# Chris10M/Ev2Hands

Hardware: AMD Instinct MI355X
Metric: event-windows/sec at B=256 N=2048 (f16x2) (higher is better)
Workload: dtype f32 (each f32 operand split into 2 fp16 planes with per-window power-of-two range scaling, 3 plane products per MAC on the f16 MFMA, f32 accumulate); 1 GPU; TEHNet.forward+MANO both hands, B=256/GPU N=2048 C=4 fp32, E-clouds, random-init 342-key checkpoint, synthetic MANO-shaped assets; global_batch=256, points=2048, channels=4, precision=f16x2, forwards_in_flight=1, world_size_seen=1, parallelism=batch-shard x1

## Files before the change

### ev2hands_amd/csrc/attention.hip

```cpp
#include "common.hpp"
#include "ev2hands_hip.h"

namespace {

constexpr int ATT_D = 256;

__global__ __launch_bounds__(1024) void attn_sim_kernel(const float4* __restrict__ logits, const float* __restrict__ query,
                                                        int ldq, size_t hand_stride, int N, float* __restrict__ sim) {
    __shared__ float red[4][4][ATT_D];
    const int b = blockIdx.x, h = blockIdx.y;
    const int d = threadIdx.x & (ATT_D - 1), part = threadIdx.x >> 8;
    const int per = (N + 3) / 4;
    const int n_lo = part * per, n_hi = min(N, n_lo + per);
    const float* q = query + h * hand_stride + (size_t)b * N * ldq + d;
    const float4* kk = logits + (size_t)b * N;
    float a0 = 0.f, a1 = 0.f, a2 = 0.f, a3 = 0.f;
    int n = n_lo;
    for (; n + 4 <= n_hi; n += 4) {
        const float q0 = q[(size_t)n * ldq], q1 = q[(size_t)(n + 1) * ldq], q2 = q[(size_t)(n + 2) * ldq],
                    q3 = q[(size_t)(n + 3) * ldq];
        const float4 k0 = kk[n], k1 = kk[n + 1], k2 = kk[n + 2], k3 = kk[n + 3];
        a0 = fmaf(k0.x, q0, a0); a1 = fmaf(k0.y, q0, a1); a2 = fmaf(k0.z, q0, a2); a3 = fmaf(k0.w, q0, a3);
        a0 = fmaf(k1.x, q1, a0); a1 = fmaf(k1.y, q1, a1); a2 = fmaf(k1.z, q1, a2); a3 = fmaf(k1.w, q1, a3);
        a0 = fmaf(k2.x, q2, a0); a1 = fmaf(k2.y, q2, a1); a2 = fmaf(k2.z, q2, a2); a3 = fmaf(k2.w, q2, a3);
        a0 = fmaf(k3.x, q3, a0); a1 = fmaf(k3.y, q3, a1); a2 = fmaf(k3.z, q3, a2); a3 = fmaf(k3.w, q3, a3);
    }
    for (; n < n_hi; ++n) {
        const float q0 = q[(size_t)n * ldq];
        const float4 k0 = kk[n];
        a0 = fmaf(k0.x, q0, a0); a1 = fmaf(k0.y, q0, a1); a2 = fmaf(k0.z, q0, a2); a3 = fmaf(k0.w, q0, a3);
    }
    red[part][0][d] = a0; red[part][1][d] = a1; red[part][2][d] = a2; red[part][3][d] = a3;
    __syncthreads();
    if (part == 0) {
        float s[4];
#pragma unroll
        for (int c = 0; c < 4; ++c) {
            const float t = ((red[0][c][d] + red[1][c][d]) + red[2][c][d]) + red[3][c][d];
            s[c] = 0.0625f * t;
        }
        const float mx = fmaxf(fmaxf(s[0], s[1]), fmaxf(s[2], s[3]));
        float e[4], sum = 0.f;
#pragma unroll
        for (int c = 0; c < 4; ++c) { e[c] = expf(s[c] - mx); sum += e[c]; }
#pragma unroll
        for (int c = 0; c < 4; ++c) sim[(((size_t)b * 2 + h) * 4 + c) * ATT_D + d] = e[c] / sum;
    }
}

constexpr int ZS_ROWS = 256;

__global__ __launch_bounds__(256) void attn_zsum_kernel(const float4* __restrict__ logits, const float* __restrict__ q1, int ldq, int N,
                                                        float* __restrict__ zpart) {
    __shared__ float4 sk[ZS_ROWS + 2];
    const int b = blockIdx.y, ch = blockIdx.x, nch = gridDim.x, tid = threadIdx.x;
    const int n0 = ch * ZS_ROWS, n1 = min(N, n0 + ZS_ROWS);
    for (int i = tid; i < ZS_ROWS + 2; i += 256) {
        const int n = n0 - 1 + i;
        sk[i] = (n >= 0 && n < N) ? logits[(size_t)b * N + n] : make_float4(0.f, 0.f, 0.f, 0.f);
    }
    __syncthreads();
    float ax[3][4], ay[3][4];
#pragma unroll
    for (int t = 0; t < 3; ++t)
#pragma unroll
        for (int c = 0; c < 4; ++c) { ax[t][c] = 0.f; ay[t][c] = 0.f; }
    const float* qp = q1 + ((size_t)b * N + n0) * ldq + 2 * tid;
    auto step = [&](int i, float2 v) {
#pragma unroll
        for (int t = 0; t < 3; ++t) {
            const float4 k = sk[i + 2 - t];
            ax[t][0] = fmaf(k.x, v.x, ax[t][0]); ax[t][1] = fmaf(k.y, v.x, ax[t][1]); ax[t][2] = fmaf(k.z, v.x, ax[t][2]); ax[t][3] = fmaf(k.w, v.x, ax[t][3]);
            ay[t][0] = fmaf(k.x, v.y, ay[t][0]); ay[t][1] = fmaf(k.y, v.y, ay[t][1]); ay[t][2] = fmaf(k.z, v.y, ay[t][2]); ay[t][3] = fmaf(k.w, v.y, ay[t][3]);
        }
    };
    const int rows = n1 - n0;
    int i = 0;
    for (; i + 4 <= rows; i += 4) {
        float2 v[4];
#pragma unroll
        for (int u = 0; u < 4; ++u) v[u] = *reinterpret_cast<const float2*>(qp + (size_t)(i + u) * ldq);
#pragma unroll
        for (int u = 0; u < 4; ++u) step(i + u, v[u]);
    }
    for (; i < rows; ++i) step(i, *reinterpret_cast<const float2*>(qp + (size_t)i * ldq));
    float* zp = zpart + ((size_t)b * nch + ch) * 12 * 512 + 2 * tid;
#pragma unroll
    for (int c = 0; c < 4; ++c)
#pragma unroll
        for (int t = 0; t < 3; ++t) *reinterpret_cast<float2*>(zp + (c * 3 + t) * 512) = make_float2(ax[t][c], ay[t][c]);
}

__global__ __launch_bounds__(1024) void attn_simfold_kernel(const float* __restrict__ zpart, int nch, const float4* __restrict__ logits, int N,
                                                            const float* __restrict__ w4t0, const float* __restrict__ w4t1,
                                                            const float* __restrict__ b40, const float* __restrict__ b41, float* __restrict__ sim) {
    __shared__ float4 zs[3 * ATT_D];
    __shared__ float4 kp[1024];
    __shared__ float4 kp2[32];
    __shared__ float red[3][4][ATT_D];
    const int b = blockIdx.x, h = blockIdx.y, tid = threadIdx.x, d = tid & (ATT_D - 1), q = tid >> 8;
    const float* w4t = h ? w4t1 : w4t0;
    if (q < 3) {
        float z[4] = {0.f, 0.f, 0.f, 0.f};
        for (int ch = 0; ch < nch; ++ch)
#pragma unroll
            for (int c = 0; c < 4; ++c) z[c] += zpart[(((size_t)b * nch + ch) * 12 + c * 3 + q) * 512 + h * ATT_D + d];
        zs[q * ATT_D + d] = make_float4(z[0], z[1], z[2], z[3]);
    }
    float4 ks = make_float4(0.f, 0.f, 0.f, 0.f);
    for (int n = tid; n < N; n += 1024) {
        const float4 k = logits[(size_t)b * N + n];
        ks.x += k.x; ks.y += k.y; ks.z += k.z; ks.w += k.w;
    }
    kp[tid] = ks;
    __syncthreads();
    if (tid < 32) {
        float4 k2 = kp[tid * 32];
        for (int j = 1; j < 32; ++j) { const float4 k = kp[tid * 32 + j]; k2.x += k.x; k2.y += k.y; k2.z += k.z; k2.w += k.w; }
        kp2[tid] = k2;
    }
    __syncthreads();
    float a0 = 0.f, a1 = 0.f, a2 = 0.f, a3 = 0.f;
    if (q == 0) {
        float4 K = kp2[0];
        for (int j = 1; j < 32; ++j) { const float4 k = kp2[j]; K.x += k.x; K.y += k.y; K.z += k.z; K.w += k.w; }
        const float bd = (h ? b41 : b40)[d];
        a0 = bd * K.x; a1 = bd * K.y; a2 = bd * K.z; a3 = bd * K.w;
    }
    constexpr int KQ = 3 * ATT_D / 4;
#pragma unroll 8
    for (int k = q * KQ; k < (q + 1) * KQ; ++k) {
        const float w = w4t[(size_t)k * ATT_D + d];
        const float4 z = zs[k];
        a0 = fmaf(w, z.x, a0); a1 = fmaf(w, z.y, a1); a2 = fmaf(w, z.z, a2); a3 = fmaf(w, z.w, a3);
    }
    if (q > 0) { red[q - 1][0][d] = a0; red[q - 1][1][d] = a1; red[q - 1][2][d] = a2; red[q - 1][3][d] = a3; }
    __syncthreads();
    if (q == 0) {
        const float t[4] = {a0, a1, a2, a3};
        float s[4];
#pragma unroll
        for (int c = 0; c < 4; ++c) s[c] = 0.0625f * (((t[c] + red[0][c][d]) + red[1][c][d]) + red[2][c][d]);
        const float mx = fmaxf(fmaxf(s[0], s[1]), fmaxf(s[2], s[3]));
        float e[4], sum = 0.f;
#pragma unroll
        for (int c = 0; c < 4; ++c) { e[c] = expf(s[c] - mx); sum += e[c]; }
#pragma unroll
        for (int c = 0; c < 4; ++c) sim[(((size_t)b * 2 + h) * 4 + c) * ATT_D + d] = e[c] / sum;
    }
}

constexpr int CTX_PTS_PER_WAVE = 32;
template <int VBF16>
__global__ __launch_bounds__(256) void attn_context_kernel(const float* __restrict__ sim, const float* __restrict__ value,
                                                           int ldv, int N, size_t rows_total, float* __restrict__ hf8,
                                                           unsigned* __restrict__ amax, int amax_hand_stride,
                                                           const float* __restrict__ value_unscale, const float* __restrict__ vscale = nullptr) {
    const int b = blockIdx.y;
    const int lane = threadIdx.x & 63, wave = threadIdx.x >> 6;
    float4 w[2][4];
    const float4 vu = value_unscale ? *reinterpret_cast<const float4*>(value_unscale + lane * 4) : make_float4(1.f, 1.f, 1.f, 1.f);
#pragma unroll
    for (int h = 0; h < 2; ++h)
#pragma unroll
        for (int c = 0; c < 4; ++c) {
            float4 t = *reinterpret_cast<const float4*>(sim + (((size_t)b * 2 + h) * 4 + c) * ATT_D + lane * 4);
            t.x *= vu.x; t.y *= vu.y; t.z *= vu.z; t.w *= vu.w;
            if constexpr (VBF16 == 2) {
                const float iv = 1.f / vscale[b];
                t.x *= iv; t.y *= iv; t.z *= iv; t.w *= iv;
            }
            w[h][c] = t;
        }
    const int n0 = (blockIdx.x * 4 + wave) * CTX_PTS_PER_WAVE;
    unsigned am = 0u;
    for (int n = n0; n < n0 + CTX_PTS_PER_WAVE && n < N; ++n) {
        const size_t row = (size_t)b * N + n;
        float4 v;
        if constexpr (VBF16 == 1) {
            const uint2 h = *reinterpret_cast<const uint2*>(reinterpret_cast<const unsigned short*>(value) + row * ldv + lane * 4);
            v = make_float4(__uint_as_float(h.x << 16), __uint_as_float(h.x & 0xffff0000u), __uint_as_float(h.y << 16), __uint_as_float(h.y & 0xffff0000u));
        } else if constexpr (VBF16 == 2) {
            typedef _Float16 h16x2 __attribute__((ext_vector_type(2)));
            const uint2 h = *reinterpret_cast<const uint2*>(reinterpret_cast<const unsigned short*>(value) + row * ldv + lane * 4);
            const h16x2 a = __builtin_bit_cast(h16x2, h.x), b_ = __builtin_bit_cast(h16x2, h.y);
            v = make_float4((float)a[0], (float)a[1], (float)b_[0], (float)b_[1]);
        } else {
            v = *reinterpret_cast<const float4*>(value + row * ldv + lane * 4);
        }
        float acc[8];
#pragma unroll
        for (int h = 0; h < 2; ++h)
#pragma unroll
            for (int c = 0; c < 4; ++c)
                acc[h * 4 + c] = fmaf(w[h][c].w, v.w, fmaf(w[h][c].z, v.z, fmaf(w[h][c].y, v.y, w[h][c].x * v.x)));
        float r4[4], r2[2];
        const bool hi32 = lane & 32, hi16 = lane & 16, hi8 = lane & 8;
#pragma unroll
        for (int i = 0; i < 4; ++i) r4[i] = (hi32 ? acc[4 + i] : acc[i]) + __shfl_xor(hi32 ? acc[i] : acc[4 + i], 32, 64);
#pragma unroll
        for (int i = 0; i < 2; ++i) r2[i] = (hi16 ? r4[2 + i] : r4[i]) + __shfl_xor(hi16 ? r4[i] : r4[2 + i], 16, 64);
        float r = (hi8 ? r2[1] : r2[0]) + __shfl_xor(hi8 ? r2[0] : r2[1], 8, 64);
        r += __shfl_xor(r, 4, 64);
        r += __shfl_xor(r, 2, 64);
        r += __shfl_xor(r, 1, 64);
        if ((lane & 7) == 0) {
            const int gsum = lane >> 3;
            hf8[((size_t)(gsum >> 2) * rows_total + row) * 8 + (gsum & 3)] = r;
            am = max(am, __float_as_uint(r) & 0x7fffffffu);
        } else if ((lane & 7) == 4) {
            const int gsum = lane >> 3;
            hf8[((size_t)(gsum >> 2) * rows_total + row) * 8 + 4 + (gsum & 3)] = 0.f;
        }
    }
    if (amax) {
        unsigned a0 = wave_max_u32_dpp(lane < 32 ? am : 0u), a1 = wave_max_u32_dpp(lane < 32 ? 0u : am);
        if (lane == 0) {
            if (a0) atomicMax(&amax[b], a0);
            if (a1) atomicMax(&amax[amax_hand_stride + b], a1);
        }
    }
}

}

extern "C" int ev2h_attn_sim(const float* logits_pm, const float* query_pm, int ldq, size_t query_hand_stride, int B, int N,
                             float* sim, ev2h_stream_t stream) {
    EV2H_CHECK_ARG(logits_pm && query_pm && sim && B > 0 && N > 0 && ldq >= ATT_D);
    dim3 grid(B, 2);
    attn_sim_kernel<<<grid, 1024, 0, (hipStream_t)stream>>>((const float4*)logits_pm, query_pm, ldq, query_hand_stride, N, sim);
    EV2H_CHECK_LAUNCH();
    return EV2H_OK;
}

extern "C" size_t ev2h_attn_sim_folded_scratch(int B, int N) {
    if (B <= 0 || N <= 0) return 0;
    return (size_t)B * ceil_div(N, ZS_ROWS) * 12 * 512;
}

int ev2h_attn_simfold_partials(const float* zpart, int rows_per_partial, const float* logits_pm, int B, int N, const float* w4t_left,
                               const float* w4t_right, const float* b4_left, const float* b4_right, float* sim, ev2h_stream_t stream) {
    EV2H_CHECK_ARG(zpart && logits_pm && w4t_left && w4t_right && b4_left && b4_right && sim && B > 0 && N > 0 && rows_per_partial > 0 &&
                   N % rows_per_partial == 0);
    attn_simfold_kernel<<<dim3(B, 2), 1024, 0, (hipStream_t)stream>>>(zpart, N / rows_per_partial, (const float4*)logits_pm, N, w4t_left, w4t_right,
                                                                      b4_left, b4_right, sim);
    EV2H_CHECK_LAUNCH();
    return EV2H_OK;
}

extern "C" int ev2h_attn_sim_folded(const float* logits_pm, const float* q1_pm, int ldq, int B, int N, const float* w4t_left,
                                    const float* w4t_right, const float* b4_left, const float* b4_right, float* scratch, float* sim,
                                    ev2h_stream_t stream) {
    EV2H_CHECK_ARG(logits_pm && q1_pm && w4t_left && w4t_right && b4_left && b4_right && scratch && sim);
    EV2H_CHECK_ARG(B > 0 && N > 0 && ldq >= 2 * ATT_D && (ldq % 2) == 0);
    const int nch = ceil_div(N, ZS_ROWS);
    attn_zsum_kernel<<<dim3(nch, B), 256, 0, (hipStream_t)stream>>>((const float4*)logits_pm, q1_pm, ldq, N, scratch);
    EV2H_CHECK_LAUNCH();
    attn_simfold_kernel<<<dim3(B, 2), 1024, 0, (hipStream_t)stream>>>(scratch, nch, (const float4*)logits_pm, N, w4t_left, w4t_right, b4_left,
                                                                      b4_right, sim);
    EV2H_CHECK_LAUNCH();
    return EV2H_OK;
}

extern "C" int ev2h_attn_context(const float* sim, const float* value_pm, int ldv, int B, int N, float* hf8, uint32_t* hf_amax,
                                 int amax_hand_stride, const float* value_unscale, ev2h_stream_t stream) {
    EV2H_CHECK_ARG(sim && value_pm && hf8 && B > 0 && N > 0 && ldv >= ATT_D && (ldv % 4) == 0);
    dim3 grid(ceil_div(N, 4 * CTX_PTS_PER_WAVE), B);
    attn_context_kernel<0><<<grid, 256, 0, (hipStream_t)stream>>>(sim, value_pm, ldv, N, (size_t)B * N, hf8, hf_amax, amax_hand_stride, value_unscale);
    EV2H_CHECK_LAUNCH();
    return EV2H_OK;
}

int ev2h_attn_context_bf16rows(const float* sim, const void* value_pm, int ldv, int B, int N, float* hf8, const float* value_unscale, ev2h_stream_t stream) {
    EV2H_CHECK_ARG(sim && value_pm && hf8 && B > 0 && N > 0 && ldv >= ATT_D && (ldv % 4) == 0);
    dim3 grid(ceil_div(N, 4 * CTX_PTS_PER_WAVE), B);
    attn_context_kernel<1><<<grid, 256, 0, (hipStream_t)stream>>>(sim, reinterpret_cast<const float*>(value_pm), ldv, N, (size_t)B * N, hf8, nullptr, 0, value_unscale);
    EV2H_CHECK_LAUNCH();
    return EV2H_OK;
}

int ev2h_attn_context_f16rows(const float* sim, const void* value_pm, int ldv, int B, int N, float* hf8, uint32_t* hf_amax, int amax_hand_stride,
                              const float* value_unscale, const float* vscale, ev2h_stream_t stream) {
    EV2H_CHECK_ARG(sim && value_pm && hf8 && vscale && B > 0 && N > 0 && ldv >= ATT_D && (ldv % 4) == 0);
    dim3 grid(ceil_div(N, 4 * CTX_PTS_PER_WAVE), B);
    attn_context_kernel<2><<<grid, 256, 0, (hipStream_t)stream>>>(sim, reinterpret_cast<const float*>(value_pm), ldv, N, (size_t)B * N, hf8, hf_amax, amax_hand_stride,
                                                                 value_unscale, vscale);
    EV2H_CHECK_LAUNCH();
    return EV2H_OK;
}
```

### ev2hands_amd/csrc/forward.hip

```cpp
#include <cstdarg>
#include <cstdio>
#include <cstdlib>
#include <cstring>

#include "common.hpp"
#include "planes.hpp"
#include "ev2hands_hip.h"
#include "side_stream.hpp"
#include "workspace.hpp"

int ev2h_gemm_init();

static thread_local char g_err[512] = "";

void ev2h_set_error(const char* fmt, ...) {
    va_list ap;
    va_start(ap, fmt);
    vsnprintf(g_err, sizeof(g_err), fmt, ap);
    va_end(ap);
}

extern "C" const char* ev2h_last_error(void) { return g_err; }
extern "C" int ev2h_abi_version(void) { return EV2H_ABI_VERSION; }

extern "C" void ev2h_struct_sizes(size_t out[8]) {
    out[0] = sizeof(ev2h_gemm_desc);
    out[1] = sizeof(ev2h_sa_desc);
    out[2] = sizeof(ev2h_sa_module);
    out[3] = sizeof(ev2h_weights);
    out[4] = sizeof(ev2h_mano_consts);
    out[5] = sizeof(ev2h_outputs);
    out[6] = sizeof(ev2h_fp_desc);
    out[7] = sizeof(ev2h_tensor_desc);
}

extern "C" int ev2h_init(void) {
    (void)ev2h_side_ctx(nullptr, false);
    return ev2h_gemm_init();
}

static thread_local struct {
    char tag[32];
    hipEvent_t* start;
    hipEvent_t* stop;
    int n;
    long calls;
} g_prof = {"", nullptr, nullptr, 0, 0};

extern "C" int ev2h_profile_set(const char* tag, void** start_events, void** stop_events, int n) {
    if (!tag || n <= 0 || !start_events || !stop_events) {
        g_prof.tag[0] = 0; g_prof.start = g_prof.stop = nullptr; g_prof.n = 0; g_prof.calls = 0;
        return EV2H_OK;
    }
    snprintf(g_prof.tag, sizeof(g_prof.tag), "%s", tag);
    g_prof.start = reinterpret_cast<hipEvent_t*>(start_events);
    g_prof.stop = reinterpret_cast<hipEvent_t*>(stop_events);
    g_prof.n = n;
    g_prof.calls = 0;
    return EV2H_OK;
}

static inline bool prof_hit(const char* tag) { return g_prof.n > 0 && !strcmp(tag, g_prof.tag); }
static inline void prof_begin(const char* tag, ev2h_stream_t st) {
    if (prof_hit(tag)) (void)hipEventRecord(g_prof.start[g_prof.calls % g_prof.n], (hipStream_t)st);
}
static inline void prof_end(const char* tag, ev2h_stream_t st) {
    if (prof_hit(tag)) { (void)hipEventRecord(g_prof.stop[g_prof.calls % g_prof.n], (hipStream_t)st); ++g_prof.calls; }
}

namespace {
__global__ void clock_probe_kernel(unsigned long long ticks, unsigned long long* out) {
    const unsigned long long c0 = __builtin_amdgcn_s_memtime(), r0 = __builtin_amdgcn_s_memrealtime();
    unsigned long long r1 = r0;
    while (r1 - r0 < ticks) { __builtin_amdgcn_s_sleep(8); r1 = __builtin_amdgcn_s_memrealtime(); }
    const unsigned long long c1 = __builtin_amdgcn_s_memtime();
    r1 = __builtin_amdgcn_s_memrealtime();
    if (threadIdx.x == 0) { out[0] = c1 - c0; out[1] = r1 - r0; }
}
}

extern "C" int ev2h_shader_clock_probe(ev2h_stream_t stream, int spin_us, unsigned long long* out_dev) {
    EV2H_CHECK_ARG(out_dev && spin_us > 0 && spin_us <= 100000);
    clock_probe_kernel<<<1, 64, 0, (hipStream_t)stream>>>((unsigned long long)spin_us * 100ull, out_dev);
    EV2H_CHECK_LAUNCH();
    return EV2H_OK;
}

int ev2h_fps_multi_chunk(const float* pts4, int B, int N, int njobs, const int* S, const int64_t* const* init, int32_t* const* idx, float* const* ctr4,
                         int s_begin, int s_end, float* state, ev2h_stream_t stream);
int ev2h_ball_query_range(const float* pts4, const float* ctr4, int B, int N, int S, int s_off, int s_cnt, int nrad, const double* radius,
                          const int* nsample, int32_t* const* gidx, int32_t* cnt, ev2h_stream_t stream);
bool ev2h_gemm_bf16_zsum_supported(const ev2h_gemm_desc* d);
int ev2h_gemm_bf16_zsum(const ev2h_gemm_desc* d, const float* key_pm, float* zpart, int x_bf16, ev2h_stream_t stream, const float* x_scale = nullptr);
int ev2h_fp_mlp_ex(const ev2h_fp_desc* d, int t_bf16, int out_bf16, ev2h_stream_t stream, float* row16_scale = nullptr, float w3_norm = 0.f, float b3_max = 0.f);
int ev2h_attn_context_f16rows(const float* sim, const void* value_pm, int ldv, int B, int N, float* hf8, uint32_t* hf_amax, int amax_hand_stride,
                              const float* value_unscale, const float* vscale, ev2h_stream_t stream);
int ev2h_attn_context_bf16rows(const float* sim, const void* value_pm, int ldv, int B, int N, float* hf8, const float* value_unscale, ev2h_stream_t stream);
int ev2h_attn_simfold_partials(const float* zpart, int rows_per_partial, const float* logits_pm, int B, int N, const float* w4t_left,
                               const float* w4t_right, const float* b4_left, const float* b4_right, float* sim, ev2h_stream_t stream);

namespace {

struct Call {
    Ws ws;
    int prec = EV2H_PREC_F32;
    int f16_families = 0;
    ev2h_stream_t st = nullptr;
    SideCtx* side = nullptr;
    int fam_prec(int fam) const { return prec == EV2H_PREC_F16 && !(f16_families & fam) ? EV2H_PREC_F16X2 : prec; }
    int signal_side(int e) const {
        if (!side) return EV2H_OK;
        EV2H_CHECK_HIP(hipEventRecord(side->ev[e], (hipStream_t)st));
        EV2H_CHECK_HIP(hipStreamWaitEvent(side->stream, side->ev[e], 0));
        return EV2H_OK;
    }
    int side_records(int e) const {
        if (side) EV2H_CHECK_HIP(hipEventRecord(side->ev[e], side->stream));
        return EV2H_OK;
    }
    int wait_side(int e) const {
        if (side) EV2H_CHECK_HIP(hipStreamWaitEvent((hipStream_t)st, side->ev[e], 0));
        return EV2H_OK;
    }
};

struct Rng {
    const uint32_t* xa = nullptr; const uint32_t* xa2 = nullptr; int xg = 0;
    uint32_t* ya = nullptr; int yg = 0;
};

#define RUN(expr)                 \
    do {                          \
        int rc__ = (expr);        \
        if (rc__) return rc__;    \
    } while (0)

struct DenseOpt {
    const float* group_bias = nullptr; int group_rows = 0, ldbias = 0;
    int taps = 1, rows_per_seq = 0;
    int rowmax_rows = 0;
    int skinny = 0;
    int fam = EV2H_FAM_DENSE;
};

static ev2h_gemm_desc dense_desc(const Call& cx, const ev2h_dense& w, const float* X, int ldx, int M, float* Y, int ldy, int relu, const Rng& rg,
                                 const DenseOpt& o = {}) {
    ev2h_gemm_desc d{};
    d.skinny = o.skinny;
    d.x_amax = rg.xa; d.x_amax2 = rg.xa2; d.x_group_rows = rg.xg; d.y_amax = rg.ya; d.y_group_rows = rg.yg;
    d.X = X; d.ldx = ldx; d.W = w.W; d.ldw = w.ldw; d.Y = Y; d.ldy = ldy;
    d.M = M; d.N = w.O; d.K = w.K;
    d.bias = o.group_bias ? o.group_bias : w.b;
    d.bias_group_rows = o.group_rows; d.ldbias = o.ldbias;
    d.relu = relu; d.post_scale = w.post_scale; d.post_shift = w.post_shift;
    d.taps = o.taps; d.rows_per_seq = o.rows_per_seq; d.rowmax_rows = o.rowmax_rows;
    d.precision = cx.fam_prec(o.fam);
    d.Ws = (cx.prec != EV2H_PREC_F32) ? w.Ws : nullptr;
    d.ws_tile_rows = w.ws_tile_rows;
    d.w_unscale = w.w_unscale;
    return d;
}

static int dense(const Call& cx, const ev2h_dense& w, const float* X, int ldx, int M, float* Y, int ldy, int relu, ev2h_stream_t st, const Rng& rg,
                 const DenseOpt& o = {}) {
    const ev2h_gemm_desc d = dense_desc(cx, w, X, ldx, M, Y, ldy, relu, rg, o);
    return ev2h_gemm(&d, st);
}

static int sa_table(int precision, const ev2h_sa_module& m, const float* feat, int ldf, int B, int Npts, float* P1, ev2h_stream_t st,
                    const uint32_t* feat_amax, uint32_t* p1_amax, float* p1_scale, bool chain = true) {
    int c1sum = 0;
    float extra = 0.f;
    for (int i = 0; i < m.nbranch; ++i) {
        c1sum += m.br[i].C1;
        extra = fmaxf(extra, m.br[i].w1x_norm * (float)m.br[i].radius * 1.0000002f);
    }
    ev2h_gemm_desc g{};
    g.X = feat; g.ldx = ldf; g.W = m.W1f; g.ldw = m.kf; g.Y = P1; g.ldy = c1sum;
    g.M = B * Npts; g.N = c1sum; g.K = m.kf; g.bias = m.b1; g.taps = 1;
    g.precision = precision;
    g.w_unscale = m.w1f_unscale;
    if (precision != EV2H_PREC_F32 && m.W1fs) { g.Ws = m.W1fs; g.ws_tile_rows = 128; }
    if (feat_amax) {
        g.x_amax = feat_amax; g.x_group_rows = Npts;
        g.y_amax = p1_amax; g.y_group_rows = Npts;
        g.y_scale = p1_scale; g.y_bound_w = m.w1f_norm; g.y_bound_b = m.b1_max + extra;
        if (precision == EV2H_PREC_F16 && chain) {
            float wmul = 1.f, badd = g.y_bound_b;
            for (int i = 0; i < m.nbranch; ++i) {
                const float iu = 1.000001f / (m.br[i].w2_unscale > 0.f ? m.br[i].w2_unscale : 1.f);
                wmul = fmaxf(wmul, m.br[i].w2_norm * iu);
                badd = fmaxf(badd, (m.br[i].w2_norm * g.y_bound_b + m.br[i].b2_max) * iu);
            }
            g.y_bound_w *= wmul; g.y_bound_b = badd;
        }
    }
    return ev2h_gemm(&g, st);
}

static bool bf16_direct_layer1(int precision, const ev2h_sa_module& m) {
    static const bool table = getenv("EV2H_L1_TABLE") != nullptr;
    return precision != EV2H_PREC_F32 && m.kf == 8 && !table;
}

static int sa_branches(int precision, const char* tag, const ev2h_sa_module& m, const float* pts4, const float* ctr4, int32_t* const* gidx,
                       const int32_t* cnt, int B, int Npts, const float* P1, float* out, int ldo, ev2h_stream_t st, bool ranges,
                       const uint32_t* p1_amax, const float* p1_scale, uint32_t* out_amax, const float* feat = nullptr, int nfeat = 0,
                       const uint32_t* feat_amax = nullptr, float* xyz_out = nullptr, int xyz_ld = 0, int s_off = 0, int s_cnt = 0) {
    int c1sum = 0;
    for (int i = 0; i < m.nbranch; ++i) c1sum += m.br[i].C1;
    int coff1 = 0, coff3 = 0;
    for (int i = 0; i < m.nbranch; ++i) {
        const ev2h_sa_branch& br = m.br[i];
        ev2h_sa_desc d{};
        d.P1 = P1 + coff1; d.ldp = c1sum; d.pts4 = pts4; d.ctr4 = ctr4; d.gidx = gidx[i];
        d.W1x = br.W1x; d.W2 = br.W2; d.b2 = br.b2; d.W3 = br.W3; d.b3 = br.b3;
        d.out = out + coff3; d.ldo = ldo;
        d.B = B; d.Npts = Npts; d.S = m.npoint; d.K = br.K; d.C1 = br.C1; d.C2 = br.C2; d.C3 = br.C3;
        if (s_cnt > 0) { d.S = s_cnt; d.S_total = m.npoint; d.s_off = s_off; }
        d.precision = precision; d.W2s = br.W2s; d.W3s = br.W3s; d.w2_unscale = br.w2_unscale; d.w3_unscale = br.w3_unscale;
        const bool direct = feat && bf16_direct_layer1(precision, m);
        if (direct) {
            d.feat = feat; d.ldf = 8; d.W1f = m.W1f + (size_t)coff1 * m.kf; d.ldw1f = m.kf; d.b1 = m.b1 + coff1; d.nfeat = nfeat;
            d.w1f_unscale = br.w1f_unscale; d.w1x_unscale = br.w1x_unscale;
            if (ranges) { d.feat_amax = feat_amax; d.w1f_norm = m.w1f_norm; d.b1_max = m.b1_max; }
        }
        if (ranges) {
            if (!direct) { d.p1_scale = p1_scale; d.p1_amax = p1_amax; }
            d.out_amax = out_amax;
            d.w1x_norm = br.w1x_norm; d.dmax = (float)br.radius * 1.0000002f ; d.w2_norm = br.w2_norm; d.b2_max = br.b2_max;
        }
        d.cnt = cnt ? cnt + i : nullptr; d.cnt_ld = m.nbranch;
        if (i == 0 && xyz_out) { d.xyz_out = xyz_out; d.xyz_ld = xyz_ld; }
        char t[40];
        snprintf(t, sizeof(t), "%s.%d", tag, i);
        prof_begin(t, st);
        RUN(ev2h_sa_mlp_max(&d, st));
        prof_end(t, st);
        coff1 += br.C1;
        coff3 += br.C3;
    }
    return EV2H_OK;
}

static int sa_module(int precision, const char* tag, const ev2h_sa_module& m, const float* feat, int ldf, const float* pts4, const float* ctr4,
                     int32_t* const* gidx, const int32_t* cnt, int B, int Npts, float* P1, float* out, int ldo, ev2h_stream_t st,
                     const uint32_t* feat_amax, uint32_t* p1_amax, float* p1_scale, uint32_t* out_amax, int nfeat = 0, float* xyz_out = nullptr,
                     int xyz_ld = 0) {
    if (!bf16_direct_layer1(precision, m)) RUN(sa_table(precision, m, feat, ldf, B, Npts, P1, st, feat_amax, p1_amax, p1_scale));
    return sa_branches(precision, tag, m, pts4, ctr4, gidx, cnt, B, Npts, P1, out, ldo, st, feat_amax != nullptr, p1_amax, p1_scale, out_amax,
                       ldf == 8 ? feat : nullptr, nfeat, feat_amax, xyz_out, xyz_ld);
}

}

static int forward_body(const ev2h_weights* w, const ev2h_mano_consts* const* mano, float* xyz_cm, int B, int C, int N, int mhlnes,
                        const int64_t* fps_init, const ev2h_outputs* out, const Call& cx, bool* forked) {
    const Ws& ws = cx.ws;
    const ev2h_stream_t st = cx.st;
    const int R = B * N;
    const int prec = cx.prec;
    const int prec_sa = cx.fam_prec(EV2H_FAM_SA), prec_rows = cx.fam_prec(EV2H_FAM_ROWS), prec_q = cx.fam_prec(EV2H_FAM_QCONV);
    auto rg = [&](int xid, int xg, int yid = -1, int yg = 0, int xid2 = -1) {
        Rng r{};
        if (ws.ranges_on) {
            r.xa = ws.r(xid); r.xg = xg;
            if (xid2 >= 0) r.xa2 = ws.r(xid2);
            if (yid >= 0) { r.ya = ws.r(yid); r.yg = yg; }
        }
        return r;
    };
    if (ws.ranges_on) EV2H_CHECK_HIP(hipMemsetAsync(ws.i(WS_RANGES), 0, ws.L.count[WS_RANGES] * 4, (hipStream_t)st));

    RUN(ev2h_prep_points(xyz_cm, B, C, N, mhlnes, ws.f(WS_PTS4), ws.f(WS_FEAT8), ws.r(R_FEAT), st));
    const bool fork = cx.side != nullptr;
    const ev2h_stream_t sd = fork ? (ev2h_stream_t)cx.side->stream : st;
    RUN(cx.signal_side(EV_INPUT));
    *forked = fork;
    if (!bf16_direct_layer1(prec, w->sa1)) RUN(sa_table(prec_sa, w->sa1, ws.f(WS_FEAT8), 8, B, N, ws.f(WS_P1A), sd, ws.r(R_FEAT), ws.r(R_P1A), ws.p1scale(0)));
    RUN(cx.side_records(EV_SA1_TABLE));
    static const int chunk_env = [] { const char* e = getenv("EV2H_FPS_CHUNKS"); return e ? atoi(e) : -1; }();
    const int chunk_max_wg = chunk_env > 1 ? chunk_env : (N <= 2048 ? 0x7fffffff : 256), chunk_min_b = chunk_env > 1 ? 1 : 8;
    const bool chunked = fork && chunk_env != 0 && B >= chunk_min_b && 3 * B <= chunk_max_wg && bf16_direct_layer1(prec, w->sa1) && w->sa1.npoint % FPS_CHUNKS == 0;
    {
        const int S[3] = {512, 128, 128};
        const int64_t* init[3] = {fps_init, fps_init + 2 * (size_t)B, fps_init + 3 * (size_t)B};
        int32_t* idx[3] = {ws.i(WS_FPS1), ws.i(WS_FPSM_L), ws.i(WS_FPSM_R)};
        float* ctr[3] = {ws.f(WS_CTR1), ws.f(WS_CTRM_L), ws.f(WS_CTRM_R)};
        if (!chunked) {
            RUN(ev2h_fps_multi(ws.f(WS_PTS4), B, N, 3, S, init, idx, ctr, st));
        } else {
            const int q = w->sa1.npoint / FPS_CHUNKS;
            for (int c = 0; c < FPS_CHUNKS; ++c) {
                RUN(ev2h_fps_multi_chunk(ws.f(WS_PTS4), B, N, 3, S, init, idx, ctr, c * q, (c + 1) * q, ws.f(WS_FPS_STATE), sd));
                RUN(cx.side_records(EV_SA1_QUARTER0 + c));
            }
        }
    }
    if (!chunked) RUN(cx.signal_side(EV_SAMPLED));
    int32_t* gi2[2] = {ws.i(WS_GIDX2_0), ws.i(WS_GIDX2_1)};
    {
        const ev2h_sa_module& m = w->sa2;
        RUN(ev2h_fps(ws.f(WS_CTR1), B, 512, 128, fps_init + (size_t)B, ws.i(WS_FPS2), ws.f(WS_CTR2), sd));
        double rad[2]; int ns[2];
        for (int i = 0; i < 2; ++i) { rad[i] = m.br[i].radius; ns[i] = m.br[i].K; }
        RUN(ev2h_ball_query(ws.f(WS_CTR1), ws.f(WS_CTR2), B, 512, 128, 2, rad, ns, gi2, ws.i(WS_CNT2), sd));
        RUN(cx.side_records(EV_SA2_QUERY));
    }
    static const bool unfused_fp1 = getenv("EV2H_FP1_UNFUSED") != nullptr;
    const bool fp1_fused = prec != EV2H_PREC_F32 && w->fp1m.W1fs && !unfused_fp1;
    if (fp1_fused) {
        RUN(ev2h_three_nn_interp(ws.f(WS_PTS4), ws.f(WS_CTR1), B, N, 512, nullptr, 0, 0, nullptr, 0, ws.i(WS_NN1_IDX), ws.f(WS_NN1_W), nullptr, sd));
        RUN(cx.side_records(EV_FP1_NN));
    }
    for (int h = 0; h < 2; ++h) {
        const ev2h_sa_module& m = w->mano_sa1[h];
        double rad[2]; int ns[2];
        int32_t* gi[2] = {ws.i(hand(WS_GIDXM0_L, h)), ws.i(hand(WS_GIDXM1_L, h))};
        for (int i = 0; i < 2; ++i) { rad[i] = m.br[i].radius; ns[i] = m.br[i].K; }
        RUN(ev2h_ball_query(ws.f(WS_PTS4), ws.f(hand(WS_CTRM_L, h)), B, N, 128, 2, rad, ns, gi, ws.i(hand(WS_CNTM_L, h)), sd));
    }
    RUN(cx.side_records(EV_HAND_QUERIES));
    {
        const ev2h_sa_module& m = w->sa1;
        double rad[3]; int ns[3];
        int32_t* gi[3] = {ws.i(WS_GIDX1_0), ws.i(WS_GIDX1_1), ws.i(WS_GIDX1_2)};
        for (int i = 0; i < 3; ++i) { rad[i] = m.br[i].radius; ns[i] = m.br[i].K; }
        if (!chunked) {
            RUN(ev2h_ball_query(ws.f(WS_PTS4), ws.f(WS_CTR1), B, N, 512, 3, rad, ns, gi, ws.i(WS_CNT1), st));
            RUN(cx.wait_side(EV_SA1_TABLE));
            RUN(sa_branches(prec_sa, "sa1", m, ws.f(WS_PTS4), ws.f(WS_CTR1), gi, ws.i(WS_CNT1), B, N, ws.f(WS_P1A), ws.f(WS_L1CAT), 576, st, ws.ranges_on,
                            ws.r(R_P1A), ws.p1scale(0), ws.r(R_L1A), ws.f(WS_FEAT8), C, ws.r(R_FEAT)));
        } else {
            const int q = m.npoint / FPS_CHUNKS;
            for (int c = 0; c < FPS_CHUNKS; ++c) {
                RUN(cx.wait_side(EV_SA1_QUARTER0 + c));
                RUN(ev2h_ball_query_range(ws.f(WS_PTS4), ws.f(WS_CTR1), B, N, 512, c * q, q, 3, rad, ns, gi, ws.i(WS_CNT1), st));
                RUN(sa_branches(prec_sa, "sa1", m, ws.f(WS_PTS4), ws.f(WS_CTR1), gi, ws.i(WS_CNT1), B, N, ws.f(WS_P1A), ws.f(WS_L1CAT), 576, st, ws.ranges_on,
                                ws.r(R_P1A), ws.p1scale(0), ws.r(R_L1A), ws.f(WS_FEAT8), C, ws.r(R_FEAT), nullptr, 0, c * q, q));
            }
        }
    }
    {
        const ev2h_sa_module& m = w->sa2;
        RUN(cx.wait_side(EV_SA2_QUERY));
        RUN(sa_module(prec_sa, "sa2", m, ws.f(WS_L1CAT), 576, ws.f(WS_CTR1), ws.f(WS_CTR2), gi2, ws.i(WS_CNT2), B, 512, ws.f(WS_P1B), ws.f(WS_L2BUF), 520, st,
                      ws.r(R_L1A), ws.r(R_P1B), ws.p1scale(1), ws.r(R_L2), 0, ws.f(WS_L2BUF) + 512, 520));
    }
    RUN(dense(cx, w->sa3[0], ws.f(WS_L2BUF), 520, B * 128, ws.f(WS_SA3H1), 256, 1, st, rg(R_L2, 128, R_SA3H1, 128, R_FEAT)));
    RUN(dense(cx, w->sa3[1], ws.f(WS_SA3H1), 256, B * 128, ws.f(WS_SA3H2), 512, 1, st, rg(R_SA3H1, 128, R_SA3H2, 128)));
    RUN(dense(cx, w->sa3[2], ws.f(WS_SA3H2), 512, B * 128, ws.f(WS_L3), 1024, 1, st, rg(R_SA3H2, 128, R_L3, 1), {.rowmax_rows = 128}));
    RUN(dense(cx, w->fp3_bcast, ws.f(WS_L3), 1024, B, ws.f(WS_FP3BIAS), 256, 0, st, rg(R_L3, 1), {.skinny = 1}));
    RUN(dense(cx, w->fp3_skip, ws.f(WS_L2BUF), 520, B * 128, ws.f(WS_FP3H), 256, 1, st, rg(R_L2, 128, R_FP3H, 128, R_FEAT),
              {.group_bias = ws.f(WS_FP3BIAS), .group_rows = 128, .ldbias = 256}));
    RUN(dense(cx, w->fp3_1, ws.f(WS_FP3H), 256, B * 128, ws.f(WS_FP3O), 256, 1, st, rg(R_FP3H, 128, R_FP3O, 128)));
    RUN(ev2h_three_nn_interp(ws.f(WS_CTR1), ws.f(WS_CTR2), B, 512, 128, ws.f(WS_FP3O), 256, 256, ws.f(WS_L1CAT) + 320, 576,
                             ws.i(WS_NN2_IDX), ws.f(WS_NN2_W), ws.r(R_L1B), st));
    RUN(dense(cx, w->fp2[0], ws.f(WS_L1CAT), 576, B * 512, ws.f(WS_FP2H), 256, 1, st, rg(R_L1A, 512, R_FP2H, 512, R_L1B)));
    RUN(dense(cx, w->fp2[1], ws.f(WS_FP2H), 256, B * 512, ws.f(WS_L1NEW), 128, 1, st, rg(R_FP2H, 512, R_L1NEW, 512)));
    static const bool unfused_cls = getenv("EV2H_CLS_UNFUSED") != nullptr;
    static const bool unfused_zsum = getenv("EV2H_ATTN_UNFUSED_ZSUM") != nullptr;
    static const bool l0_f32 = getenv("EV2H_L0_F32") != nullptr;
    const bool cls_fused = prec != EV2H_PREC_F32 && w->clsm.W2s && !unfused_cls;
    const ev2h_gemm_desc qd = dense_desc(cx, w->qconv0, ws.f(WS_L0), 256, R, ws.f(WS_Q1), 512, 1, rg(R_L0, N),
                                         {.taps = 3, .rows_per_seq = N, .fam = EV2H_FAM_QCONV});
    const bool zsum_ok = !unfused_zsum && prec != EV2H_PREC_F32 && w->qconv0.Ws && ev2h_gemm_bf16_zsum_supported(&qd);
    const bool l0_bf16 = prec == EV2H_PREC_BF16 && fp1_fused && cls_fused && zsum_ok && !l0_f32;
    const bool l0_f16 = prec == EV2H_PREC_F16 && prec_rows == EV2H_PREC_F16 && prec_q == EV2H_PREC_F16 && ws.ranges_on && fp1_fused && cls_fused && zsum_ok && !l0_f32;
    const bool l0_16 = l0_bf16 || l0_f16;
    g_last_l0_bf16 = l0_bf16 ? 1 : (l0_f16 ? 2 : 0);
    if (fp1_fused) {
        const ev2h_sa_module& m = w->fp1m;
        RUN(cx.wait_side(EV_FP1_NN));
        RUN(sa_table(prec_rows, m, ws.f(WS_L1NEW), 128, B, 512, ws.f(WS_FP1T), st, ws.r(R_L1NEW), ws.r(R_FP1T), ws.p1scale(4), false));
        ev2h_fp_desc d{};
        d.T = ws.f(WS_FP1T); d.ldt = 128; d.nn_idx = ws.i(WS_NN1_IDX); d.nn_w = ws.f(WS_NN1_W);
        d.b2 = m.br[0].b2; d.b3 = m.br[0].b3; d.W2s = m.br[0].W2s; d.W3s = m.br[0].W3s;
        d.w2_unscale = m.br[0].w2_unscale; d.w3_unscale = m.br[0].w3_unscale;
        d.out = ws.f(WS_L0); d.ldo = 256; d.B = B; d.N = N; d.S = 512; d.C1 = 128; d.C2 = 128; d.C3 = 256; d.precision = prec_rows;
        if (ws.ranges_on) {
            d.t_scale = ws.p1scale(4); d.t_amax = ws.r(R_FP1T); d.w2_norm = m.br[0].w2_norm; d.b2_max = m.br[0].b2_max; d.out_amax = ws.r(R_L0);
        }
        prof_begin("fp1", st);
        RUN(ev2h_fp_mlp_ex(&d, 0, l0_16, st, l0_f16 ? ws.p1scale(5) : nullptr, m.br[0].w3_norm, m.br[0].b3_max));
        prof_end("fp1", st);
    } else {
        RUN(ev2h_three_nn_interp(ws.f(WS_PTS4), ws.f(WS_CTR1), B, N, 512, ws.f(WS_L1NEW), 128, 128, ws.f(WS_FP1IN), 128,
                                 ws.i(WS_NN1_IDX), ws.f(WS_NN1_W), ws.r(R_FP1IN), st));
        RUN(dense(cx, w->fp1[0], ws.f(WS_FP1IN), 128, R, ws.f(WS_FP1H1), 128, 1, st, rg(R_FP1IN, N, R_FP1H1, N)));
        RUN(dense(cx, w->fp1[1], ws.f(WS_FP1H1), 128, R, ws.f(WS_FP1H2), 128, 1, st, rg(R_FP1H1, N, R_FP1H2, N)));
        RUN(dense(cx, w->fp1[2], ws.f(WS_FP1H2), 128, R, ws.f(WS_L0), 256, 1, st, rg(R_FP1H2, N, R_L0, N)));
    }
    RUN(cx.signal_side(EV_L0));
    if (cls_fused) {
        const ev2h_sa_branch& c = w->clsm;
        ev2h_fp_desc d{};
        d.T = ws.f(WS_L0); d.ldt = 256; d.b2 = c.b2; d.b3 = c.b3; d.W2s = c.W2s; d.W3s = c.W3s;
        d.w2_unscale = c.w2_unscale; d.w3_unscale = c.w3_unscale;
        d.out = ws.f(WS_LOGITS_PM); d.ldo = 4; d.out_cols = 4; d.no_relu_out = 1; d.out_cm = out->class_logits; d.out_cm_stride = out->logits_stride;
        d.B = B; d.N = N; d.C1 = c.C1; d.C2 = c.C2; d.C3 = c.C3; d.precision = prec_rows;
        if (ws.ranges_on) { d.t_amax = ws.r(R_L0); d.w2_norm = c.w2_norm; d.b2_max = c.b2_max; }
        RUN(ev2h_fp_mlp_ex(&d, l0_16, 0, sd, l0_f16 ? ws.p1scale(5) : nullptr));
    } else {
        RUN(dense(cx, w->cls0, ws.f(WS_L0), 256, R, ws.f(WS_CLSH), 256, 1, sd, rg(R_L0, N, R_CLSH, N)));
        RUN(dense(cx, w->cls4, ws.f(WS_CLSH), 256, R, ws.f(WS_LOGITS_PM), 4, 0, sd, rg(R_CLSH, N)));
        RUN(ev2h_transpose_logits(ws.f(WS_LOGITS_PM), B, N, out->class_logits, out->logits_stride, sd));
    }
    RUN(cx.side_records(EV_LOGITS));
    if (zsum_ok) {
        RUN(cx.wait_side(EV_LOGITS));
        prof_begin("qconv0", st);
        RUN(ev2h_gemm_bf16_zsum(&qd, ws.f(WS_LOGITS_PM), ws.f(WS_ZPART), l0_16, st, l0_f16 ? ws.p1scale(5) : nullptr));
        prof_end("qconv0", st);
    } else {
        prof_begin("qconv0", st);
        RUN(ev2h_gemm(&qd, st));
        prof_end("qconv0", st);
    }
    RUN(cx.wait_side(EV_LOGITS));
    if (zsum_ok) {
        RUN(ev2h_attn_simfold_partials(ws.f(WS_ZPART), 128, ws.f(WS_LOGITS_PM), B, N, w->qconv4T[0], w->qconv4T[1], w->qconv4[0].b, w->qconv4[1].b,
                                       ws.f(WS_SIM), st));
    } else {
        RUN(ev2h_attn_sim_folded(ws.f(WS_LOGITS_PM), ws.f(WS_Q1), 512, B, N, w->qconv4T[0], w->qconv4T[1], w->qconv4[0].b, w->qconv4[1].b,
                                 ws.f(WS_ZPART), ws.f(WS_SIM), st));
    }
    if (l0_bf16) RUN(ev2h_attn_context_bf16rows(ws.f(WS_SIM), ws.f(WS_L0), 256, B, N, ws.f(WS_HF8), w->l0_unscale, st));
    else if (l0_f16) RUN(ev2h_attn_context_f16rows(ws.f(WS_SIM), ws.f(WS_L0), 256, B, N, ws.f(WS_HF8), ws.r(R_HF), B, w->l0_unscale, ws.p1scale(5), st));
    else RUN(ev2h_attn_context(ws.f(WS_SIM), ws.f(WS_L0), 256, B, N, ws.f(WS_HF8), ws.r(R_HF), B, w->l0_unscale, st));
    RUN(cx.wait_side(EV_HAND_QUERIES));
    RUN(cx.signal_side(EV_HF8));
    for (int h = 0; h < 2; ++h) {
        const ev2h_sa_module& m = w->mano_sa1[h];
        ev2h_stream_t sh = (h == 1) ? sd : st;
        int32_t* gi[2] = {ws.i(hand(WS_GIDXM0_L, h)), ws.i(hand(WS_GIDXM1_L, h))};
        RUN(sa_module(prec_sa, h ? "manoR" : "manoL", m, ws.f(WS_HF8) + (size_t)h * R * 8, 8, ws.f(WS_PTS4), ws.f(hand(WS_CTRM_L, h)), gi, ws.i(hand(WS_CNTM_L, h)), B, N, ws.f(hand(WS_P1M_L, h)), ws.f(hand(WS_M1BUF_L, h)), 520, sh,
                      ws.r(R_HF + h), ws.r(R_P1M + h), ws.p1scale(2 + h), ws.r(R_M1 + h), 4, ws.f(hand(WS_M1BUF_L, h)) + 512, 520));
        RUN(dense(cx, w->mano_sa2[h][0], ws.f(hand(WS_M1BUF_L, h)), 520, B * 128, ws.f(hand(WS_MSA2H_L, h)), 256, 1, sh, rg(R_M1 + h, 128, R_MSA2H + h, 128, R_FEAT)));
        RUN(dense(cx, w->mano_sa2[h][1], ws.f(hand(WS_MSA2H_L, h)), 256, B * 128, ws.f(hand(WS_M2_L, h)), 512, 1, sh, rg(R_MSA2H + h, 128, R_M2 + h, 1), {.rowmax_rows = 128}));
        RUN(dense(cx, w->head0[h], ws.f(hand(WS_M2_L, h)), 512, B, ws.f(hand(WS_FC1_L, h)), 1024, 1, sh, rg(R_M2 + h, 1, R_FC1 + h, 1), {.skinny = 1}));
        const int ldprm = out->params_stride ? (int)out->params_stride : w->head4[h].O;
        RUN(dense(cx, w->head4[h], ws.f(hand(WS_FC1_L, h)), 1024, B, out->params[h], ldprm, 0, sh, rg(R_FC1 + h, 1), {.skinny = 1}));
        if (mano[h]) RUN(ev2h_mano(mano[h], out->params[h], ldprm, B, out->vertices[h], out->vertices_stride, out->joints[h], out->joints_stride, sh));
    }
    return EV2H_OK;
}

extern "C" int ev2h_forward(const ev2h_weights* w, const ev2h_mano_consts* mano_left, const ev2h_mano_consts* mano_right,
                            float* xyz_cm, int B, int C, int N, int mhlnes, const int64_t* fps_init, const ev2h_outputs* out,
                            void* workspace, size_t workspace_bytes, ev2h_stream_t st) {
    EV2H_CHECK_ARG(w && xyz_cm && fps_init && out && workspace);
    EV2H_CHECK_ARG(B > 0 && N >= 128 && N <= 32768 && (C == 4 || C == 5));
    EV2H_CHECK_ARG(out->class_logits && out->params[0] && out->params[1]);
    EV2H_CHECK_ARG(!mano_left || (out->vertices[0] && out->joints[0]));
    EV2H_CHECK_ARG(!mano_right || (out->vertices[1] && out->joints[1]));
    EV2H_CHECK_ARG((out->logits_stride == 0 || out->logits_stride >= (size_t)4 * N) && (out->params_stride == 0 || out->params_stride >= (size_t)w->head4[0].O));
    EV2H_CHECK_ARG(w->head4[0].O == w->head4[1].O && w->head4[0].O >= 17 && w->head4[0].O <= 61);
    for (int h = 0; h < 2; ++h) {
        const ev2h_mano_consts* mc = h ? mano_right : mano_left;
        if (mc && 3 + mc->ncomps + 13 != w->head4[h].O) {
            ev2h_set_error("ev2h_forward: the checkpoint regresses %d pose coefficients per hand, the %s MANO model takes %d", w->head4[h].O - 16,
                           h ? "right" : "left", mc->ncomps);
            return EV2H_ERR_ARG;
        }
    }
    EV2H_CHECK_ARG(out->params_stride <= 0x7fffffff);
    EV2H_CHECK_ARG((out->vertices_stride == 0 || out->vertices_stride >= 2334) && (out->joints_stride == 0 || out->joints_stride >= 63));
    EV2H_CHECK_ARG(w->sa1.npoint == 512 && w->sa2.npoint == 128 && w->mano_sa1[0].npoint == 128 && w->mano_sa1[1].npoint == 128);
    EV2H_CHECK_ARG(w->sa1.nbranch == 3 && w->sa2.nbranch == 2 && w->mano_sa1[0].nbranch == 2 && w->mano_sa1[1].nbranch == 2);
    if ((w->precision == EV2H_PREC_F16X2 || w->precision == EV2H_PREC_F16) && !(w->flags & (EV2H_W_EQUALIZED | EV2H_W_UNEQUALIZED_OK))) {
        ev2h_set_error("ev2h_forward: F16X2 / F16 weights are not channel-equalised (pack them with ev2h_pack_weights(..., EV2H_PACK_EQUALIZE), "
                       "or set EV2H_W_UNEQUALIZED_OK in ev2h_weights.flags to run them anyway, or use BF16X3 / F32)");
        return EV2H_ERR_ARG;
    }
    RUN(ev2h_init());
    Call cx;
    cx.prec = w->precision;
    cx.f16_families = w->precision == EV2H_PREC_F16 ? w->f16_families : 0;
    cx.st = st;
    Ws& ws = cx.ws;
    ws.base = static_cast<char*>(workspace);
    ws.B = B;
    ws.ranges_on = (w->precision == EV2H_PREC_F16X2 || w->precision == EV2H_PREC_F16);
    build_layout(ws.L, B, N);
    if (workspace_bytes < ws.L.total) {
        ev2h_set_error("ev2h_forward: workspace too small (%zu < %zu bytes)", workspace_bytes, ws.L.total);
        return EV2H_ERR_WORKSPACE;
    }
    const ev2h_mano_consts* mano[2] = {mano_left, mano_right};
    SideCtx* side = ev2h_side_ctx(st, true);
    if (g_side_disabled) side = nullptr;
    cx.side = side;
    bool forked = false;
    const int rc = forward_body(w, mano, xyz_cm, B, C, N, mhlnes, fps_init, out, cx, &forked);
    if (forked) {
        const hipError_t e1 = hipEventRecord(side->ev[EV_JOIN], side->stream);
        const hipError_t e2 = hipStreamWaitEvent((hipStream_t)st, side->ev[EV_JOIN], 0);
        if (rc == EV2H_OK && (e1 != hipSuccess || e2 != hipSuccess)) {
            ev2h_set_error("ev2h_forward: joining the side stream failed: %s", hipGetErrorString(e1 != hipSuccess ? e1 : e2));
            return EV2H_ERR_HIP;
        }
    }
    return rc;
}
```

### ev2hands_amd/csrc/gemm_bf16.hip

```cpp
#include <cstdlib>

#include "planes.hpp"
#include "ev2hands_hip.h"

namespace {


constexpr int GB_BM = 128, GB_BN = 128, GB_BK = 32, GB_THREADS = 512;
constexpr int GO_THREADS_ = 256, GB_BN_ = 128;

struct GemmBP {
    const float* X; int ldx;
    const float* W; int ldw;
    float* Y; int ldy;
    int M, N, K;
    const float* bias; int bias_group_rows; int ldbias;
    int relu;
    const float* post_scale; const float* post_shift;
    int taps; int Kc; int rows_per_seq;
    int rowmax_rows;
    float w_unscale;
    const unsigned* x_amax; const unsigned* x_amax2; int x_group_rows;
    unsigned* y_amax; int y_group_rows;
    float* y_scale; float y_bound_w, y_bound_b;
// ... 449 lines not shown
        for (int i = lane; i < 4 * KLD; i += 64) km = fmaxf(km, (i % KLD) < GB_BM + 2 ? fabsf(keyL[i]) : 0.f);
        sk = f16x2_scale(wave_max_u32_dpp(__float_as_uint(km)));
    }
    const int m = l31 < 12 ? l31 : 0, kc = m / 3, kt = m - 3 * kc;
    const float* kr = keyL + kc * KLD + 2 - kt + wm * 64;
    f32x16 z[2];
#pragma unroll
    for (int j = 0; j < 2; ++j)
#pragma unroll
        for (int r = 0; r < 16; ++r) z[j][r] = 0.f;
#pragma unroll
    for (int i = 0; i < 2; ++i)
#pragma unroll
        for (int kb = 0; kb < 2; ++kb) {
            u32x4 ap[plane_count(NS)];
#pragma unroll
            for (int w = 0; w < 4; ++w) {
                const float a0 = kr[32 * i + mfma_row(8 * kb + 2 * w, half)] * sk, a1 = kr[32 * i + mfma_row(8 * kb + 2 * w + 1, half)] * sk;
                unsigned o[plane_count(NS)];
                split_planes<NS>(a0, a1, o);
#pragma unroll
                for (int s_ = 0; s_ < plane_count(NS); ++s_) ap[s_][w] = o[s_];
            }
#pragma unroll
            for (int j = 0; j < 2; ++j) {
                u32x4 bq[plane_count(NS)];
#pragma unroll
                for (int w = 0; w < 4; ++w) {
                    unsigned o[plane_count(NS)];
                    split_planes<NS>(acc[i][j][8 * kb + 2 * w] * sq, acc[i][j][8 * kb + 2 * w + 1] * sq, o);
#pragma unroll
                    for (int s_ = 0; s_ < plane_count(NS); ++s_) bq[s_][w] = o[s_];
                }
#pragma unroll
                for (int q = 0; q < Planes<NS>::NPROD; ++q) z[j] = mfma_planes<NS>(ap[Planes<NS>::A[q]], bq[Planes<NS>::B[q]], z[j]);
            }
        }
    const float iq = pow2_inverse(sq), ik = pow2_inverse(sk);
    const int ch = pos0 / GB_BM, nch = p.rows_per_seq / GB_BM;
    const long bw = m0 / p.rows_per_seq;
    float* zp = p.zs_out + ((size_t)bw * nch + ch) * 12 * p.N;
    if (wm == 1) {
#pragma unroll
        for (int j = 0; j < 2; ++j)
#pragma unroll
            for (int r = 0; r < 8; ++r) {
                const int mr = mfma_row(r, half);
                if (mr < 12) red[mr * GB_BN_ + wn * 64 + j * 32 + l31] = (z[j][r] * iq) * ik;
            }
    }
    __syncthreads();
    if (wm == 0) {
#pragma unroll
        for (int j = 0; j < 2; ++j)
#pragma unroll
            for (int r = 0; r < 8; ++r) {
                const int mr = mfma_row(r, half);
                const int col = n0 + wn * 64 + j * 32 + l31;
                if (mr < 12 && col < p.N) zp[(size_t)mr * p.N + col] = (z[j][r] * iq) * ik + red[mr * GB_BN_ + wn * 64 + j * 32 + l31];
            }
    }
}

constexpr int GO_BN = 128, GO_THREADS = 256;

template <int NS, bool TAP3>
struct GOCfg {
    static constexpr int RS = plane_count(NS) * 64 + 16;
    static constexpr int A_ROWS = GB_BM + (TAP3 ? 2 : 0);
    static constexpr int A_BYTES = A_ROWS * RS;
    static constexpr int B_BYTES = GO_BN * RS;
    static constexpr int LDS_BYTES = A_BYTES + B_BYTES;
};

template <int NS, bool TAP3, bool PIPE = false, bool ZS = false>
__global__ __launch_bounds__(GO_THREADS, 3) void gemm_nt_bf16_occ_kernel(GemmBP p, const char* __restrict__ Ws) {
    static_assert(!ZS || TAP3, "the q1-free epilogue belongs to the tap kernel");
    using Cfg = GOCfg<NS, TAP3>;
    constexpr int RS = Cfg::RS;
    static_assert(!(PIPE && TAP3), "the pipelined variant is for the plain K loop");
    extern __shared__ __attribute__((aligned(16))) char smem[];
    char* sA = smem;
    char* sB = smem + Cfg::A_BYTES;

    const int L = xcd_remap(blockIdx.x, p.nblk);
    const int tn = L % p.tiles_n, tm = L / p.tiles_n;
    const int m0 = tm * GB_BM, n0 = tn * GO_BN;
    const int tid = threadIdx.x, lane = tid & 63;
    const int wave = __builtin_amdgcn_readfirstlane(tid >> 6);
    const int wm = wave >> 1, wn = wave & 1;
    const int half = lane >> 5, l31 = lane & 31;
    const int lrow = tid >> 1, lseg = tid & 1;
    const int nk = (p.K + GB_BK - 1) / GB_BK;
    f32x4 ra[4], rh[4];
    bool oka = true, okh = true, fulla = true;
    const float xs = x_row_scale<NS>(p, m0);
    const float xsh = xs;

    auto load16 = [&](const float* g, bool full, f32x4 (&r)[4]) {
        const float* g2 = full ? g + 8 : g;
        asm volatile("global_load_dwordx4 %0, %4, off\n\tglobal_load_dwordx4 %1, %4, off offset:16\n\t"
                     "global_load_dwordx4 %2, %5, off\n\tglobal_load_dwordx4 %3, %5, off offset:16"
                     : "=&v"(r[0]), "=&v"(r[1]), "=&v"(r[2]), "=&v"(r[3]) : "v"(g), "v"(g2) : "memory");
    };
    auto gload = [&](int kt, f32x4 (&dst)[4]) {
        const int k = kt * GB_BK + lseg * 16;
        int tap = 0, kc = k;
        if (p.taps == 3) { tap = k / p.Kc; kc = k - tap * p.Kc; }
        const int m = m0 + lrow;
        bool ok = (m < p.M) && (k < p.K);
        long src = m;
        if (p.taps == 3) {
            const int pos = m % p.rows_per_seq + tap - 1;
            ok = ok && (pos >= 0) && (pos < p.rows_per_seq);
            src = (long)m + tap - 1;
        }
        fulla = (k + 16 <= p.K);
        load16(p.X + (ok ? src : 0) * p.ldx + (ok ? kc : 0), fulla, dst);
        oka = ok;
    };
    auto load16h = [&](const unsigned short* g, f32x4 (&r)[4]) {
        asm volatile("global_load_dwordx4 %0, %2, off\n\tglobal_load_dwordx4 %1, %2, off offset:16" : "=&v"(r[0]), "=&v"(r[1]) : "v"(g) : "memory");
    };
    auto gload3 = [&](int kc) {
        const int k = kc * GB_BK + lseg * 16;
        const int m = m0 + lrow;
        oka = m < p.M;
        const bool xh = (NS == 1 || NS == 4) && p.x_bf16;
        if (xh) load16h(reinterpret_cast<const unsigned short*>(p.X) + (oka ? (long)m : 0) * p.ldx + k, ra);
        else load16(p.X + (oka ? (long)m : 0) * p.ldx + k, true, ra);
        if (tid < 4) {
            const long mh = (tid >> 1) ? (long)m0 + GB_BM : (long)m0 - 1;
            okh = (tid >> 1) ? ((m0 + GB_BM) % p.rows_per_seq != 0 && mh < p.M) : (m0 % p.rows_per_seq != 0);
            if (xh) load16h(reinterpret_cast<const unsigned short*>(p.X) + (okh ? mh : 0) * p.ldx + k, rh);
            else load16(p.X + (okh ? mh : 0) * p.ldx + k, true, rh);
        }
    };
    auto wait_all = [&]() {
        if constexpr (TAP3)
            asm volatile("s_waitcnt vmcnt(0)" : "+v"(ra[0]), "+v"(ra[1]), "+v"(ra[2]), "+v"(ra[3]), "+v"(rh[0]), "+v"(rh[1]), "+v"(rh[2]), "+v"(rh[3]) : : "memory");
        else
            asm volatile("s_waitcnt vmcnt(0)" : "+v"(ra[0]), "+v"(ra[1]), "+v"(ra[2]), "+v"(ra[3]) : : "memory");
    };
    auto swrite_row = [&](const f32x4 (&r)[4], bool ok, int ldsrow, float sc) {
        if constexpr ((NS == 1 || NS == 4) && TAP3) {
            if (p.x_bf16) {
#pragma unroll
                for (int hh = 0; hh < 2; ++hh) {
                    u32x4 v = __builtin_bit_cast(u32x4, r[hh]);
                    if (!ok) v = u32x4{0u, 0u, 0u, 0u};
                    *reinterpret_cast<u32x4*>(sA + ldsrow * RS + lseg * 32 + hh * 16) = v;
                }
                return;
            }
        }
#pragma unroll
        for (int hh = 0; hh < 2; ++hh) {
            f32x4 r0 = r[2 * hh], r1 = r[2 * hh + 1];
            if (!ok || (hh == 1 && !fulla)) { r0 = f32x4{0.f, 0.f, 0.f, 0.f}; r1 = r0; }
            scale_rows<NS>(r0, sc); scale_rows<NS>(r1, sc);
            unsigned q[4][plane_count(NS)];
            split_planes<NS>(r0[0], r0[1], q[0]);
            split_planes<NS>(r0[2], r0[3], q[1]);
            split_planes<NS>(r1[0], r1[1], q[2]);
            split_planes<NS>(r1[2], r1[3], q[3]);
#pragma unroll
            for (int s = 0; s < plane_count(NS); ++s) {
                u32x4 v = {q[0][s], q[1][s], q[2][s], q[3][s]};
                *reinterpret_cast<u32x4*>(sA + ldsrow * RS + s * 64 + lseg * 32 + hh * 16) = v;
            }
        }
    };
    auto dma_b = [&](int kt) {
        const char* src = Ws + ((size_t)tn * nk + kt) * Cfg::B_BYTES;
        for (int off = wave * 1024; off < Cfg::B_BYTES; off += 4 * 1024)
            __builtin_amdgcn_global_load_lds((const __attribute__((address_space(1))) void*)(src + off + lane * 16),
                                             (__attribute__((address_space(3))) void*)(sB + off), 16, 0, 0);
    };
    static_assert(Cfg::B_BYTES % 1024 == 0, "B tile image must be a whole number of 1 KiB DMA pieces");

    f32x16 acc[2][2];
#pragma unroll
    for (int i = 0; i < 2; ++i)
#pragma unroll
        for (int j = 0; j < 2; ++j)
#pragma unroll
            for (int r = 0; r < 16; ++r) acc[i][j][r] = 0.f;

    auto mma_tile = [&](int arow) {
        const char* pa = sA + (wm * 64 + l31 + arow) * RS + half * 16;
        const char* pb = sB + (wn * 64 + l31) * RS + half * 16;
#pragma unroll
        for (int m = 0; m < 2; ++m) {
            u32x4 a[2][plane_count(NS)], b[2][plane_count(NS)];
#pragma unroll
            for (int s = 0; s < plane_count(NS); ++s) {
                a[0][s] = *reinterpret_cast<const u32x4*>(pa + s * 64 + m * 32);
                a[1][s] = *reinterpret_cast<const u32x4*>(pa + 32 * RS + s * 64 + m * 32);
                b[0][s] = *reinterpret_cast<const u32x4*>(pb + s * 64 + m * 32);
                b[1][s] = *reinterpret_cast<const u32x4*>(pb + 32 * RS + s * 64 + m * 32);
            }
#pragma unroll
            for (int q = 0; q < Planes<NS>::NPROD; ++q)
#pragma unroll
                for (int i = 0; i < 2; ++i)
#pragma unroll
                    for (int j = 0; j < 2; ++j)
                        acc[i][j] = mfma_planes<NS>(a[i][Planes<NS>::A[q]], b[j][Planes<NS>::B[q]], acc[i][j]);
        }
        __builtin_amdgcn_s_waitcnt(0x0070);
    };
    if constexpr (TAP3) {
        const int nkc = p.Kc / GB_BK;
        for (int kc = 0; kc < nkc; ++kc) {
            if (kc) __builtin_amdgcn_s_barrier();
            dma_b(kc);
            gload3(kc);
            wait_all();
            swrite_row(ra, oka, lrow + 1, xs);
            if (tid < 4) swrite_row(rh, okh, (tid >> 1) ? GB_BM + 1 : 0, xsh);
            __builtin_amdgcn_s_waitcnt(0x0070);
            __builtin_amdgcn_s_barrier();
#pragma unroll 1
            for (int tap = 0; tap < 3; ++tap) {
                if (tap) {
                    __builtin_amdgcn_s_barrier();
                    dma_b(tap * nkc + kc);
                    __builtin_amdgcn_s_waitcnt(0x0070);
                    __builtin_amdgcn_s_barrier();
                }
                mma_tile(tap);
            }
        }
    } else if constexpr (PIPE) {
        constexpr int KT = 1;
        char* const base = smem;
        auto use = [&](int bufi, int j) { sA = base + (bufi * KT + j) * Cfg::LDS_BYTES; sB = sA + Cfg::A_BYTES; };
        f32x4 rq[KT][4];
        bool okq[KT], fullq[KT];
        auto stage = [&](int kt0, int bufi) {
#pragma unroll
            for (int j = 0; j < KT; ++j)
                if (kt0 + j < nk) {
                    use(bufi, j);
                    dma_b(kt0 + j);
                    gload(kt0 + j, rq[j]);
                    okq[j] = oka; fullq[j] = fulla;
                }
        };
        auto commit = [&](int kt0, int bufi) {
            if constexpr (KT == 2)
                asm volatile("s_waitcnt vmcnt(0)" : "+v"(rq[0][0]), "+v"(rq[0][1]), "+v"(rq[0][2]), "+v"(rq[0][3]), "+v"(rq[1][0]), "+v"(rq[1][1]), "+v"(rq[1][2]), "+v"(rq[1][3]) : : "memory");
            else
                asm volatile("s_waitcnt vmcnt(0)" : "+v"(rq[0][0]), "+v"(rq[0][1]), "+v"(rq[0][2]), "+v"(rq[0][3]) : : "memory");
#pragma unroll
            for (int j = 0; j < KT; ++j)
                if (kt0 + j < nk) {
                    use(bufi, j);
                    fulla = fullq[j];
                    swrite_row(rq[j], okq[j], lrow, xs);
                }
            __builtin_amdgcn_s_waitcnt(0x0070);
        };
        stage(0, 0);
        commit(0, 0);
        int bufi = 0;
        for (int kt = 0; kt < nk; kt += KT, bufi ^= 1) {
            __builtin_amdgcn_s_barrier();
            const bool more = kt + KT < nk;
            if (more) stage(kt + KT, bufi ^ 1);
#pragma unroll
            for (int j = 0; j < KT; ++j)
                if (kt + j < nk) { use(bufi, j); mma_tile(0); }
            if (more) commit(kt + KT, bufi ^ 1);
        }
        __builtin_amdgcn_s_barrier();
    } else {
        for (int kt = 0; kt < nk; ++kt) {
            if (kt) __builtin_amdgcn_s_barrier();
            dma_b(kt);
            gload(kt, ra);
            wait_all();
            swrite_row(ra, oka, lrow, xs);
            __builtin_amdgcn_s_waitcnt(0x0070);
            __builtin_amdgcn_s_barrier();
            mma_tile(0);
        }
    }

    if constexpr (ZS) {
        zsum_epilogue<NS>(p, acc, m0, wm, wn, n0, smem, tid);
        return;
    }
    gemm_epilogue<NS, 2, 2, false>(p, acc, m0, wm * 64, n0 + wn * 64, wm, wn * 64, GO_BN, reinterpret_cast<float*>(smem), tid);
}

template <int NS, bool TAP3, bool ZS = false>
int launch_go_t(const GemmBP& p, const char* Ws, hipStream_t st) {
    static PerDevice attr_set{};
    EV2H_ONCE_PER_DEVICE(attr_set,
        EV2H_CHECK_HIP(hipFuncSetAttribute(reinterpret_cast<const void*>(gemm_nt_bf16_occ_kernel<NS, TAP3, false, ZS>),
                                           hipFuncAttributeMaxDynamicSharedMemorySize, GOCfg<NS, TAP3>::LDS_BYTES)););
    gemm_nt_bf16_occ_kernel<NS, TAP3, false, ZS><<<p.nblk, GO_THREADS, GOCfg<NS, TAP3>::LDS_BYTES, st>>>(p, Ws);
    EV2H_CHECK_LAUNCH();
    return EV2H_OK;
}

template <int NS>
struct GSCfg {
    static constexpr int RS = plane_count(NS) * 64 + 16;
    static constexpr int A_BYTES = 64 * RS, B_BYTES = 64 * RS, BUF = A_BYTES + B_BYTES, LDS_BYTES = 2 * BUF;
};

template <int NS>
__global__ __launch_bounds__(GO_THREADS, 3) void gemm_nt_bf16_small_kernel(GemmBP p, const char* __restrict__ Ws) {
    using Cfg = GSCfg<NS>;
    constexpr int RS = Cfg::RS;
    extern __shared__ __attribute__((aligned(16))) char smem[];
    const int L = xcd_remap(blockIdx.x, p.nblk);
    const int tn = L % p.tiles_n, tm = L / p.tiles_n;
    const int m0 = tm * 64, n0 = tn * 64;
    const int tid = threadIdx.x, lane = tid & 63;
    const int wave = __builtin_amdgcn_readfirstlane(tid >> 6);
    const int wm = wave >> 1, wn = wave & 1;
    const int half = lane >> 5, l31 = lane & 31;
    const int lrow = tid >> 2, lseg = tid & 3;
    const int nk = (p.K + GB_BK - 1) / GB_BK;
    const float xs = x_row_scale<NS>(p, m0);
    f32x4 r0, r1;
    bool ok = true;
    auto gload = [&](int kt) {
        const int k = kt * GB_BK + lseg * 8, m = m0 + lrow;
        ok = (m < p.M) && (k < p.K);
        const float* g = p.X + (ok ? (long)m : 0) * p.ldx + (ok ? k : 0);
        asm volatile("global_load_dwordx4 %0, %2, off\n\tglobal_load_dwordx4 %1, %2, off offset:16" : "=&v"(r0), "=&v"(r1) : "v"(g) : "memory");
    };
    auto commit = [&](char* A) {
        asm volatile("s_waitcnt vmcnt(0)" : "+v"(r0), "+v"(r1) : : "memory");
        f32x4 a = r0, b = r1;
        if (!ok) { a = f32x4{0.f, 0.f, 0.f, 0.f}; b = a; }
        scale_rows<NS>(a, xs); scale_rows<NS>(b, xs);
        unsigned q[4][plane_count(NS)];
        split_planes<NS>(a[0], a[1], q[0]);
        split_planes<NS>(a[2], a[3], q[1]);
        split_planes<NS>(b[0], b[1], q[2]);
        split_planes<NS>(b[2], b[3], q[3]);
#pragma unroll
        for (int s_ = 0; s_ < plane_count(NS); ++s_) {
            u32x4 v = {q[0][s_], q[1][s_], q[2][s_], q[3][s_]};
            *reinterpret_cast<u32x4*>(A + lrow * RS + s_ * 64 + lseg * 16) = v;
        }
        __builtin_amdgcn_s_waitcnt(0x0070);
    };
    auto dma_b = [&](int kt, char* B) {
        const char* src = Ws + ((size_t)(tn >> 1) * nk + kt) * (size_t)(GO_BN * RS) + (size_t)(tn & 1) * Cfg::B_BYTES;
        for (int off = wave * 1024; off < Cfg::B_BYTES; off += 4 * 1024)
            __builtin_amdgcn_global_load_lds((const __attribute__((address_space(1))) void*)(src + off + lane * 16),
                                             (__attribute__((address_space(3))) void*)(B + off), 16, 0, 0);
    };
    static_assert(Cfg::B_BYTES % 1024 == 0, "half an image tile must be a whole number of 1 KiB DMA pieces");
    f32x16 acc[1][1];
#pragma unroll
    for (int r = 0; r < 16; ++r) acc[0][0][r] = 0.f;
    auto mma = [&](const char* A, const char* B) {
        const char* pa = A + (wm * 32 + l31) * RS + half * 16;
        const char* pb = B + (wn * 32 + l31) * RS + half * 16;
#pragma unroll
        for (int m = 0; m < 2; ++m) {
            u32x4 a[plane_count(NS)], b[plane_count(NS)];
#pragma unroll
            for (int s_ = 0; s_ < plane_count(NS); ++s_) {
                a[s_] = *reinterpret_cast<const u32x4*>(pa + s_ * 64 + m * 32);
                b[s_] = *reinterpret_cast<const u32x4*>(pb + s_ * 64 + m * 32);
            }
#pragma unroll
            for (int q = 0; q < Planes<NS>::NPROD; ++q) acc[0][0] = mfma_planes<NS>(a[Planes<NS>::A[q]], b[Planes<NS>::B[q]], acc[0][0]);
        }
        __builtin_amdgcn_s_waitcnt(0x0070);
    };
    dma_b(0, smem + Cfg::A_BYTES);
    gload(0);
    commit(smem);
    for (int kt = 0; kt < nk; ++kt) {
        __builtin_amdgcn_s_barrier();
        const bool more = kt + 1 < nk;
        char* cur = smem + (kt & 1) * Cfg::BUF;
        char* nxt = smem + ((kt + 1) & 1) * Cfg::BUF;
        if (more) { dma_b(kt + 1, nxt + Cfg::A_BYTES); gload(kt + 1); }
        mma(cur, cur + Cfg::A_BYTES);
        if (more) commit(nxt);
    }
    __builtin_amdgcn_s_barrier();
    gemm_epilogue<NS, 1, 1, false>(p, acc, m0, wm * 32, n0 + wn * 32, wm, wn * 32, 64, reinterpret_cast<float*>(smem), tid);
}

template <int NS>
int launch_go_small(GemmBP p, const char* Ws, hipStream_t st) {
    p.tiles_n = ceil_div(p.N, 64);
    p.nblk = ceil_div(p.M, 64) * p.tiles_n;
    static PerDevice attr_set{};
    EV2H_ONCE_PER_DEVICE(attr_set,
        EV2H_CHECK_HIP(hipFuncSetAttribute(reinterpret_cast<const void*>(gemm_nt_bf16_small_kernel<NS>),
                                           hipFuncAttributeMaxDynamicSharedMemorySize, GSCfg<NS>::LDS_BYTES)););
    gemm_nt_bf16_small_kernel<NS><<<p.nblk, GO_THREADS, GSCfg<NS>::LDS_BYTES, st>>>(p, Ws);
    EV2H_CHECK_LAUNCH();
    return EV2H_OK;
}

template <int NS>
constexpr int go_pipe_lds() { return 2 * GOCfg<NS, false>::LDS_BYTES; }

template <int NS>
int launch_go_pipe(const GemmBP& p, const char* Ws, hipStream_t st) {
    static PerDevice attr_set{};
    EV2H_ONCE_PER_DEVICE(attr_set,
        EV2H_CHECK_HIP(hipFuncSetAttribute(reinterpret_cast<const void*>(gemm_nt_bf16_occ_kernel<NS, false, true>),
                                           hipFuncAttributeMaxDynamicSharedMemorySize, go_pipe_lds<NS>())););
    gemm_nt_bf16_occ_kernel<NS, false, true><<<p.nblk, GO_THREADS, go_pipe_lds<NS>(), st>>>(p, Ws);
    EV2H_CHECK_LAUNCH();
    return EV2H_OK;
}

template <int NS>
int launch_go(const GemmBP& p, const char* Ws, hipStream_t st) {
    if (p.taps == 3 && p.Kc % GB_BK == 0 && p.rows_per_seq % GB_BM == 0 && p.M % p.rows_per_seq == 0)
        return launch_go_t<NS, true>(p, Ws, st);
    if (p.nblk <= 64 && p.rowmax_rows == 0 && p.taps == 1) return launch_go_small<NS>(p, Ws, st);
    if (p.nblk <= 128) return launch_go_pipe<NS>(p, Ws, st);
    return launch_go_t<NS, false>(p, Ws, st);
}

}

int ev2h_gemm_tile_geometry(int ns, int out[2]) {
    out[0] = ns == 1 ? GBCfg<1>::RS : ns == 2 ? GBCfg<2>::RS : ns == 3 ? GBCfg<3>::RS : GBCfg<4>::RS;
    out[1] = GB_BK;
    return EV2H_OK;
}

bool ev2h_gemm_bf16_zsum_supported(const ev2h_gemm_desc* d) {
    if (!(d->taps == 3 && d->Ws && d->ws_tile_rows == 128 && (d->precision == EV2H_PREC_F16X2 || d->precision == EV2H_PREC_BF16 || d->precision == EV2H_PREC_BF16X3 || d->precision == EV2H_PREC_F16) &&
          d->K % GB_BK == 0 && d->rows_per_seq > 0 && d->rows_per_seq % GB_BM == 0 && d->M % d->rows_per_seq == 0 && d->N % GO_BN == 0))
        return false;
    if ((d->precision == EV2H_PREC_F16X2 || d->precision == EV2H_PREC_F16) && d->x_amax) {
        const int xg = d->x_group_rows > 0 ? d->x_group_rows : 1;
        if (xg % GB_BM != 0 || xg % d->rows_per_seq != 0) return false;
    }
    return true;
}

int ev2h_gemm_bf16_zsum(const ev2h_gemm_desc* d, const float* key_pm, float* zpart, int x_bf16, ev2h_stream_t stream, const float* x_scale) {
    EV2H_CHECK_ARG(d && key_pm && zpart && ev2h_gemm_bf16_zsum_supported(d));
    EV2H_CHECK_ARG(!x_bf16 || d->precision == EV2H_PREC_BF16 || (d->precision == EV2H_PREC_F16 && x_scale && d->x_group_rows > 0));
    GemmBP p{};
    p.X = d->X; p.ldx = d->ldx; p.W = d->W; p.ldw = d->ldw; p.Y = nullptr; p.ldy = 0;
    p.M = d->M; p.N = d->N; p.taps = 3; p.Kc = d->K; p.K = d->K * 3;
    p.rows_per_seq = d->rows_per_seq;
    p.bias = d->bias; p.relu = d->relu; p.post_scale = d->post_scale; p.post_shift = d->post_shift;
    p.w_unscale = d->w_unscale > 0.f ? d->w_unscale : 1.f;
    p.x_group_rows = p.y_group_rows = 1;
    if ((d->precision == EV2H_PREC_F16X2 || d->precision == EV2H_PREC_F16) && d->x_amax) {
        p.x_amax = d->x_amax; p.x_amax2 = d->x_amax2; p.x_group_rows = d->x_group_rows > 0 ? d->x_group_rows : 1;
    }
    p.zs_key = reinterpret_cast<const float4*>(key_pm); p.zs_out = zpart;
    p.x_bf16 = x_bf16;
    if (x_bf16 && d->precision == EV2H_PREC_F16) { p.x_scale = x_scale; p.x_amax = p.x_amax2 = nullptr; p.x_group_rows = d->x_group_rows; }
    p.tiles_n = d->N / GO_BN;
    p.nblk = (d->M / GB_BM) * p.tiles_n;
    if (d->precision == EV2H_PREC_F16X2) return launch_go_t<2, true, true>(p, (const char*)d->Ws, (hipStream_t)stream);
    if (d->precision == EV2H_PREC_BF16) return launch_go_t<1, true, true>(p, (const char*)d->Ws, (hipStream_t)stream);
    if (d->precision == EV2H_PREC_BF16X3) return launch_go_t<3, true, true>(p, (const char*)d->Ws, (hipStream_t)stream);
    if (d->precision == EV2H_PREC_F16) return launch_go_t<4, true, true>(p, (const char*)d->Ws, (hipStream_t)stream);
    return EV2H_ERR_ARG;
}

int ev2h_gemm_bf16(const ev2h_gemm_desc* d, ev2h_stream_t stream) {
    EV2H_CHECK_ARG((d->K % 8) == 0);
    if (d->taps == 3) EV2H_CHECK_ARG((d->K % 16) == 0);
    GemmBP p{};
    p.X = d->X; p.ldx = d->ldx; p.W = d->W; p.ldw = d->ldw; p.Y = d->Y; p.ldy = d->ldy;
    p.M = d->M; p.N = d->N; p.taps = d->taps; p.Kc = d->K; p.K = d->K * d->taps;
    p.rows_per_seq = d->rows_per_seq;
    p.bias = d->bias; p.bias_group_rows = d->bias_group_rows; p.ldbias = d->ldbias;
    p.relu = d->relu; p.post_scale = d->post_scale; p.post_shift = d->post_shift;
    p.rowmax_rows = d->rowmax_rows;
    p.w_unscale = d->w_unscale > 0.f ? d->w_unscale : 1.f;
    if (d->precision == EV2H_PREC_F16X2 || d->precision == EV2H_PREC_F16) {
        p.x_amax = d->x_amax; p.x_amax2 = d->x_amax2; p.x_group_rows = d->x_group_rows > 0 ? d->x_group_rows : 1;
        p.y_amax = d->y_amax; p.y_group_rows = d->y_group_rows > 0 ? d->y_group_rows : 1;
        p.y_scale = d->y_scale; p.y_bound_w = d->y_bound_w; p.y_bound_b = d->y_bound_b;
        if (!p.x_amax) { p.x_amax2 = nullptr; p.y_scale = nullptr; }
        if (p.y_scale) EV2H_CHECK_ARG(p.x_group_rows == p.y_group_rows && d->rowmax_rows == 0);
        if (d->taps == 3 && p.x_amax) EV2H_CHECK_ARG(p.x_group_rows % d->rows_per_seq == 0);
    } else {
        p.x_group_rows = p.y_group_rows = 1;
    }
    const bool general = (p.x_amax && p.x_group_rows % GB_BM != 0) ||
                         (p.y_amax && d->rowmax_rows == 0 && p.y_group_rows % GB_BM != 0);
    if (general) {
        p.tiles_n = ceil_div(d->N, GB_BN);
        p.nblk = ceil_div(d->M, GB_BM) * p.tiles_n;
        return d->precision == EV2H_PREC_F16 ? launch_gb<4, true>(p, (hipStream_t)stream) : launch_gb<2, true>(p, (hipStream_t)stream);
    }
    if (d->Ws && d->ws_tile_rows == 128) {
        p.tiles_n = ceil_div(d->N, GO_BN);
        p.nblk = ceil_div(d->M, GB_BM) * p.tiles_n;
        if (d->precision == EV2H_PREC_BF16X3) return launch_go<3>(p, (const char*)d->Ws, (hipStream_t)stream);
        if (d->precision == EV2H_PREC_F16X2) return launch_go<2>(p, (const char*)d->Ws, (hipStream_t)stream);
        if (d->precision == EV2H_PREC_BF16) return launch_go<1>(p, (const char*)d->Ws, (hipStream_t)stream);
        if (d->precision == EV2H_PREC_F16) return launch_go<4>(p, (const char*)d->Ws, (hipStream_t)stream);
    }
    if (d->Ws) {
        p.tiles_n = ceil_div(d->N, GW_BN);
        p.nblk = ceil_div(d->M, GB_BM) * p.tiles_n;
        if (d->precision == EV2H_PREC_BF16X3) return launch_gw<3>(p, (const char*)d->Ws, (hipStream_t)stream);
        if (d->precision == EV2H_PREC_F16X2) return launch_gw<2>(p, (const char*)d->Ws, (hipStream_t)stream);
        if (d->precision == EV2H_PREC_BF16) return launch_gw<1>(p, (const char*)d->Ws, (hipStream_t)stream);
        if (d->precision == EV2H_PREC_F16) return launch_gw<4>(p, (const char*)d->Ws, (hipStream_t)stream);
    }
    p.tiles_n = ceil_div(d->N, GB_BN);
    p.nblk = ceil_div(d->M, GB_BM) * p.tiles_n;
    if (d->precision == EV2H_PREC_BF16X3) return launch_gb<3, false>(p, (hipStream_t)stream);
    if (d->precision == EV2H_PREC_F16X2) return launch_gb<2, false>(p, (hipStream_t)stream);
    if (d->precision == EV2H_PREC_BF16) return launch_gb<1, false>(p, (hipStream_t)stream);
    if (d->precision == EV2H_PREC_F16) return launch_gb<4, false>(p, (hipStream_t)stream);
    ev2h_set_error("ev2h_gemm: unknown precision %d", d->precision);
    return EV2H_ERR_ARG;
}
```

### ev2hands_amd/csrc/sa_mlp_bf16.hip

```cpp
#include <algorithm>
#include <cmath>
#include <cstdlib>
#include <type_traits>
#include "planes.hpp"
#include "ev2hands_hip.h"

namespace {

struct SaBP {
    const float* P1; int ldp;
    const float4* pts4;
    const float4* ctr4;
    const int32_t* gidx;
    const float4* W1x;
    const char* W2s; const float* b2;
    const char* W3s; const float* b3;
    float* out; int ldo;
    int B, Npts, S, K;
    int S_total, s_off;
    int nblk;
    const int32_t* cnt; int cnt_ld;
    float u2, u3;
    int per_xcd;
    const float* p1_scale; const unsigned* p1_amax;
    float w1x_norm, dmax, w2_norm, b2_max;
    unsigned* out_amax;
    const int32_t* nn_idx; const float* nn_w; int N;
    int ncols; int relu_out; float* out_cm; size_t out_cm_stride;
    const float* feat; int ldf; const float* W1f; int ldw1f; const float* b1; int nfeat;
    const unsigned* feat_amax; float w1f_norm, b1_max, u1f, u1x;
    float a1f, a1x, a1b;
    int spg;
    float* xyz_out; int xyz_ld;
    int t_bf16, out_bf16;
    float* row16_scale; float w3_norm, b3_max;
};

#ifdef EV2H_SAB_TIMELINE
__device__ long long g_sab_timeline[256];
#define STAMP(i) do { if (dbgw && strip == dbg_strip) g_sab_timeline[(i)] = __builtin_amdgcn_s_memtime(); } while (0)
#else
#define STAMP(i) do { } while (0)
#endif
constexpr int SAB_WAVES = 8;
constexpr int SAB_THREADS = SAB_WAVES * 64;

template <int C1, int C2, int C3, int NS>
struct SaBCfg {
    static constexpr int NPL = plane_count(NS);
    static constexpr bool F16 = planes_f16(NS);
    static constexpr int T2 = (C2 + 31) / 32;
    static constexpr int REM = C2 % 32;
    static constexpr int M_LAST = REM == 0 ? 2 : (REM <= 16 ? 1 : 2);
    static constexpr int C2P = 32 * (T2 - 1) + 16 * M_LAST;
    static constexpr int T3 = C3 / 32;
    static constexpr int NC1 = C1 / 32;
    static constexpr int RS2 = NPL * 64 + 16;
    static constexpr int RS3 = NPL * C2P * 2 + 16;
    static constexpr int TB2 = T2 * 32 * RS2;
    static constexpr int TB3 = 32 * RS3;
    static constexpr int SB2W = F16 ? SAB_WAVES * T2 * 32 * 4 : 0;
    static constexpr int RSA = (NS == 3) ? 112 : 80;
    static constexpr int W1B = (NS == 1 || NS == 4) ? C1 * 32 : F16 ? C1 * RSA + SAB_WAVES * C1 * 4 : C1 * RSA + C1 * 4;
    static constexpr int REC_SLOTS = 64;
    static constexpr int REC = F16 ? REC_SLOTS * 4 : 0;
    static constexpr int SMALL_NOREC = W1B + T2 * 32 * 4 + 16 + SB2W;
    static constexpr int SMALL = SMALL_NOREC + REC;
    static constexpr int tile_bytes(int cpt, int upt) { return ((cpt * TB2 > upt * TB3 ? cpt * TB2 : upt * TB3) + 1023) / 1024 * 1024; }
    static constexpr bool fits(int n) { return NC1 % n == 0 && T3 % n == 0 && 2 * tile_bytes(n, n) + SMALL <= 158 * 1024; }
    static constexpr int CPT = fits(2) ? 2 : 1, UPT = CPT;
    static constexpr int TILE = tile_bytes(CPT, UPT);
    static constexpr int LDS_BYTES = 2 * TILE + SMALL;
    static constexpr int RES_W = (NC1 * TB2 + T3 * TB3 + 1023) / 1024 * 1024;
    static constexpr int RES_LDS_BYTES = RES_W + SMALL;
    static constexpr bool FITS_RESIDENT = RES_LDS_BYTES <= 160 * 1024 && C1 >= 64;
    static constexpr bool PACK4 = (NS == 2) && REM >= 1 && REM <= 4;
};

template <int C1, int C2, int C3, int NS, bool RES, int MODE>
constexpr int sab_min_waves() {
    return (NS == 4 && RES && MODE == 3 && 2 * SaBCfg<C1, C2, C3, NS>::RES_LDS_BYTES <= 160 * 1024) ? 4 : 2;
}
template <int C1, int C2, int C3, int NS, bool RES, int MODE = 0>
__global__ __launch_bounds__(SAB_THREADS, (sab_min_waves<C1, C2, C3, NS, RES, MODE>())) void sa_mlp_max_bf16_kernel(SaBP p) {
    constexpr int WV = SAB_WAVES;
    constexpr bool ROWS = MODE == 1 || MODE == 2, DIRECT = MODE == 2;
    static_assert(!(RES && ROWS), "the row-output variants stream their tiles");
    constexpr bool L1M = (NS == 1 || NS == 4) && !ROWS;
    constexpr bool L1F = (NS == 2 || NS == 3) && MODE == 3;
    constexpr bool L2PIPE = !ROWS && (NS == 1 || NS == 4) && (C1 / 32) % 2 == 0;
    constexpr bool H2FUSE = NS != 3;
    constexpr bool FRAG_PIPE = (NS != 3);
    using Cfg = SaBCfg<C1, C2, C3, NS>;
    using PL = Planes<NS>;
    constexpr int NPL = Cfg::NPL;
    constexpr bool F16 = Cfg::F16;
    constexpr int T2 = Cfg::T2, T3 = Cfg::T3, NC1 = Cfg::NC1, RS2 = Cfg::RS2, RS3 = Cfg::RS3, C2P = Cfg::C2P;
    constexpr int WBYTES = RES ? Cfg::RES_W : 2 * Cfg::TILE;
    extern __shared__ __attribute__((aligned(16))) char smem[];
    char* wt0 = smem;
    char* wt1 = smem + Cfg::TILE;
    f32x4* sW1xT = reinterpret_cast<f32x4*>(smem + WBYTES);
    float* sb2 = reinterpret_cast<float*>(smem + WBYTES + Cfg::W1B);

    const int tid = threadIdx.x, lane = tid & 63;
    const int wave = __builtin_amdgcn_readfirstlane(tid >> 6);
    const int half = lane >> 5, l31 = lane & 31;
    const int L = xcd_remap(blockIdx.x, p.nblk);
    const int ngroups = p.B * p.S;
    constexpr bool hasfeat = MODE == 3;
    constexpr bool fmode = L1F && hasfeat;
    float* sb1w = F16 ? reinterpret_cast<float*>(smem + WBYTES + C1 * Cfg::RSA) + wave * C1 : reinterpret_cast<float*>(smem + WBYTES + C1 * Cfg::RSA);

    if constexpr (L1M) {
        const float iaf = F16 ? 1.f / p.a1f : 1.f, iax = F16 ? 1.f / p.a1x : 1.f, iab = F16 ? 1.f / p.a1b : 1.f;
        for (int i = tid; i < C1; i += WV * 64) {
            const float4 w = p.W1x[i];
            float k[16];
#pragma unroll
            for (int j = 0; j < 16; ++j) k[j] = 0.f;
            k[5] = k[8] = w.x * iax; k[6] = k[9] = w.y * iax; k[7] = k[10] = w.z * iax;
            if (hasfeat) {
                for (int j = 0; j < p.nfeat; ++j) k[j] = p.W1f[(size_t)i * p.ldw1f + j] * iaf;
#pragma unroll
                for (int j = 0; j < 4; ++j) k[12 + j] = k[j];
                k[11] = p.b1[i] * iab;
            }
            unsigned* d = reinterpret_cast<unsigned*>(smem + WBYTES) + i * 8;
#pragma unroll
            for (int j = 0; j < 8; ++j) { unsigned o[1]; split_planes<NS>(k[2 * j], k[2 * j + 1], o); d[j] = o[0]; }
        }
    } else if constexpr (!ROWS) {
        if (fmode) {
            const float iu = F16 ? 1.f / p.u1f : 1.f, iux = F16 ? 1.f / p.u1x : 1.f;
            for (int i = tid; i < C1; i += WV * 64) {
                const float4 w = p.W1x[i];
                float k[8];
#pragma unroll
                for (int j = 0; j < 8; ++j) k[j] = 0.f;
                for (int j = 0; j < p.nfeat; ++j) k[j] = p.W1f[(size_t)i * p.ldw1f + j] * iu;
                k[5] = w.x * iux; k[6] = w.y * iux; k[7] = w.z * iux;
                if constexpr (F16) {
                    unsigned* d = reinterpret_cast<unsigned*>(smem + WBYTES + i * Cfg::RSA);
#pragma unroll
                    for (int j = 0; j < 4; ++j) {
                        unsigned o[2];
                        split_planes<2>(k[2 * j], k[2 * j + 1], o);
                        d[j] = o[0]; d[4 + j] = o[0]; d[8 + j] = o[1]; d[12 + j] = 0u;
                    }
                } else if constexpr (NS == 3) {
                    unsigned* d = reinterpret_cast<unsigned*>(smem + WBYTES + i * Cfg::RSA);
#pragma unroll
                    for (int j = 0; j < 4; ++j) {
                        unsigned o[3];
                        split_planes<3>(k[2 * j], k[2 * j + 1], o);
                        d[j] = o[0]; d[4 + j] = o[0]; d[8 + j] = o[1]; d[12 + j] = o[1]; d[16 + j] = o[2]; d[20 + j] = o[0];
                    }
                    sb1w[i] = p.b1[i];
                }
            }
        } else {
            for (int i = tid; i < C1; i += WV * 64) {
                const float4 w = p.W1x[i];
                float* d = reinterpret_cast<float*>(sW1xT) + (i >> 2) * 12 + (i & 3);
                d[0] = w.x; d[4] = w.y; d[8] = w.z;
            }
        }
    }
    for (int i = tid; i < T2 * 32; i += WV * 64) sb2[i] = p.b2[i] / p.u2;
    float* sbw = F16 ? reinterpret_cast<float*>(smem + WBYTES + Cfg::W1B + T2 * 32 * 4 + 16) + wave * (T2 * 32) : sb2;

    auto dma_tile = [&](const char* src, char* dst, int bytes) {
        for (int off = wave * 1024; off < bytes; off += WV * 1024) {
            if (off + lane * 16 < bytes)
                __builtin_amdgcn_global_load_lds((const __attribute__((address_space(1))) void*)(src + off + lane * 16),
                                                 (__attribute__((address_space(3))) void*)(dst + off), 16, 0, 0);
        }
    };
    constexpr int CPT = RES ? 1 : Cfg::CPT, UPT = RES ? 1 : Cfg::UPT;
    auto dma_w2 = [&](int step, char* dst) { dma_tile(p.W2s + (size_t)step * CPT * Cfg::TB2, dst, CPT * Cfg::TB2); };
    auto dma_w3 = [&](int step, char* dst) { dma_tile(p.W3s + (size_t)step * UPT * Cfg::TB3, dst, UPT * Cfg::TB3); };

    int buf = 0;
    if constexpr (RES && F16) {
        if (tid < Cfg::REC_SLOTS) reinterpret_cast<unsigned*>(smem + WBYTES + Cfg::SMALL_NOREC)[tid] = 0u;
    }
    if constexpr (RES) {
        dma_tile(p.W2s, smem, NC1 * Cfg::TB2);
        dma_tile(p.W3s, smem + NC1 * Cfg::TB2, T3 * Cfg::TB3);
    } else {
        dma_w2(0, wt0);
    }
    asm volatile("s_waitcnt vmcnt(0)" ::: "memory");
    __syncthreads();

    const int xcd = blockIdx.x & 7, slot = blockIdx.x >> 3, nbx = p.nblk >> 3;
    const int g_end = RES ? min(ngroups, (xcd + 1) * p.per_xcd) : ngroups;
  const int spg = (RES || ROWS) ? 1 : max(1, __builtin_amdgcn_readfirstlane(p.spg)), sw = wave % spg;
  for (int g = (RES ? xcd * p.per_xcd + slot * WV : (spg > 1 ? L * (WV / spg) + wave / spg : L * WV)) + wave * (RES || spg == 1); RES ? g < g_end : true;
       g += nbx * WV) {
    const bool valid = g < ngroups;
    const int gg = valid ? g : ngroups - 1;
    const int b = gg / p.S;
    const size_t gf = ROWS ? (size_t)gg : (size_t)b * p.S_total + p.s_off + (gg - b * p.S);
    float mrun[T3];
#pragma unroll
    for (int u = 0; u < T3; ++u) mrun[u] = -INFINITY;

    float4 ctr = make_float4(0.f, 0.f, 0.f, 0.f);
    const int32_t* gi = nullptr;
    if constexpr (!ROWS) { ctr = p.ctr4[gf]; gi = p.gidx + gf * p.K + sw * 32; }
    const int row0 = ROWS ? (gg - b * p.S) * 32 : 0;
    unsigned am = 0u;
    constexpr bool C2ONE = NS == 4 && !ROWS;
    float s1 = 1.f, c2 = p.u2, c3 = C2ONE ? p.u3 * p.u2 : p.u3;
    float so = 1.f;
    float b1s_f = 1.f, b1s_x = 1.f, b1s_b = 1.f;
    const bool fform = fmode || (L1M && hasfeat);
    if constexpr (F16) {
        if (fform && p.feat_amax) {
            const float bnd = __fmaf_rn(p.w1f_norm, __uint_as_float(p.feat_amax[b]), p.b1_max) + p.w1x_norm * p.dmax;
            s1 = f16x2_scale(__float_as_uint(bnd));
            float s2 = f16x2_scale(__float_as_uint(__fmaf_rn(p.w2_norm, bnd, p.b2_max)));
            if constexpr (C2ONE) { s1 = fminf(s1, p.u2 * s2); s2 = s1 * pow2_inverse(p.u2); }
            c2 = p.u2 * s2 * pow2_inverse(s1);
            c3 = p.u3 * pow2_inverse(s2);
        } else if (!fform && p.p1_amax) {
            float a1 = __uint_as_float(p.p1_amax[b]);
            if constexpr (DIRECT) {
                if (NS == 4 && p.t_bf16) s1 = p.row16_scale[b];
                else { s1 = f16x2_scale(p.p1_amax[b]); a1 *= s1; }
            }
            else s1 = p.p1_scale[b];
            const float inv_s1 = pow2_inverse(s1);
            const float bh1 = a1 + s1 * (p.w1x_norm * p.dmax);
            const float bh2 = __fmaf_rn(p.w2_norm, bh1 * inv_s1, p.b2_max);
            float s2 = f16x2_scale(__float_as_uint(bh2));
            c2 = p.u2 * s2 * inv_s1;
            c3 = p.u3 * pow2_inverse(s2);
            if constexpr (C2ONE) {
                s2 = s1 * pow2_inverse(p.u2);
                c3 = (s2 * bh2 <= 65504.f) ? p.u3 * pow2_inverse(s2) : __uint_as_float(0x7fc00000u);
            }
        }
        s1 = __uint_as_float(__builtin_amdgcn_readfirstlane(__float_as_uint(s1)));
        c2 = __uint_as_float(__builtin_amdgcn_readfirstlane(__float_as_uint(c2)));
        c3 = __uint_as_float(__builtin_amdgcn_readfirstlane(__float_as_uint(c3)));
        if constexpr (ROWS && NS == 4) {
            if (p.out_bf16) {
                const float bound2 = 32768.f * (c3 / p.u3);
                so = f16x2_scale(__float_as_uint(__fmaf_rn(p.w3_norm, bound2, p.b3_max)));
                so = __uint_as_float(__builtin_amdgcn_readfirstlane(__float_as_uint(so)));
                if (lane == 0 && valid && row0 == 0) p.row16_scale[b] = so;
            }
        }
        for (int i = lane; i < T2 * 32; i += 64) sbw[i] = sb2[i] * s1;
        if constexpr (L1F) {
            if (fmode) for (int i = lane; i < C1; i += 64) sb1w[i] = p.b1[i] * s1;
        }
        if constexpr (L1M) { b1s_f = s1 * p.a1f; b1s_x = s1 * p.a1x; b1s_b = s1 * p.a1b; }
    }
    int my_strips = ROWS ? 1 : p.K >> 5;
    if (!ROWS && p.cnt) my_strips = min(my_strips, max(1, (p.cnt[gf * p.cnt_ld] + 31) >> 5));
    if (spg > 1) my_strips = (valid && sw < my_strips) ? 1 : 0;
    int nstrips = my_strips;
    if constexpr (!RES && !ROWS) {
        int* s_strips = reinterpret_cast<int*>(smem + WBYTES + Cfg::W1B + T2 * 32 * 4);
        if (tid == 0) *s_strips = 1;
        __syncthreads();
        if (lane == 0) atomicMax(s_strips, my_strips);
        __syncthreads();
        nstrips = *s_strips;
    }

#ifdef EV2H_SAB_TIMELINE
    const bool dbgw = (blockIdx.x == 300 && tid == 0);
    const int dbg_strip = nstrips > 1 ? 1 : 0;
#endif
    constexpr bool XPF = !ROWS && NS != 3;
    f32x4 raw[4];
    int idx_cur = 0, idx_nxt = 0;
    float4 q_cur = make_float4(0.f, 0.f, 0.f, 0.f), f0_cur = q_cur, f1_cur = q_cur;
    if constexpr (XPF) {
        idx_cur = gi[l31];
        q_cur = p.pts4[(size_t)b * p.Npts + idx_cur];
        if (hasfeat) {
            const float4* fr = reinterpret_cast<const float4*>(p.feat + ((size_t)b * p.Npts + idx_cur) * p.ldf);
            f0_cur = fr[0]; f1_cur = fr[1];
        }
    }
    for (int strip = 0; strip < nstrips; ++strip) {
        STAMP(0);
        if constexpr (!RES) {
            if (strip >= my_strips) {
                for (int c = 0; c < NC1; ++c) {
                    char* nxt = buf ? wt0 : wt1;
                    if (c % CPT == 0) { if (c + CPT < NC1) dma_w2(c / CPT + 1, nxt); else dma_w3(0, nxt); }
                    if (c % CPT == CPT - 1) { asm volatile("s_waitcnt vmcnt(0)" ::: "memory"); __syncthreads(); buf ^= 1; }
                }
                for (int u = 0; u < T3; ++u) {
                    char* nxt = buf ? wt0 : wt1;
                    if (u % UPT == 0) { if (u + UPT < T3) dma_w3(u / UPT + 1, nxt); else if (strip + 1 < nstrips) dma_w2(0, nxt); }
                    if (u % UPT == UPT - 1) { asm volatile("s_waitcnt vmcnt(0)" ::: "memory"); __syncthreads(); buf ^= 1; }
                }
                continue;
            }
        }
        float dx = 0.f, dy = 0.f, dz = 0.f;
        auto qi = [&](int j4) { return 2 * j4 + half; };
        const float4* prow = nullptr;
        const float4* trow[3] = {nullptr, nullptr, nullptr};
        float tw[3] = {0.f, 0.f, 0.f};
        u32x4 b1f = {0u, 0u, 0u, 0u};
        u32x4 b1g = {0u, 0u, 0u, 0u};
        float cj = 1.f;
        f32x4 trw[ROWS ? 3 : 1][4];
        auto fetch = [&](int c) {
#pragma unroll
            for (int j = 0; j < ((ROWS && !DIRECT) ? 3 : 1); ++j)
#pragma unroll
                for (int j4 = 0; j4 < 4; ++j4) {
                    if constexpr ((NS == 1 || NS == 4) && DIRECT) {
                        if (p.t_bf16) {
                            const uint2 h = *reinterpret_cast<const uint2*>(reinterpret_cast<const char*>(trow[j]) + (size_t)(c * 32 + 4 * qi(j4)) * 2);
                            if constexpr (NS == 1) {
                                trw[j][j4] = f32x4{__uint_as_float(h.x << 16), __uint_as_float(h.x & 0xffff0000u), __uint_as_float(h.y << 16),
                                                   __uint_as_float(h.y & 0xffff0000u)};
                            } else {
                                const f16x2 a = __builtin_bit_cast(f16x2, h.x), b_ = __builtin_bit_cast(f16x2, h.y);
                                trw[j][j4] = f32x4{(float)a[0], (float)a[1], (float)b_[0], (float)b_[1]};
                            }
                            continue;
                        }
                    }
                    trw[j][j4] = *reinterpret_cast<const f32x4*>(trow[j] + c * 8 + qi(j4));
                }
        };
        auto blend = [&]() {
#pragma unroll
            for (int j4 = 0; j4 < 4; ++j4)
#pragma unroll
                for (int e = 0; e < 4; ++e)
                    raw[j4][e] = DIRECT ? ((F16 && !(NS == 4 && p.t_bf16)) ? trw[0][j4][e] * s1 : trw[0][j4][e])
                                        : __fmaf_rn(tw[2], trw[ROWS ? 2 : 0][j4][e], __fmaf_rn(tw[1], trw[ROWS ? 1 : 0][j4][e], __fmul_rn(tw[0], trw[0][j4][e])));
        };
        if constexpr (DIRECT) {
            trow[0] = ((NS == 1 || NS == 4) && p.t_bf16)
                          ? reinterpret_cast<const float4*>(reinterpret_cast<const char*>(p.P1) + ((size_t)b * p.N + min(row0 + l31, p.N - 1)) * p.ldp * 2)
                          : reinterpret_cast<const float4*>(p.P1 + ((size_t)b * p.N + min(row0 + l31, p.N - 1)) * p.ldp);
            fetch(0);
            blend();
        } else if constexpr (ROWS) {
            const size_t gr = ((size_t)b * p.N + min(row0 + l31, p.N - 1)) * 3;
#pragma unroll
            for (int j = 0; j < 3; ++j) {
                trow[j] = reinterpret_cast<const float4*>(p.P1 + ((size_t)b * p.Npts + p.nn_idx[gr + j]) * p.ldp);
                tw[j] = p.nn_w[gr + j];
            }
            fetch(0);
            blend();
        } else {
            const int idx = XPF ? idx_cur : gi[strip * 32 + l31];
            const float4 q = XPF ? q_cur : p.pts4[(size_t)b * p.Npts + idx];
            if constexpr (XPF) idx_nxt = (strip + 1 < my_strips) ? gi[(strip + 1) * 32 + l31] : idx_cur;
            dx = __fsub_rn(q.x, ctr.x); dy = __fsub_rn(q.y, ctr.y); dz = __fsub_rn(q.z, ctr.z);
            if constexpr (F16 && !L1M) { if (!fmode) { dx *= s1; dy *= s1; dz *= s1; } }
            if (fmode) {
                if constexpr (L1F && NS == 3) {
                    const float4* fr = reinterpret_cast<const float4*>(p.feat + ((size_t)b * p.Npts + idx) * p.ldf);
                    const float4 fa = fr[0], fb = fr[1];
                    const float v[8] = {fa.x, fa.y, fa.z, fa.w, fb.x, dx, dy, dz};
#pragma unroll
                    for (int w = 0; w < 4; ++w) {
                        unsigned o[3];
                        split_planes<3>(v[2 * w], v[2 * w + 1], o);
                        b1f[w] = half ? o[1] : o[0];
                        b1g[w] = half ? o[2] : o[0];
                    }
                }
                if constexpr (L1F && F16) {
                    float v[8] = {f0_cur.x, f0_cur.y, f0_cur.z, f0_cur.w, f1_cur.x, dx, dy, dz};
                    const float af = fmaxf(fmaxf(fmaxf(fabsf(v[0]), fabsf(v[1])), fmaxf(fabsf(v[2]), fabsf(v[3]))), fabsf(v[4]));
                    const float ax = fmaxf(fmaxf(fabsf(v[5]), fabsf(v[6])), fabsf(v[7]));
                    const float kap = fminf(f16x2_scale(__float_as_uint(af)) * (1.f / p.u1f), f16x2_scale(__float_as_uint(ax)) * (1.f / p.u1x));
                    const float sgf = kap * p.u1f, sgx = kap * p.u1x;
                    cj = s1 * pow2_inverse(kap);
#pragma unroll
                    for (int j = 0; j < 5; ++j) v[j] *= sgf;
#pragma unroll
                    for (int j = 5; j < 8; ++j) v[j] *= sgx;
#pragma unroll
                    for (int w = 0; w < 4; ++w) {
                        unsigned o[2];
                        split_planes<2>(v[2 * w], v[2 * w + 1], o);
                        b1f[w] = half ? o[1] : o[0];
                    }
                }
            } else if constexpr (L1M) {
                float f[8];
#pragma unroll
                for (int j = 0; j < 8; ++j) f[j] = 0.f;
                if (hasfeat) {
                    f[0] = f0_cur.x; f[1] = f0_cur.y; f[2] = f0_cur.z; f[3] = f0_cur.w; f[4] = f1_cur.x;
                    if constexpr (F16) {
#pragma unroll
                        for (int j = 0; j < 5; ++j) f[j] *= b1s_f;
                    }
                } else {
                    prow = reinterpret_cast<const float4*>(p.P1 + ((size_t)b * p.Npts + idx) * p.ldp);
                    if (strip == 0) {
#pragma unroll
                        for (int j4 = 0; j4 < 4; ++j4) raw[j4] = *reinterpret_cast<const f32x4*>(prow + qi(j4));
                    }
                }
                auto lo_of = [](float x) {
                    if constexpr (F16) return x - (float)(_Float16)x;
                    else return x - __uint_as_float(__builtin_bit_cast(unsigned, __builtin_convertvector(f32x2{x, 0.f}, bf16x2)) << 16);
                };
                const float ex = F16 ? dx * b1s_x : dx, ey = F16 ? dy * b1s_x : dy, ez = F16 ? dz * b1s_x : dz;
                const float va[8] = {f[0], f[1], f[2], f[3], f[4], lo_of(ex), lo_of(ey), lo_of(ez)};
                const float vb[8] = {ex, ey, ez, F16 ? (hasfeat ? b1s_b : 0.f) : 1.f, lo_of(f[0]), lo_of(f[1]), lo_of(f[2]), lo_of(f[3])};
#pragma unroll
                for (int w = 0; w < 4; ++w) {
                    unsigned o[1];
                    split_planes<NS>(half ? vb[2 * w] : va[2 * w], half ? vb[2 * w + 1] : va[2 * w + 1], o);
                    b1f[w] = o[0];
                }
            } else {
                prow = reinterpret_cast<const float4*>(p.P1 + ((size_t)b * p.Npts + idx) * p.ldp);
                if (!XPF || strip == 0) {
#pragma unroll
                    for (int j4 = 0; j4 < 4; ++j4) raw[j4] = *reinterpret_cast<const f32x4*>(prow + qi(j4));
                }
            }
        }
        auto layer1 = [&](int c) {
            f32x16 acc;
            if constexpr (L1F && NS == 3) {
#pragma unroll
                for (int q = 0; q < 4; ++q) {
                    const f32x4 bv = *reinterpret_cast<const f32x4*>(sb1w + 32 * c + 8 * q + 4 * half);
#pragma unroll
                    for (int e = 0; e < 4; ++e) acc[4 * q + e] = bv[e];
                }
                const char* ar = smem + WBYTES + (32 * c + l31) * Cfg::RSA + half * 16;
                const u32x4 a0 = *reinterpret_cast<const u32x4*>(ar), a1 = *reinterpret_cast<const u32x4*>(ar + 32), a2 = *reinterpret_cast<const u32x4*>(ar + 64);
                acc = mfma_planes<3>(a2, b1g, acc);
                acc = mfma_planes<3>(a1, b1f, acc);
                return mfma_planes<3>(a0, b1f, acc);
            } else if constexpr (L1F) {
#pragma unroll
                for (int r = 0; r < 16; ++r) acc[r] = 0.f;
                const char* ar = smem + WBYTES + (32 * c + l31) * Cfg::RSA + half * 16;
                const u32x4 ah = *reinterpret_cast<const u32x4*>(ar), al = *reinterpret_cast<const u32x4*>(ar + 32);
                acc = mfma_planes<2>(al, b1f, acc);
                return mfma_planes<2>(ah, b1f, acc);
            } else {
            if (hasfeat) {
#pragma unroll
                for (int r = 0; r < 16; ++r) acc[r] = 0.f;
            } else {
#pragma unroll
                for (int r = 0; r < 16; ++r) acc[r] = raw[r >> 2][r & 3];
            }
            const u32x4 a1 = *reinterpret_cast<const u32x4*>(smem + WBYTES + (32 * c + l31) * 32 + half * 16);
            return mfma_planes<NS>(a1, b1f, acc);
            }
        };
        f32x16 d1;
        if constexpr (L1F) { if (fmode) d1 = layer1(0); }
        if constexpr (L1M) {
            d1 = layer1(0);
            if (!hasfeat && NC1 > 1) {
#pragma unroll
                for (int j4 = 0; j4 < 4; ++j4) raw[j4] = *reinterpret_cast<const f32x4*>(prow + 8 + qi(j4));
            }
        }

        f32x16 h2[T2];
#pragma unroll
        for (int t = 0; t < T2; ++t)
#pragma unroll
            for (int j = 0; j < 4; ++j) {
                const f32x4 bv = *reinterpret_cast<const f32x4*>(sbw + 32 * t + 8 * j + 4 * half);
#pragma unroll
                for (int e = 0; e < 4; ++e) h2[t][4 * j + e] = bv[e];
            }

#ifdef EV2H_SAB_TIMELINE
        if (dbgw && strip == dbg_strip) asm volatile("s_waitcnt vmcnt(0)" ::: "memory");
#endif
        STAMP(1);
        auto finish_slice = [&](int c, int j4, u32x4 (&bp)[2][NPL]) {
            if constexpr (L1M) {
#pragma unroll
                for (int w = 2 * j4; w < 2 * j4 + 2; ++w) {
                    unsigned o[1];
                    split_planes<NS>(d1[2 * w], d1[2 * w + 1], o);
                    bp[w >> 2][0][w & 3] = relu_pk_bf16(o[0]);
                }
            } else if (fmode) {
                if constexpr (L1F && NS == 3) {
                    const int q = j4;
                    unsigned lo[3], hi[3];
                    split_planes<3>(relu_bits(d1[4 * q]), relu_bits(d1[4 * q + 1]), lo);
                    split_planes<3>(relu_bits(d1[4 * q + 2]), relu_bits(d1[4 * q + 3]), hi);
#pragma unroll
                    for (int s_ = 0; s_ < 3; ++s_) {
                        bp[q >> 1][s_][(q & 1) * 2 + 0] = lo[s_];
                        bp[q >> 1][s_][(q & 1) * 2 + 1] = hi[s_];
                    }
                }
                if constexpr (L1F && F16) {
                    const int q = j4;
                    const f32x4 bv = *reinterpret_cast<const f32x4*>(sb1w + 32 * c + 8 * q + 4 * half);
                    unsigned lo[NPL], hi[NPL];
                    split_planes<NS>(relu_sat_f16(__fmaf_rn(d1[4 * q], cj, bv[0])), relu_sat_f16(__fmaf_rn(d1[4 * q + 1], cj, bv[1])), lo);
                    split_planes<NS>(relu_sat_f16(__fmaf_rn(d1[4 * q + 2], cj, bv[2])), relu_sat_f16(__fmaf_rn(d1[4 * q + 3], cj, bv[3])), hi);
#pragma unroll
                    for (int s_ = 0; s_ < NPL; ++s_) {
                        bp[q >> 1][s_][(q & 1) * 2 + 0] = lo[s_];
                        bp[q >> 1][s_][(q & 1) * 2 + 1] = hi[s_];
                    }
                }
            } else {
                const f32x4* wp = sW1xT + (8 * c + 2 * j4 + half) * 3;
                const f32x4 wx = wp[0], wy = wp[1], wz = wp[2];
                f32x4 v;
#pragma unroll
                for (int e = 0; e < 4; ++e)
                    v[e] = ROWS ? raw[j4][e] : __fmaf_rn(wz[e], dz, __fmaf_rn(wy[e], dy, __fmaf_rn(wx[e], dx, raw[j4][e])));
                unsigned lo[NPL], hi[NPL];
                if constexpr (DIRECT) {
                    split_planes<NS>(v[0], v[1], lo);
                    split_planes<NS>(v[2], v[3], hi);
                } else if constexpr (NS == 1) {
                    split_planes<NS>(v[0], v[1], lo);
                    split_planes<NS>(v[2], v[3], hi);
                    lo[0] = relu_pk_bf16(lo[0]); hi[0] = relu_pk_bf16(hi[0]);
                } else if constexpr (F16) {
                    split_planes<NS>(relu_sat_f16(v[0]), relu_sat_f16(v[1]), lo);
                    split_planes<NS>(relu_sat_f16(v[2]), relu_sat_f16(v[3]), hi);
                } else {
                    split_planes<NS>(relu_bits(v[0]), relu_bits(v[1]), lo);
                    split_planes<NS>(relu_bits(v[2]), relu_bits(v[3]), hi);
                }
#pragma unroll
                for (int s = 0; s < NPL; ++s) {
                    bp[j4 >> 1][s][(j4 & 1) * 2 + 0] = lo[s];
                    bp[j4 >> 1][s][(j4 & 1) * 2 + 1] = hi[s];
                }
            }
        };
        auto mfma_groups = [&](const char* cur, u32x4 (&bp)[2][NPL], auto&& between) {
            const char* pa = cur + l31 * RS2 + (16 * half) * 2;
            auto ld2 = [&](int pr, u32x4 (&x0)[NPL], u32x4 (&x1)[NPL]) {
                const int m0 = (2 * pr) / T2, t0 = (2 * pr) % T2, m1 = (2 * pr + 1) / T2, t1 = (2 * pr + 1) % T2;
#pragma unroll
                for (int s = 0; s < NPL; ++s) {
                    x0[s] = *reinterpret_cast<const u32x4*>(pa + 32 * t0 * RS2 + s * 64 + m0 * 16);
                    x1[s] = *reinterpret_cast<const u32x4*>(pa + 32 * t1 * RS2 + s * 64 + m1 * 16);
                }
            };
            u32x4 fa[2][2][NPL];
            if constexpr (FRAG_PIPE) ld2(0, fa[0][0], fa[0][1]);
#pragma unroll
            for (int pr = 0; pr < T2; ++pr) {
                const int m0 = (2 * pr) / T2, t0 = (2 * pr) % T2, m1 = (2 * pr + 1) / T2, t1 = (2 * pr + 1) % T2;
                if constexpr (FRAG_PIPE) {
                    if (pr + 1 < T2) ld2(pr + 1, fa[(pr + 1) & 1][0], fa[(pr + 1) & 1][1]);
                    __builtin_amdgcn_sched_barrier(0);
                } else {
                    ld2(pr, fa[pr & 1][0], fa[pr & 1][1]);
                }
                u32x4 (&a0)[NPL] = fa[pr & 1][0];
                u32x4 (&a1)[NPL] = fa[pr & 1][1];
#pragma unroll
                for (int j = 0; j < PL::NPROD; ++j) {
                    if (!(Cfg::PACK4 && t0 == T2 - 1 && PL::A[j] == 1)) h2[t0] = mfma_planes<NS>(a0[PL::A[j]], bp[m0][PL::B[j]], h2[t0]);
                    if (!(Cfg::PACK4 && t1 == T2 - 1 && PL::A[j] == 1)) h2[t1] = mfma_planes<NS>(a1[PL::A[j]], bp[m1][PL::B[j]], h2[t1]);
                }
                if constexpr (FRAG_PIPE) __builtin_amdgcn_sched_barrier(0);
                between(pr);
            }
        };
        auto l2_dma = [&](int c) {
            if constexpr (!RES) {
                char* nxt = buf ? wt0 : wt1;
                if (c % CPT == 0) { if (c + CPT < NC1) dma_w2(c / CPT + 1, nxt); else dma_w3(0, nxt); }
            }
        };
        auto l2_sync = [&](int c) {
            STAMP(4 + 4 * c);
            if constexpr (!RES) {
                if (c % CPT == CPT - 1) {
                    asm volatile("s_waitcnt vmcnt(0)" ::: "memory");
                    __syncthreads();
                    buf ^= 1;
                }
            }
            STAMP(5 + 4 * c);
        };
        u32x4 bpA[2][NPL];
        if constexpr (!L2PIPE) {
#pragma unroll 1
            for (int c = 0; c < NC1; ++c) {
                STAMP(2 + 4 * c);
                char* cur = RES ? smem + c * Cfg::TB2 : (buf ? wt1 : wt0) + (c % CPT) * Cfg::TB2;
                l2_dma(c);
#pragma unroll
                for (int j4 = 0; j4 < 4; ++j4) finish_slice(c, j4, bpA);
                if constexpr (ROWS) {
                    if (c + 1 < NC1) fetch(c + 1);
                } else if (!L1M && !fmode && c + 1 < NC1) {
#pragma unroll
                    for (int j4 = 0; j4 < 4; ++j4) raw[j4] = *reinterpret_cast<const f32x4*>(prow + (c + 1) * 8 + qi(j4));
                }
                STAMP(3 + 4 * c);
                mfma_groups(cur, bpA, [](int) {});
                if constexpr (ROWS) {
                    if (c + 1 < NC1) blend();
                }
                if constexpr (L1F) {
                    if (fmode && c + 1 < NC1) d1 = layer1(c + 1);
                }
                if constexpr (L1M) {
                    if (c + 1 < NC1) {
                        d1 = layer1(c + 1);
                        if (!hasfeat && c + 2 < NC1) {
#pragma unroll
                            for (int j4 = 0; j4 < 4; ++j4) raw[j4] = *reinterpret_cast<const f32x4*>(prow + (c + 2) * 8 + qi(j4));
                        }
                    }
                }
                l2_sync(c);
            }
        } else {
            u32x4 bpB[2][NPL];
            const bool vtab = !L1M && !fmode;
#pragma unroll
            for (int j4 = 0; j4 < 4; ++j4) {
                finish_slice(0, j4, bpA);
                if (vtab) raw[j4] = *reinterpret_cast<const f32x4*>(prow + 8 + qi(j4));
            }
            auto l2_step = [&](int c, u32x4 (&bc)[2][NPL], u32x4 (&bn)[2][NPL]) {
                STAMP(2 + 4 * c);
                char* cur = RES ? smem + c * Cfg::TB2 : (buf ? wt1 : wt0) + (c % CPT) * Cfg::TB2;
                l2_dma(c);
                const bool more = c + 1 < NC1;
                if (more) {
                    if constexpr (L1F) { if (fmode) d1 = layer1(c + 1); }
                    if constexpr (L1M) {
                        d1 = layer1(c + 1);
                        if (!hasfeat && c + 2 < NC1) {
#pragma unroll
                            for (int j4 = 0; j4 < 4; ++j4) raw[j4] = *reinterpret_cast<const f32x4*>(prow + (c + 2) * 8 + qi(j4));
                        }
                    }
                }
                STAMP(3 + 4 * c);
                mfma_groups(cur, bc, [&](int pr) {
                    if (more) {
#pragma unroll
                        for (int j4 = 0; j4 < 4; ++j4) {
                            if (j4 * T2 / 4 == pr) {
                                __builtin_amdgcn_sched_barrier(0);
                                finish_slice(c + 1, j4, bn);
                                if (vtab && c + 2 < NC1) raw[j4] = *reinterpret_cast<const f32x4*>(prow + (c + 2) * 8 + qi(j4));
                                __builtin_amdgcn_sched_barrier(0);
                            }
                        }
                    }
                });
                l2_sync(c);
            };
#pragma unroll 1
            for (int c = 0; c < NC1; c += 2) {
                l2_step(c, bpA, bpB);
                l2_step(c + 1, bpB, bpA);
            }
        }

        STAMP(38);
        if constexpr (XPF) {
            if (strip + 1 < my_strips) {
                q_cur = p.pts4[(size_t)b * p.Npts + idx_nxt];
                if (hasfeat) {
                    const float4* fr = reinterpret_cast<const float4*>(p.feat + ((size_t)b * p.Npts + idx_nxt) * p.ldf);
                    f0_cur = fr[0]; f1_cur = fr[1];
                } else {
                    const float4* pn = reinterpret_cast<const float4*>(p.P1 + ((size_t)b * p.Npts + idx_nxt) * p.ldp);
#pragma unroll
                    for (int j4 = 0; j4 < 4; ++j4) raw[j4] = *reinterpret_cast<const f32x4*>(pn + qi(j4));
                }
                idx_cur = idx_nxt;
            }
        }
        if constexpr (Cfg::PACK4) {
#pragma unroll
            for (int r = 0; r < 4; ++r) { h2[T2 - 1][r] += h2[T2 - 1][r + 4]; h2[T2 - 1][r + 4] = 0.f; }
        }
        u32x4 h2p[NPL][T2][2];
        auto split_half = [&](int t, int m) {
#pragma unroll
            for (int k = 4 * m; k < 4 * m + 4; ++k) {
                unsigned o[NPL];
                if constexpr (C2ONE) {
                    split_planes<NS>(h2[t][2 * k], h2[t][2 * k + 1], o);
                    o[0] = relu_pk_bf16(o[0]);
                }
                else if constexpr (F16) split_planes<NS>(relu_sat_f16(h2[t][2 * k] * c2), relu_sat_f16(h2[t][2 * k + 1] * c2), o);
                else if constexpr (NS == 1) { split_planes<NS>(h2[t][2 * k], h2[t][2 * k + 1], o); o[0] = relu_pk_bf16(o[0]); }
                else split_planes<NS>(relu_bits(h2[t][2 * k] * c2), relu_bits(h2[t][2 * k + 1] * c2), o);
#pragma unroll
                for (int s = 0; s < NPL; ++s) h2p[s][t][k >> 2][k & 3] = o[s];
            }
            if constexpr (Cfg::PACK4) {
                if (t == T2 - 1 && m == 0) {
                    const unsigned h01 = h2p[0][T2 - 1][0][0], h23 = h2p[0][T2 - 1][0][1];
                    const unsigned l01 = h2p[1][T2 - 1][0][0], l23 = h2p[1][T2 - 1][0][1];
                    const unsigned ph01 = (unsigned)__shfl_xor((int)h01, 32, 64), ph23 = (unsigned)__shfl_xor((int)h23, 32, 64);
                    h2p[0][T2 - 1][0][0] = half ? ph01 : h01;
                    h2p[0][T2 - 1][0][1] = half ? ph23 : h23;
                    h2p[0][T2 - 1][0][2] = half ? 0u : l01;
                    h2p[0][T2 - 1][0][3] = half ? 0u : l23;
                }
            }
        };
#pragma unroll
        for (int t = 0; t < (H2FUSE ? 1 : T2); ++t) { split_half(t, 0); split_half(t, 1); }
        STAMP(39);

        auto finish_tile = [&](int u, const f32x16& acc) {
            float mx = fmaxf(fmaxf(acc[0], acc[1]), acc[2]);
#pragma unroll
            for (int r = 3; r < 15; r += 2) mx = fmaxf(fmaxf(mx, acc[r]), acc[r + 1]);
            mx = fmaxf(mx, acc[15]);
#pragma unroll
            for (int uu = 0; uu < T3; ++uu) mrun[uu] = (uu == u) ? fmaxf(mrun[uu], mx) : mrun[uu];
        };
        constexpr int TPS = (!ROWS && (RES || UPT == 2)) ? 2 : 1;
        static_assert(T3 % TPS == 0, "layer-3 tiles are walked in pairs");
        auto l3_step = [&](int u, auto first_tag) {
            constexpr bool FIRST = decltype(first_tag)::value;
            STAMP(40 + 4 * u);
            char* cur = RES ? smem + NC1 * Cfg::TB2 + u * Cfg::TB3 : (buf ? wt1 : wt0) + (u % UPT) * Cfg::TB3;
            char* nxt = buf ? wt0 : wt1;
            if constexpr (!RES) {
                if (u % UPT == 0) {
                    const bool more_w3 = (u + UPT < T3);
                    const bool more = more_w3 || (strip + 1 < nstrips);
                    if (more_w3) dma_w3(u / UPT + 1, nxt); else if (more) dma_w2(0, nxt);
                }
            }
            float b3u = 0.f;
            if constexpr (ROWS) b3u = p.b3[32 * u + l31];
            f32x16 acc, acc1;
#pragma unroll
            for (int r = 0; r < 16; ++r) { acc[r] = 0.f; acc1[r] = 0.f; }
            const char* pb = cur + l31 * RS3 + (8 * half) * 2;
            constexpr int NG3 = 2 * (T2 - 1) + Cfg::M_LAST;
            auto ld3 = [&](int g, u32x4 (&x)[NPL], u32x4 (&x1)[TPS == 2 ? NPL : 1]) {
#pragma unroll
                for (int s = 0; s < NPL; ++s) {
                    x[s] = *reinterpret_cast<const u32x4*>(pb + s * (C2P * 2) + (16 * g) * 2);
                    if constexpr (TPS == 2) x1[s] = *reinterpret_cast<const u32x4*>(pb + Cfg::TB3 + s * (C2P * 2) + (16 * g) * 2);
                }
            };
            u32x4 fw[2][NPL], fw1[2][TPS == 2 ? NPL : 1];
            if constexpr (FRAG_PIPE) ld3(0, fw[0], fw1[0]);
#pragma unroll
            for (int t = 0; t < T2; ++t) {
#pragma unroll
                for (int m = 0; m < 2; ++m) {
                    if (t < T2 - 1 || m < Cfg::M_LAST) {
                        const int g = 2 * t + m;
                        if constexpr (FRAG_PIPE) {
                            if (g + 1 < NG3) ld3(g + 1, fw[(g + 1) & 1], fw1[(g + 1) & 1]);
                            __builtin_amdgcn_sched_barrier(0);
                        } else {
                            ld3(g, fw[g & 1], fw1[g & 1]);
                        }
                        u32x4 a[NPL];
                        u32x4 (&w)[NPL] = fw[g & 1];
                        u32x4 (&w1)[TPS == 2 ? NPL : 1] = fw1[g & 1];
#pragma unroll
                        for (int s = 0; s < NPL; ++s) a[s] = h2p[s][t][m];
#pragma unroll
                        for (int j = 0; j < PL::NPROD; ++j) {
                            if (Cfg::PACK4 && t == T2 - 1 && !(PL::A[j] == 0 && PL::B[j] == 0)) continue;
                            if constexpr (TPS == 2) {
                                acc = mfma_planes<NS>(a[PL::A[j]], w[PL::B[j]], acc);
                                acc1 = mfma_planes<NS>(a[PL::A[j]], w1[PL::B[j]], acc1);
                            } else {
                                if (((2 * t + m) * PL::NPROD + j) & 1) acc1 = mfma_planes<NS>(a[PL::A[j]], w[PL::B[j]], acc1);
                                else acc = mfma_planes<NS>(a[PL::A[j]], w[PL::B[j]], acc);
                            }
                        }
                        if constexpr (FRAG_PIPE) __builtin_amdgcn_sched_barrier(0);
                        if constexpr (FIRST) {
                            if (t + 1 < T2) {
                                if constexpr (!FRAG_PIPE) __builtin_amdgcn_sched_barrier(0);
                                split_half(t + 1, m);
                                __builtin_amdgcn_sched_barrier(0);
                            }
                        }
                    }
                }
            }
            STAMP(41 + 4 * u);
            if constexpr (TPS == 2) {
                finish_tile(u, acc);
                finish_tile(u + 1, acc1);
            } else {
#pragma unroll
                for (int r = 0; r < 16; ++r) acc[r] += acc1[r];
                if constexpr (ROWS) {
                    float* orow = p.out + ((size_t)b * p.N + row0 + 4 * half) * p.ldo + 32 * u + l31;
                    const bool colok = valid && (32 * u + l31 < p.ncols);
                    float* ocm = p.out_cm ? p.out_cm + (size_t)b * p.out_cm_stride + (size_t)(32 * u + l31) * p.N + row0 + 4 * half : nullptr;
    #pragma unroll
                    for (int r = 0; r < 16; ++r) {
                        const int pt = 8 * (r >> 2) + (r & 3);
                        float o = acc[r] * c3 + b3u;
                        if (p.relu_out) o = fmaxf(o, 0.f);
                        if (colok && row0 + 4 * half + pt < p.N) {
                            if (NS == 1 && p.out_bf16) {
                                unsigned short* o16 = reinterpret_cast<unsigned short*>(p.out) + ((size_t)b * p.N + row0 + 4 * half + pt) * p.ldo + 32 * u + l31;
                                *o16 = (unsigned short)(__builtin_bit_cast(unsigned, __builtin_convertvector(f32x2{o, 0.f}, bf16x2)) & 0xffffu);
                            } else if (NS == 4 && p.out_bf16) {
                                o = fminf(o * so, 65504.f);
                                unsigned short* o16 = reinterpret_cast<unsigned short*>(p.out) + ((size_t)b * p.N + row0 + 4 * half + pt) * p.ldo + 32 * u + l31;
                                const _Float16 h16 = (_Float16)o;
                                *o16 = __builtin_bit_cast(unsigned short, h16);
                                o = (float)h16;
                            } else
                            orow[(size_t)pt * p.ldo] = o;
                            if (ocm) ocm[pt] = o;
                            am = max(am, abs_bits(o));
                        }
                    }
                } else {
                    finish_tile(u, acc);
                }
            }
            STAMP(42 + 4 * u);
            if constexpr (!RES) {
                if ((u + TPS - 1) % UPT == UPT - 1) {
                    asm volatile("s_waitcnt vmcnt(0)" ::: "memory");
                    __syncthreads();
                    buf ^= 1;
                }
            }
            STAMP(43 + 4 * u);
        };
        if constexpr (H2FUSE) l3_step(0, std::true_type{});
#pragma unroll 1
        for (int u = H2FUSE ? TPS : 0; u < T3; u += TPS) l3_step(u, std::false_type{});
        STAMP(37);
    }
    if constexpr (!ROWS && !RES) {
        if (spg > 1) {
            float* smax = reinterpret_cast<float*>(smem);
#pragma unroll
            for (int u = 0; u < T3; ++u) {
                const float v = fmaxf(mrun[u], __shfl_xor(mrun[u], 32, 64));
                if (half == 0) smax[wave * C3 + 32 * u + l31] = v;
            }
            __syncthreads();
            if (sw == 0) {
#pragma unroll
                for (int u = 0; u < T3; ++u) {
                    float v = smax[wave * C3 + 32 * u + l31];
                    for (int k = 1; k < spg; ++k) v = fmaxf(v, smax[(wave + k) * C3 + 32 * u + l31]);
                    mrun[u] = v;
                }
            }
        }
    }
    if constexpr (!ROWS) {
#pragma unroll
        for (int u = 0; u < T3; ++u) {
            const float v = fmaxf(mrun[u], __shfl_xor(mrun[u], 32, 64));
            if (valid && half == 0 && sw == 0) {
                float o = fmaxf(v * c3 + p.b3[32 * u + l31], 0.f);
                if constexpr (C2ONE) o = (c3 == c3) ? o : c3;
                p.out[gf * p.ldo + 32 * u + l31] = o;
                am = max(am, __float_as_uint(o));
            }
        }
    }
    if constexpr (!ROWS) {
        if (p.xyz_out && valid && sw == 0 && lane < 8)
            p.xyz_out[gf * p.xyz_ld + lane] = lane == 0 ? ctr.x : lane == 1 ? ctr.y : lane == 2 ? ctr.z : 0.f;
    }
    if constexpr (F16) {
        if (p.out_amax) {
            am = wave_max_u32_dpp(am);
            char* rec = smem + WBYTES + Cfg::SMALL_NOREC;
            if constexpr (RES) {
                if (lane == 0 && am) {
                    const int slot = b - (xcd * p.per_xcd) / p.S;
                    unsigned old = 0u;
                    if (slot >= 0 && slot < Cfg::REC_SLOTS) old = atomicMax(reinterpret_cast<unsigned*>(rec) + slot, am);
                    if (am > old) atomicMax(&p.out_amax[b], am);
                }
            } else {
                int* sb = reinterpret_cast<int*>(rec);
                unsigned* sa = reinterpret_cast<unsigned*>(rec + 32);
                if (lane == 0) { sb[wave] = (valid && am) ? b : -1; sa[wave] = am; }
                __syncthreads();
                if (lane == 0 && valid && am) {
                    bool first = true;
                    unsigned m = am;
#pragma unroll
                    for (int w = 0; w < WV; ++w) {
                        if (sb[w] == b) { first = first && w >= wave; m = max(m, sa[w]); }
                    }
                    if (first) atomicMax(&p.out_amax[b], m);
                }
            }
        }
    }
    if constexpr (!RES) break;
  }
}

template <int C1, int C2, int C3, int NS, int MODE = 0>
int launch_sab(SaBP p, hipStream_t st) {
    using Cfg = SaBCfg<C1, C2, C3, NS>;
    static const bool streamed_only = getenv("EV2H_SA_STREAMED") != nullptr;
    if constexpr (Cfg::FITS_RESIDENT) {
        if (!streamed_only) {
            static PerDevice wg_slot{};
            std::atomic<int>& wg = wg_slot.cur();
            int wg_per_cu = wg.load(std::memory_order_acquire);
            if (!wg_per_cu) {
                auto k = sa_mlp_max_bf16_kernel<C1, C2, C3, NS, true, MODE>;
                EV2H_CHECK_HIP(hipFuncSetAttribute(reinterpret_cast<const void*>(k), hipFuncAttributeMaxDynamicSharedMemorySize, Cfg::RES_LDS_BYTES));
                int n = 0;
                EV2H_CHECK_HIP(hipOccupancyMaxActiveBlocksPerMultiprocessor(&n, k, SAB_THREADS, Cfg::RES_LDS_BYTES));
                wg_per_cu = n > 0 ? n : 1;
                wg.store(wg_per_cu, std::memory_order_release);
            }
            const int ngroups = p.B * p.S;
            const int want = 256 * wg_per_cu;
            p.per_xcd = ceil_div(ceil_div(ngroups, 8), SAB_WAVES) * SAB_WAVES;
            p.nblk = 8 * std::min(want / 8, ceil_div(p.per_xcd, SAB_WAVES));
            sa_mlp_max_bf16_kernel<C1, C2, C3, NS, true, MODE><<<p.nblk, SAB_THREADS, Cfg::RES_LDS_BYTES, st>>>(p);
            EV2H_CHECK_LAUNCH();
            return EV2H_OK;
        }
    }
    static PerDevice attr_set{};
    EV2H_ONCE_PER_DEVICE(attr_set,
        EV2H_CHECK_HIP(hipFuncSetAttribute(reinterpret_cast<const void*>(sa_mlp_max_bf16_kernel<C1, C2, C3, NS, false, MODE>),
                                           hipFuncAttributeMaxDynamicSharedMemorySize, Cfg::LDS_BYTES)););
    {
        const int spg = p.K / 32;
        p.spg = 1;
        if ((spg == 2 || spg == 4) && p.nblk < 256 && SAB_WAVES * C3 * 4 <= 2 * Cfg::TILE) {
            p.spg = spg;
            p.nblk = ceil_div(p.B * p.S, SAB_WAVES / spg);
        }
    }
    sa_mlp_max_bf16_kernel<C1, C2, C3, NS, false, MODE><<<p.nblk, SAB_THREADS, Cfg::LDS_BYTES, st>>>(p);
    EV2H_CHECK_LAUNCH();
    return EV2H_OK;
}

template <int NS, int MODE = 0>
int dispatch_sab(const SaBP& p, int c1, int c2, int c3, hipStream_t st) {
    if constexpr (MODE == 0) {
        if (p.feat) return dispatch_sab<NS, 3>(p, c1, c2, c3, st);
    }
    if (c1 == 32 && c2 == 32 && c3 == 64) return launch_sab<32, 32, 64, NS, MODE>(p, st);
    if (c1 == 64 && c2 == 64 && c3 == 128) return launch_sab<64, 64, 128, NS, MODE>(p, st);
    if (c1 == 64 && c2 == 96 && c3 == 128) return launch_sab<64, 96, 128, NS, MODE>(p, st);
    if (c1 == 128 && c2 == 128 && c3 == 256) return launch_sab<128, 128, 256, NS, MODE>(p, st);
    if (c1 == 128 && c2 == 196 && c3 == 256) return launch_sab<128, 196, 256, NS, MODE>(p, st);
    ev2h_set_error("ev2h_sa_mlp_max: unsupported MLP widths %d-%d-%d", c1, c2, c3);
    return EV2H_ERR_ARG;
}

}

#ifdef EV2H_SAB_TIMELINE
extern "C" int ev2h_sab_timeline_read(long long* host) {
    return (int)hipMemcpyFromSymbol(host, HIP_SYMBOL(g_sab_timeline), sizeof(long long) * 256);
}
#endif
template <int C1, int C2, int C3, int NS, int MODE>
static int launch_fp(SaBP p, hipStream_t st) {
    using Cfg = SaBCfg<C1, C2, C3, NS>;
    auto k = sa_mlp_max_bf16_kernel<C1, C2, C3, NS, false, MODE>;
    static PerDevice attr_set{};
    EV2H_ONCE_PER_DEVICE(attr_set,
        EV2H_CHECK_HIP(hipFuncSetAttribute(reinterpret_cast<const void*>(k), hipFuncAttributeMaxDynamicSharedMemorySize, Cfg::LDS_BYTES)););
    k<<<p.nblk, SAB_THREADS, Cfg::LDS_BYTES, st>>>(p);
    EV2H_CHECK_LAUNCH();
    return EV2H_OK;
}

template <int NS>
static int dispatch_fp(const SaBP& p, const ev2h_fp_desc* d, hipStream_t st) {
    if (d->nn_idx && d->C1 == 128 && d->C2 == 128 && d->C3 == 256) return launch_fp<128, 128, 256, NS, 1>(p, st);
    if (!d->nn_idx && d->C1 == 256 && d->C2 == 256 && d->C3 == 32) return launch_fp<256, 256, 32, NS, 2>(p, st);
    ev2h_set_error("ev2h_fp_mlp: unsupported chain %d-%d-%d (%s)", d->C1, d->C2, d->C3, d->nn_idx ? "interpolated" : "plain rows");
    return EV2H_ERR_ARG;
}

int ev2h_gemm_tile_geometry(int ns, int out[2]);
namespace {
template <int C1, int C2, int C3, int NS>
int fill_geometry(int out[10]) {
    using Cfg = SaBCfg<C1, C2, C3, NS>;
    out[0] = Cfg::T2; out[1] = Cfg::C2P; out[2] = Cfg::RS2; out[3] = Cfg::RS3; out[4] = Cfg::TB2; out[5] = Cfg::TB3;
    out[8] = Cfg::PACK4 ? Cfg::REM : 0;
    out[9] = 1;
    return EV2H_OK;
}
template <int NS>
int geometry_ns(int c1, int c2, int c3, int out[10]) {
    if (c1 == 32 && c2 == 32 && c3 == 64) return fill_geometry<32, 32, 64, NS>(out);
    if (c1 == 64 && c2 == 64 && c3 == 128) return fill_geometry<64, 64, 128, NS>(out);
    if (c1 == 64 && c2 == 96 && c3 == 128) return fill_geometry<64, 96, 128, NS>(out);
    if (c1 == 128 && c2 == 128 && c3 == 256) return fill_geometry<128, 128, 256, NS>(out);
    if (c1 == 128 && c2 == 196 && c3 == 256) return fill_geometry<128, 196, 256, NS>(out);
    if (c1 == 256 && c2 == 256 && c3 == 32) return fill_geometry<256, 256, 32, NS>(out);
    return EV2H_ERR_ARG;
}
}

extern "C" int ev2h_tile_geometry(int C1, int C2, int C3, int planes, int out[10]) {
    EV2H_CHECK_ARG(out && planes >= 1 && planes <= 4);
    for (int i = 0; i < 10; ++i) out[i] = 0;
    const int rc = planes == 1 ? geometry_ns<1>(C1, C2, C3, out) : planes == 2 ? geometry_ns<2>(C1, C2, C3, out) : planes == 3 ? geometry_ns<3>(C1, C2, C3, out) : geometry_ns<4>(C1, C2, C3, out);
    if (rc) { ev2h_set_error("ev2h_tile_geometry: unsupported chain %d-%d-%d", C1, C2, C3); return rc; }
    return ev2h_gemm_tile_geometry(planes, out + 6);
}

int ev2h_fp_mlp_ex(const ev2h_fp_desc* d, int t_bf16, int out_bf16, ev2h_stream_t stream, float* row16_scale = nullptr, float w3_norm = 0.f, float b3_max = 0.f);
extern "C" int ev2h_fp_mlp(const ev2h_fp_desc* d, ev2h_stream_t stream) { return ev2h_fp_mlp_ex(d, 0, 0, stream); }

int ev2h_fp_mlp_ex(const ev2h_fp_desc* d, int t_bf16, int out_bf16, ev2h_stream_t stream, float* row16_scale, float w3_norm, float b3_max) {
    EV2H_CHECK_ARG(d && d->T && d->W2s && d->W3s && d->b2 && d->b3 && d->out);
    EV2H_CHECK_ARG(!(t_bf16 || out_bf16) || ((d->precision == EV2H_PREC_BF16 || (d->precision == EV2H_PREC_F16 && row16_scale && d->t_amax)) &&
                                             (!out_bf16 || !d->out_cm) && (!t_bf16 || !d->nn_idx)));
    EV2H_CHECK_ARG((d->nn_idx != nullptr) == (d->nn_w != nullptr));
    EV2H_CHECK_ARG(d->B > 0 && d->N > 0 && d->ldt >= d->C1 && (d->ldt % 4) == 0);
    const int ncols = d->out_cols > 0 ? d->out_cols : d->C3;
    EV2H_CHECK_ARG(ncols <= d->C3 && d->ldo >= ncols);
    if (d->nn_idx) EV2H_CHECK_ARG(d->S >= 3);
    SaBP p{};
    p.P1 = d->T; p.ldp = d->ldt; p.nn_idx = d->nn_idx; p.nn_w = d->nn_w; p.N = d->N;
    p.W2s = (const char*)d->W2s; p.b2 = d->b2; p.W3s = (const char*)d->W3s; p.b3 = d->b3;
    p.out = d->out; p.ldo = d->ldo; p.B = d->B; p.Npts = d->S; p.S = ceil_div(d->N, 32); p.K = 32;
    p.S_total = p.S; p.s_off = 0;
    p.ncols = ncols; p.relu_out = d->no_relu_out ? 0 : 1; p.out_cm = d->out_cm;
    p.t_bf16 = t_bf16; p.out_bf16 = out_bf16;
    p.row16_scale = row16_scale; p.w3_norm = w3_norm; p.b3_max = b3_max;
    p.out_cm_stride = d->out_cm_stride ? d->out_cm_stride : (size_t)ncols * d->N;
    p.u2 = d->w2_unscale > 0.f ? d->w2_unscale : 1.f; p.u3 = d->w3_unscale > 0.f ? d->w3_unscale : 1.f;
    p.nblk = ceil_div(d->B * p.S, SAB_WAVES);
    if (d->precision == EV2H_PREC_F16X2 || d->precision == EV2H_PREC_F16) {
        p.out_amax = d->out_amax;
        if (d->t_amax) {
            EV2H_CHECK_ARG(d->w2_norm >= 0.f && d->b2_max >= 0.f);
            EV2H_CHECK_ARG(d->nn_idx ? d->t_scale != nullptr : d->t_scale == nullptr);
            p.p1_scale = d->t_scale; p.p1_amax = d->t_amax; p.w1x_norm = 0.f; p.dmax = 1.f; p.w2_norm = d->w2_norm; p.b2_max = d->b2_max;
        }
    }
    hipStream_t st = (hipStream_t)stream;
    if (d->precision == EV2H_PREC_BF16X3) return dispatch_fp<3>(p, d, st);
    if (d->precision == EV2H_PREC_F16X2) return dispatch_fp<2>(p, d, st);
    if (d->precision == EV2H_PREC_BF16) return dispatch_fp<1>(p, d, st);
    if (d->precision == EV2H_PREC_F16) return dispatch_fp<4>(p, d, st);
    ev2h_set_error("ev2h_fp_mlp: precision %d is not a 16-bit plane mode (F32: ev2h_three_nn_interp + ev2h_gemm)", d->precision);
    return EV2H_ERR_ARG;
}

int ev2h_sa_mlp_max_bf16(const ev2h_sa_desc* d, ev2h_stream_t stream) {
    EV2H_CHECK_ARG(d->W2s && d->W3s);
    SaBP p{};
    p.P1 = d->P1; p.ldp = d->ldp; p.pts4 = (const float4*)d->pts4; p.ctr4 = (const float4*)d->ctr4; p.gidx = d->gidx;
    p.W1x = (const float4*)d->W1x; p.W2s = (const char*)d->W2s; p.b2 = d->b2; p.W3s = (const char*)d->W3s; p.b3 = d->b3;
    p.out = d->out; p.ldo = d->ldo; p.B = d->B; p.Npts = d->Npts; p.S = d->S; p.K = d->K;
    p.S_total = d->S_total > 0 ? d->S_total : d->S; p.s_off = d->s_off;
    EV2H_CHECK_ARG(p.s_off >= 0 && p.s_off + p.S <= p.S_total);
    p.cnt = d->cnt; p.cnt_ld = d->cnt_ld;
    p.xyz_out = d->xyz_out; p.xyz_ld = d->xyz_ld;
    p.u2 = d->w2_unscale > 0.f ? d->w2_unscale : 1.f; p.u3 = d->w3_unscale > 0.f ? d->w3_unscale : 1.f;
    p.nblk = ceil_div(d->B * d->S, SAB_WAVES);
    if (d->feat) {
        EV2H_CHECK_ARG(d->W1f && d->b1 && d->nfeat >= 0 && d->nfeat <= 5 &&
                       d->ldf >= 8 && (d->ldf % 4) == 0 && d->ldw1f >= d->nfeat);
        p.feat = d->feat; p.ldf = d->ldf; p.W1f = d->W1f; p.ldw1f = d->ldw1f; p.b1 = d->b1; p.nfeat = d->nfeat;
        p.u1f = d->w1f_unscale > 0.f ? d->w1f_unscale : 1.f;
        p.u1x = d->w1x_unscale > 0.f ? d->w1x_unscale : 1.f;
        if ((d->precision == EV2H_PREC_F16X2 || d->precision == EV2H_PREC_F16) && d->feat_amax) {
            EV2H_CHECK_ARG(d->dmax > 0.f && d->w1f_norm >= 0.f && d->b1_max >= 0.f && d->w1x_norm >= 0.f && d->w2_norm >= 0.f && d->b2_max >= 0.f);
            p.feat_amax = d->feat_amax; p.w1f_norm = d->w1f_norm; p.b1_max = d->b1_max;
            p.w1x_norm = d->w1x_norm; p.dmax = d->dmax; p.w2_norm = d->w2_norm; p.b2_max = d->b2_max;
        }
    } else {
        EV2H_CHECK_ARG(d->P1 != nullptr);
    }
    if (d->precision == EV2H_PREC_BF16) EV2H_CHECK_ARG(p.u2 == 1.f);
    if (d->precision == EV2H_PREC_F16X2 || d->precision == EV2H_PREC_F16) {
        p.out_amax = d->out_amax;
        if (d->p1_scale) {
            EV2H_CHECK_ARG(d->p1_amax && d->dmax > 0.f && d->w1x_norm >= 0.f && d->w2_norm >= 0.f && d->b2_max >= 0.f);
            p.p1_scale = d->p1_scale; p.p1_amax = d->p1_amax;
            p.w1x_norm = d->w1x_norm; p.dmax = d->dmax; p.w2_norm = d->w2_norm; p.b2_max = d->b2_max;
        }
    }
    p.a1f = p.a1x = p.a1b = 1.f;
    if (d->precision == EV2H_PREC_F16 && (p.feat_amax || p.p1_scale)) {
        auto pow2_below = [](float norm) { int e = 0; if (!(norm > 0.f) || !std::isfinite(norm)) return 1.f; (void)std::frexp(norm, &e); return std::ldexp(1.f, e - 1 - 8); };
        p.a1x = pow2_below(d->w1x_norm);
        if (d->feat) { p.a1f = pow2_below(d->w1f_norm); p.a1b = pow2_below(d->b1_max); }
    }
    hipStream_t st = (hipStream_t)stream;
    if (d->precision == EV2H_PREC_BF16X3) return dispatch_sab<3>(p, d->C1, d->C2, d->C3, st);
    if (d->precision == EV2H_PREC_F16X2) return dispatch_sab<2>(p, d->C1, d->C2, d->C3, st);
    if (d->precision == EV2H_PREC_BF16) return dispatch_sab<1>(p, d->C1, d->C2, d->C3, st);
    if (d->precision == EV2H_PREC_F16) return dispatch_sab<4>(p, d->C1, d->C2, d->C3, st);
    ev2h_set_error("ev2h_sa_mlp_max: unknown precision %d", d->precision);
    return EV2H_ERR_ARG;
}
```

### ev2hands_amd/csrc/workspace.hip

```cpp
#include <cstring>

#include "planes.hpp"
#include "workspace.hpp"

#define X(id, name, count) name,
static const char* const kWsNames[WS_COUNT] = {EV2H_WS_BUFFERS(X)};
#undef X
#define X(id, name) name,
static const char* const kRangeNames[R_COUNT] = {EV2H_RANGE_RECORDS(X)};
#undef X

thread_local int g_last_l0_bf16 = 0;

void build_layout(Layout& L, int B, int N) {
    const size_t R = (size_t)B * N;
    const size_t b = (size_t)B;
#define X(id, name, count) count,
    const size_t counts[WS_COUNT] = {EV2H_WS_BUFFERS(X)};
#undef X
    L.total = 0;
    for (int i = 0; i < WS_COUNT; ++i) {
        L.off[i] = L.total;
        L.count[i] = counts[i];
        L.total += (counts[i] * 4 + 255) / 256 * 256;
    }
}

static int find_name(const char* const* names, int n, const char* name) {
    for (int i = 0; i < n; ++i)
        if (!strcmp(names[i], name)) return i;
    return -1;
}

extern "C" size_t ev2h_workspace_bytes(int B, int N) {
    if (B <= 0 || N <= 0) return 0;
    Layout L;
    build_layout(L, B, N);
    return L.total;
}

extern "C" const void* ev2h_workspace_buffer(void* workspace, int B, int N, const char* name, size_t* count) {
    if (!workspace || !name || B <= 0 || N <= 0) return nullptr;
    Layout L;
    build_layout(L, B, N);
    if (!strncmp(name, "rng.", 4)) {
        const int r = find_name(kRangeNames, R_COUNT, name + 4);
        if (r < 0) return nullptr;
        if (count) *count = (size_t)B;
        return static_cast<char*>(workspace) + L.off[WS_RANGES] + (size_t)r * B * 4;
    }
    const int id = find_name(kWsNames, WS_COUNT, name);
    if (id < 0) return nullptr;
    if (count) *count = L.count[id];
    return static_cast<char*>(workspace) + L.off[id];
}

extern "C" const void* ev2h_workspace_buffer_ex(void* workspace, int B, int N, const char* name, size_t* count, int* elem_type) {
    const void* p = ev2h_workspace_buffer(workspace, B, N, name, count);
    if (elem_type) *elem_type = (p && !strcmp(name, "l0")) ? g_last_l0_bf16 : 0;
    return p;
}

struct SpreadEntry { const char* name; WsId buf; int rows; int ld; int col0; int ncols; int rec; int rec2; size_t hand_off; };
constexpr int EV2H_MAX_SPREAD = 32;

static int spread_entries(SpreadEntry* e) {
    int n = 0;
    e[n++] = {"feat", WS_FEAT8, 0, 8, 0, 8, R_FEAT, -1, 0};
    e[n++] = {"l1", WS_L1CAT, 512, 576, 0, 320, R_L1A, -1, 0};
    e[n++] = {"l1cat", WS_L1CAT, 512, 576, 0, 576, R_L1A, R_L1B, 0};
    e[n++] = {"l2", WS_L2BUF, 128, 520, 0, 515, R_L2, R_FEAT, 0};
    e[n++] = {"sa3h1", WS_SA3H1, 128, 256, 0, 256, R_SA3H1, -1, 0};
    e[n++] = {"sa3h2", WS_SA3H2, 128, 512, 0, 512, R_SA3H2, -1, 0};
    e[n++] = {"l3", WS_L3, 1, 1024, 0, 1024, R_L3, -1, 0};
    e[n++] = {"fp3h", WS_FP3H, 128, 256, 0, 256, R_FP3H, -1, 0};
    e[n++] = {"fp3o", WS_FP3O, 128, 256, 0, 256, R_FP3O, -1, 0};
    e[n++] = {"fp2h", WS_FP2H, 512, 256, 0, 256, R_FP2H, -1, 0};
    e[n++] = {"l1new", WS_L1NEW, 512, 128, 0, 128, R_L1NEW, -1, 0};
    e[n++] = {"l0", WS_L0, 0, 256, 0, 256, R_L0, -1, 0};
    for (int h = 0; h < 2; ++h) {
        e[n++] = {h ? "hfR" : "hfL", WS_HF8, 0, 8, 0, 8, R_HF + h, -1, (size_t)h};
        e[n++] = {h ? "m1R" : "m1L", hand(WS_M1BUF_L, h), 128, 520, 0, 515, R_M1 + h, R_FEAT, 0};
        e[n++] = {h ? "msa2hR" : "msa2hL", hand(WS_MSA2H_L, h), 128, 256, 0, 256, R_MSA2H + h, -1, 0};
        e[n++] = {h ? "m2R" : "m2L", hand(WS_M2_L, h), 1, 512, 0, 512, R_M2 + h, -1, 0};
        e[n++] = {h ? "fc1R" : "fc1L", hand(WS_FC1_L, h), 1, 1024, 0, 1024, R_FC1 + h, -1, 0};
    }
    return n;
}

namespace {
__global__ __launch_bounds__(256) void spread_count_kernel(const float* __restrict__ buf, size_t window_stride, int rows, int ld, int col0, int ncols,
                                                           const unsigned* __restrict__ rec, const unsigned* __restrict__ rec2,
                                                           unsigned* __restrict__ counts, int half_elems) {
    const int b = blockIdx.y;
    unsigned a = rec[b];
    if (rec2) a = max(a, rec2[b]);
    const float s = f16x2_scale(a);
    const float* base = buf + (size_t)b * window_stride;
    const size_t total = (size_t)rows * ncols;
    unsigned nz = 0, lo = 0, hi = 0;
    for (size_t i = (size_t)blockIdx.x * 256 + threadIdx.x; i < total; i += (size_t)gridDim.x * 256) {
        const size_t r = i / ncols;
        const int c = (int)(i - r * ncols);
        const float v = fabsf(half_elems ? (float)reinterpret_cast<const _Float16*>(buf)[(size_t)b * window_stride + r * ld + col0 + c] : base[r * ld + col0 + c]) * s;
        nz += v > 0.f;
        lo += v > 0.f && v < 0.125f;
        hi += v > 0.f && v < 6.103515625e-05f;
    }
    nz = (unsigned)wave_sum_f32((float)nz); lo = (unsigned)wave_sum_f32((float)lo); hi = (unsigned)wave_sum_f32((float)hi);
    if ((threadIdx.x & 63) == 0) {
        atomicAdd(&counts[(size_t)b * 3 + 0], nz);
        atomicAdd(&counts[(size_t)b * 3 + 1], lo);
        atomicAdd(&counts[(size_t)b * 3 + 2], hi);
    }
}
}

extern "C" int ev2h_range_report_entries(const char** names, int max_names) {
    SpreadEntry e[EV2H_MAX_SPREAD];
    const int n = spread_entries(e);
    for (int i = 0; i < n && names && i < max_names; ++i) names[i] = e[i].name;
    return n;
}

extern "C" int ev2h_range_report(void* workspace, int B, int N, uint32_t* counts, ev2h_stream_t st) {
    EV2H_CHECK_ARG(workspace && counts && B > 0 && N >= 128 && N <= 32768);
    Ws ws;
    ws.base = static_cast<char*>(workspace);
    ws.B = B;
    ws.ranges_on = true;
    build_layout(ws.L, B, N);
    SpreadEntry e[EV2H_MAX_SPREAD];
    const int n = spread_entries(e);
    EV2H_CHECK_HIP(hipMemsetAsync(counts, 0, (size_t)n * B * 3 * sizeof(uint32_t), (hipStream_t)st));
    for (int i = 0; i < n; ++i) {
        const int rows = e[i].rows ? e[i].rows : N;
        const float* p = ws.f(e[i].buf) + e[i].hand_off * (size_t)B * N * 8;
        const size_t per_window = (size_t)rows * e[i].ld;
        const int gx = (int)std::min<size_t>(64, ((size_t)rows * e[i].ncols + 4095) / 4096);
        spread_count_kernel<<<dim3(std::max(gx, 1), B), 256, 0, (hipStream_t)st>>>(p, per_window, rows, e[i].ld, e[i].col0, e[i].ncols, ws.r(e[i].rec),
                                                                                  e[i].rec2 >= 0 ? ws.r(e[i].rec2) : nullptr, counts + (size_t)i * B * 3,
                                                                                  (e[i].buf == WS_L0 && g_last_l0_bf16 == 2) ? 1 : 0);
        EV2H_CHECK_LAUNCH();
    }
    return EV2H_OK;
}
```

### ev2hands_amd/model.py

```python
from __future__ import annotations

import ctypes as C
import math
import os

import numpy as np
import torch
import torch.nn as nn

from . import _lib, synth
from .mano import ManoHand, ManoOutput, create_mano_layers
from .pack import PackedWeights


class _MsgParams(nn.Module):

    def __init__(self, fan_in, mlps):
        super().__init__()
        self.conv_blocks = nn.ModuleList()
        self.bn_blocks = nn.ModuleList()
        for mlp in mlps:
            convs, bns, last = nn.ModuleList(), nn.ModuleList(), fan_in
            for o in mlp:
                convs.append(nn.Conv2d(last, o, 1))
# ... 68 lines not shown
        self._key_tensors = None
        self._key_gen = 0
        self._faces_cache = {}
        self._ws = None
        self.fps_init = None

    def _key_list(self):
        ts = self._key_tensors
        self._key_calls = getattr(self, "_key_calls", 0) + 1
        if ts is not None and self._key_calls % 64 == 0:
            fresh = list(self.parameters()) + list(self.buffers())
            if len(fresh) != len(ts) or any(a is not b for a, b in zip(fresh, ts)):
                ts = None
        if ts is None:
            ts = self._key_tensors = list(self.parameters()) + list(self.buffers())
            self._key_gen += 1
        return ts

    def _pack_key(self):
        ts = self._key_list()
        return (str(ts[0].device), self._key_gen, [t.data_ptr() for t in ts], [t._version for t in ts])

    def _version_key(self):
        ts = self._key_list()
        return (self._key_gen, [t._version for t in ts], [t.data_ptr() for t in ts])

    def _apply(self, fn, *args, **kwargs):
        self._key_tensors = None
        return super()._apply(fn, *args, **kwargs)

    def load_state_dict(self, *args, **kwargs):
        self._key_tensors = None
        return super().load_state_dict(*args, **kwargs)

    def __setattr__(self, name, value):
        if isinstance(value, (nn.Parameter, nn.Module)):
            self.__dict__["_key_tensors"] = None
        super().__setattr__(name, value)

    AUTO_TOLERANCE = 5e-5

    def effective_precision(self) -> str:
        if self.precision != "auto":
            return self.precision
        return self._auto[1] if self._auto is not None else "f16x2"

    def packed(self, device) -> PackedWeights:
        prec = self.effective_precision()
        key = (str(device), prec, self.equalize, self.f16_families, self._pack_key())
        if self._packed is None or self._packed_key != key:
            spare = getattr(self, "_packed_spare", None)
            if spare is not None and spare[0] == key:
                self._packed_spare = (self._packed_key, self._packed) if self._keep_spare else None
                self._packed, self._packed_key = spare[1], key
                return self._packed
            if self._keep_spare and self._packed is not None:
                self._packed_spare = (self._packed_key, self._packed)
            else:
                self._packed_spare = None
                self._packed = None
            self._packed = PackedWeights(self.state_dict(), device, self.in_channels, prec, equalize=self.equalize, f16_families=self.f16_families)
            self._packed_key = key
        return self._packed

    def workspace(self, nbytes: int, device) -> torch.Tensor:
        if self._ws is None or self._ws.numel() < nbytes or self._ws.device != torch.device(device):
            self._ws = None
            self._ws = torch.empty(nbytes, dtype=torch.uint8, device=device)
        return self._ws

    def draw_fps_init(self, B: int, N: int):
        return [torch.randint(0, hi, (B,), dtype=torch.long) for hi in (N, synth.SA1_NPOINT, N, N)]

    @staticmethod
    def seeded_fps_init(seed: int, window_ids: torch.Tensor, N: int, out: torch.Tensor | None = None) -> torch.Tensor:
        B = int(window_ids.shape[0])
        if window_ids.dtype != torch.int32 or not window_ids.is_cuda or not window_ids.is_contiguous() or window_ids.dim() != 1:
            raise ValueError("window_ids must be a contiguous int32 device tensor [B]")
        if not 0 <= int(seed) < 2 ** 64:
            raise ValueError("seed must be an unsigned 64-bit integer")
        if out is None:
            out = torch.empty(4, B, dtype=torch.long, device=window_ids.device)
        elif tuple(out.shape) != (4, B) or out.dtype != torch.long or not out.is_contiguous():
            raise ValueError(f"out must be a contiguous int64 [4, {B}] tensor")
        if B:
            _lib.check(_lib.lib().ev2h_fps_init_seeded(int(seed), window_ids.data_ptr(), B, int(N), synth.SA1_NPOINT, out.data_ptr(),
                                                       _lib.stream_handle()), "ev2h_fps_init_seeded")
        return out

    @staticmethod
    def _inits_to_device(inits, device) -> torch.Tensor:
        if torch.is_tensor(inits):
            st = inits.to(torch.long)
        else:
            st = torch.stack([t.to(torch.long) for t in inits])
        if st.device.type == "cpu":
            pin = torch.empty(st.shape, dtype=torch.long, pin_memory=True)
            pin.copy_(st)
            return pin.to(device, non_blocking=True)
        return st.to(device, non_blocking=True).contiguous()

    def _check_input(self, xyz):
        if self.training:
            raise NotImplementedError("ev2hands_amd implements the inference forward (net.eval()) only")
        if xyz.dim() != 3 or xyz.shape[1] != self.in_channels:
            raise RuntimeError(f"expected input [B, {self.in_channels}, N], got {tuple(xyz.shape)}")
        if not xyz.is_cuda:
            raise RuntimeError("ev2hands_amd runs on the GPU only (there is no CPU fallback); move the input to cuda")
        if xyz.dtype != torch.float32:
            raise RuntimeError("input must be float32")
        if self.mhlnes and not xyz.is_contiguous():
            raise RuntimeError("MHLNES=1 writes channel 2 in place and needs a contiguous input")

    def _enqueue(self, x, init_dev, mano_hands, rows=None, ws=None):
        device = x.device
        B, Cin, N = x.shape
        L = _lib.lib()
        pw = self.packed(device)
        native = {s: isinstance(mano_hands[s], ManoHand) for s in ("left", "right")}
        consts = {s: (C.byref(mano_hands[s].consts()) if native[s] else None) for s in ("left", "right")}

        f32 = dict(device=device, dtype=torch.float32)
        out = _lib.Outputs()
        NP, NVF = 3 + self.n_pose_params + 10 + 3, synth.MANO_NV * 3
        if rows is None:
            logits = torch.empty(B, 4, N, **f32)
            params = [torch.empty(B, NP, **f32) for _ in range(2)]
            verts = [torch.empty(B, synth.MANO_NV, 3, **f32) for _ in range(2)]
            joints = [torch.empty(B, 21, 3, **f32) for _ in range(2)]
        else:
            W = rows.shape[1] if rows.dim() == 2 else 0
            per_hand = NP + NVF + 63
            if (rows.dim() != 2 or rows.shape[0] != B or W < 4 * N + 2 * per_hand or rows.dtype != torch.float32 or rows.device != device
                    or rows.stride() != (W, 1)):
                raise RuntimeError(f"rows must be a float32 [B={B}, >= {4 * N + 2 * per_hand}] row-major matrix on {device}")
            logits = rows[:, :4 * N].view(B, 4, N)
            params, verts, joints = [], [], []
            for h in range(2):
                o = 4 * N + h * per_hand
                params.append(rows[:, o:o + NP])
                verts.append(rows[:, o + NP:o + NP + NVF].view(B, synth.MANO_NV, 3))
                joints.append(rows[:, o + NP + NVF:o + per_hand].view(B, 21, 3))
            out.logits_stride = out.params_stride = out.vertices_stride = out.joints_stride = W
        out.class_logits = logits.data_ptr()
        for h in range(2):
            out.params[h] = params[h].data_ptr()
            out.vertices[h] = verts[h].data_ptr()
            out.joints[h] = joints[h].data_ptr()
        nbytes = L.ev2h_workspace_bytes(B, N)
        if ws is None:
            ws = self.workspace(nbytes, device)
        elif ws.numel() < nbytes or ws.device != device:
            raise RuntimeError("workspace too small or on another device")
        with torch.cuda.device(device):
            _lib.check(L.ev2h_bind_stream(_lib.stream_handle(), None), "ev2h_bind_stream")
            _lib.check(L.ev2h_forward(C.byref(pw.struct), consts["left"], consts["right"], x.data_ptr(), B, Cin, N, self.mhlnes,
                                      init_dev.data_ptr(), C.byref(out), ws.data_ptr(), nbytes, _lib.stream_handle()),
                       "ev2h_forward")
        res = {"class_logits": logits}
        npose = self.n_pose_params
        for h, side in enumerate(("left", "right")):
            p = params[h]
            d = {"global_orient": p[:, :3], "hand_pose": p[:, 3:3 + npose], "betas": p[:, 3 + npose:-3], "transl": p[:, -3:]}
            if native[side]:
                d = {"vertices": verts[h], "j3d": joints[h], **d}
            else:
                hd = mano_hands[side].shapedirs.device
                d = {k: v.to(hd) for k, v in d.items()}
                o = mano_hands[side](**d)
                d = {"vertices": o.vertices, "j3d": o.joints, **d}
                if rows is not None:
                    verts[h].copy_(o.vertices.to(device))
                    joints[h].copy_(o.joints.to(device))
            res[side] = d
        self._last_shape = (B, N)
        self._last_ws = ws
        return res

    def range_report(self) -> dict:
        B, N = self._last_shape
        L = _lib.lib()
        names = (C.c_char_p * 64)()
        n = L.ev2h_range_report_entries(names, 64)
        ws = self._last_ws
        counts = torch.zeros(n, B, 3, dtype=torch.int32, device=ws.device)
        with torch.cuda.device(ws.device):
            _lib.check(L.ev2h_range_report(ws.data_ptr(), B, N, counts.data_ptr(), _lib.stream_handle()), "ev2h_range_report")
        c = counts.cpu().to(torch.int64)
        out = {}
        for i in range(n):
            nz, lo, hi = c[i, :, 0], c[i, :, 1], c[i, :, 2]
            out[names[i].decode()] = {"nonzero": nz, "below_2^-17": lo, "below_2^-28": hi,
                                      "worst_fraction": float((lo.double() / nz.clamp(min=1).double()).max())}
        return out

    def verify_precision(self, xyz, mano_hands, fps_init=None, reference: str = "bf16x3") -> dict:
        self._check_input(xyz)
        B, _, N = xyz.shape
        inits = fps_init if fps_init is not None else (self.fps_init if self.fps_init is not None else self.draw_fps_init(B, N))
        keep = self.precision
        outs = {}
        try:
            for prec in ("f16x2", reference):
                self.precision = prec
                self.fps_init = inits
                x = xyz.clone() if self.mhlnes else xyz
                with torch.no_grad():
                    o = self.forward(x, mano_hands)
                outs[prec] = {"class_logits": o["class_logits"].clone(),
                              **{f"{s}.{k}": o[s][k].clone() for s in ("left", "right") for k in ("global_orient", "hand_pose", "betas", "transl", "vertices", "j3d")}}
                if prec == "f16x2":
                    rng = self.range_report()
                    wsp = self._packed.weight_spread()
        finally:
            self.precision = keep
            self.fps_init = None
        a, b = outs["f16x2"], outs[reference]
        per = {k: float((a[k] - b[k]).abs().max() / b[k].abs().max().clamp(min=1e-30)) for k in a}
        agree = float((a["class_logits"].argmax(1) == b["class_logits"].argmax(1)).float().mean())
        nzw = sum(v[0] for v in wsp.values())
        rep = {"max_rel": max(per.values()), "per_output": per, "argmax_agreement": agree, "reference": reference, "range": rng,
               "range_worst": max(rng.items(), key=lambda kv: kv[1]["worst_fraction"])[0] if rng else None,
               "weights": {"nonzero": nzw, "below_2^-17": sum(v[1] for v in wsp.values())}}
        rep["ok"] = bool(rep["max_rel"] <= self.AUTO_TOLERANCE and agree == 1.0)
        return rep

    def _auto_decide(self, xyz, mano_hands, inits):
        key = (str(xyz.device), self.equalize, self._pack_key())
        if self._auto is not None and self._auto[0] == key:
            return
        self._auto = None
        self.precision = "f16x2"
        self._keep_spare = True
        try:
            rep = self.verify_precision(xyz, mano_hands, fps_init=inits)
        finally:
            self.precision = "auto"
            self._keep_spare = False
        ok = bool(rep["ok"])
        rep["ok_this_rank"] = ok
        try:
            import torch.distributed as tdist
            if tdist.is_available() and tdist.is_initialized() and tdist.get_world_size() > 1:
                from .dist import _group_moves_device_memory
                t = torch.tensor([1 if ok else 0], dtype=torch.int32, device=xyz.device if _group_moves_device_memory(None) else "cpu")
                tdist.all_reduce(t, op=tdist.ReduceOp.MIN)
                ok = bool(int(t.item()))
                rep["ranks"] = tdist.get_world_size()
        except ImportError:
            pass
        rep["ok"] = ok
        self._auto = (key, "f16x2" if ok else "bf16x3", rep)
        want = (str(xyz.device), self._auto[1], self.equalize, self.f16_families, self._pack_key())
        if self._packed_key != want and self._packed_spare is not None and self._packed_spare[0] == want:
            self._packed, self._packed_key = self._packed_spare[1], want
        self._packed_spare = None

    @property
    def auto_report(self):
        return None if self._auto is None else self._auto[2]

    def forward(self, xyz, mano_hands, rows=None, ws=None):
        self._check_input(xyz)
        device = xyz.device
        B, Cin, N = xyz.shape
        x = xyz if self.mhlnes else xyz.contiguous()
        inits = self.fps_init if self.fps_init is not None else self.draw_fps_init(B, N)
        self.fps_init = None
        if self.precision == "auto":
            self._auto_decide(xyz, mano_hands, inits)
        init_dev = self._inits_to_device(inits, device)
        res = self._enqueue(x, init_dev, mano_hands, rows=rows, ws=ws)
        for side in ("left", "right"):
            res[side]["faces"] = self._tiled_faces(mano_hands[side], B)
        return res

    def _tiled_faces(self, hand, B: int):
        key = (id(hand), id(hand.faces), B)
        hit = self._faces_cache.get(key)
        if hit is None:
            if len(self._faces_cache) > 8:
                self._faces_cache.clear()
            tiled = np.tile(hand.faces, (B, 1, 1))
            tiled.flags.writeable = False
            hit = self._faces_cache[key] = (tiled, hand, hand.faces)
        return hit[0]

    def capture(self, xyz, mano_hands, fps_init=None) -> "CapturedForward":
        self._check_input(xyz)
        if not all(isinstance(mano_hands[s], ManoHand) for s in ("left", "right")):
            raise TypeError("capture needs hand models from ev2hands_amd.create_mano_layers (foreign hand models run host code)")
        return CapturedForward(self, xyz, mano_hands, fps_init)

    def debug_buffer(self, name: str, dtype=torch.float32) -> torch.Tensor:
        B, N = self._last_shape
        L = _lib.lib()
        cnt = C.c_size_t(0)
        ws = self._last_ws
        et = C.c_int(0)
        p = L.ev2h_workspace_buffer_ex(ws.data_ptr(), B, N, name.encode(), C.byref(cnt), C.byref(et))
        if not p:
            raise KeyError(name)
        off = p - ws.data_ptr()
        if et.value in (1, 2):
            if dtype != torch.float32:
                raise TypeError(f"workspace buffer {name!r} holds {'bf16' if et.value == 1 else 'fp16'} values in this mode: ask for float32")
            if et.value == 1:
                return ws[off:off + cnt.value * 2].view(torch.bfloat16).float()
            v = ws[off:off + cnt.value * 2].view(torch.float16).float().view(B, -1)
            return (v / self.debug_buffer("p1scale").view(6, B)[5].view(B, 1)).view(-1)
        return ws[off:off + cnt.value * 4].view(dtype).clone()


class CapturedForward:

    def __init__(self, net: TEHNet, xyz, mano_hands, fps_init=None):
        device = xyz.device
        B, _, N = xyz.shape
        self.net, self.hands, self.B, self.N = net, mano_hands, B, N
        self.x = xyz.detach().clone().contiguous()
        inits = fps_init if fps_init is not None else net.draw_fps_init(B, N)
        self.init = torch.stack([t.to(torch.long) for t in inits]).to(device).contiguous()
        self._ws = torch.empty(_lib.lib().ev2h_workspace_bytes(B, N), dtype=torch.uint8, device=device)
        if net.precision == "auto":
            net._auto_decide(self.x, mano_hands, [t.cpu() for t in self.init])
        self._pw = net.packed(device)
        self._key = (net.effective_precision(), net.equalize, net._version_key())
        for s in ("left", "right"):
            mano_hands[s].consts()
        self._mano_keep = {s: (mano_hands[s]._keep, mano_hands[s].shapedirs._version) for s in ("left", "right")}
        with torch.no_grad():
            net._enqueue(self.x, self.init, mano_hands, ws=self._ws)
            torch.cuda.synchronize(device)
            self.graph = torch.cuda.CUDAGraph()
            with torch.cuda.graph(self.graph):
                self.out = net._enqueue(self.x, self.init, mano_hands, ws=self._ws)
        self.faces = {s: np.tile(mano_hands[s].faces, (B, 1, 1)) for s in ("left", "right")}
        for s in ("left", "right"):
            self.faces[s].flags.writeable = False
            self.out[s]["faces"] = self.faces[s]
        if net.mhlnes:
            self.x.copy_(xyz)

    def replay(self, xyz=None, fps_init=None) -> dict:
        if (self.net.effective_precision(), self.net.equalize, self.net._version_key()) != self._key:
            raise RuntimeError("the network's parameters, device or precision changed since this forward was captured: the graph "
                               "holds the old packed weights -- capture again")
        if any(self.hands[s].shapedirs._version != self._mano_keep[s][1] for s in ("left", "right")):
            raise RuntimeError("a hand model's shapedirs changed since this forward was captured -- capture again")
        if xyz is not None:
            if tuple(xyz.shape) != tuple(self.x.shape):
                raise RuntimeError(f"captured for input {tuple(self.x.shape)}, got {tuple(xyz.shape)}")
            self.x.copy_(xyz, non_blocking=True)
        if fps_init is not None:
            self.init.copy_(TEHNet._inits_to_device(fps_init, self.init.device), non_blocking=True)
        elif xyz is not None:
            self.init.copy_(TEHNet._inits_to_device(self.net.draw_fps_init(self.B, self.N), self.init.device), non_blocking=True)
        self.graph.replay()
        if self.net.mhlnes and xyz is not None:
            xyz[:, 2].copy_(self.x[:, 2])
        return self.out


def _rotation_x_180() -> torch.Tensor:
    c, s = math.cos(math.pi), math.sin(math.pi)
    return torch.tensor([[1.0, 0.0, 0.0, 0.0], [0.0, c, -s, 0.0], [0.0, s, c, 0.0], [0.0, 0.0, 0.0, 1.0]],
                        dtype=torch.float64)


class TEHNetWrapper:

    def __init__(self, device, mano_path="../data/models", mano_assets=None, precision=None, n_pose_params=None):
        n_pose = synth.MANO_CMPS if n_pose_params is None else int(n_pose_params)
        self.net = TEHNet(n_pose_params=n_pose).to(device)
        if precision is not None:
            self.net.precision = precision
        self.net.eval()
        self.training = False
        if torch.device(device).type == "cuda":
            with torch.cuda.device(device):
                _lib.check(_lib.lib().ev2h_init(), "ev2h_init")
        self.hands = create_mano_layers(mano_path, device, n_pose, assets=mano_assets)
        self.rot = _rotation_x_180().to(device).float()

    def state_dict(self):
        return self.net.state_dict()

    def load_state_dict(self, params, *args, **kwargs):
        stripped = {(k[len("module."):] if k.startswith("module.") else k): v for k, v in params.items()}
        w = stripped.get("sa1.conv_blocks.0.0.weight")
        if w is not None and w.dim() == 4 and int(w.shape[1]) - 3 != self.net.in_channels:
            c = int(w.shape[1]) - 3
            raise RuntimeError(f"checkpoint expects {c} input channels (trained with ERPC={int(c == 5)}) but this model was built for "
                               f"{self.net.in_channels} (ERPC={os.getenv('ERPC', '0')} when it was constructed): set ERPC={int(c == 5)} "
                               f"before creating TEHNetWrapper (the reference reads it at construction, TEHNet.py:122)")
        return self.net.load_state_dict(stripped, *args, **kwargs)

    def parameters(self):
        return self.net.parameters()

    def train(self):
        self.training = True
        return self.net.train()

    def eval(self):
        self.training = False
        return self.net.eval()

    def P3dtoP2d(self, j3d, scale, translation):
        B, N = j3d.shape[:2]
        h = torch.cat([j3d, torch.ones(B, N, 1, device=j3d.device)], 2) @ self.rot.detach()
        translation = translation.unsqueeze(1)
        scale = scale.unsqueeze(1)
        j2d = torch.zeros(B, N, 2, device=j3d.device)
        j2d[:, :, 0] = translation[:, :, 0] + scale[:, :, 0] * h[:, :, 0]
        j2d[:, :, 1] = translation[:, :, 1] + scale[:, :, 1] * h[:, :, 1]
        return j2d

    def __call__(self, inp):
        return self.net(inp, self.hands)

    def capture(self, inp, fps_init=None):
        return self.net.capture(inp, self.hands, fps_init)
```

Measured before the change: 21880 event-windows/s.

## Store L0 activations as pre-split fp16 plane pairs in f16x2 mode

```diff
diff --git a/ev2hands_amd/csrc/attention.hip b/ev2hands_amd/csrc/attention.hip
--- a/ev2hands_amd/csrc/attention.hip
+++ b/ev2hands_amd/csrc/attention.hip
@@ -166,7 +166,7 @@
         for (int c = 0; c < 4; ++c) {
             float4 t = *reinterpret_cast<const float4*>(sim + (((size_t)b * 2 + h) * 4 + c) * ATT_D + lane * 4);
             t.x *= vu.x; t.y *= vu.y; t.z *= vu.z; t.w *= vu.w;
-            if constexpr (VBF16 == 2) {
+            if constexpr (VBF16 == 2 || VBF16 == 3) {
                 const float iv = 1.f / vscale[b];
                 t.x *= iv; t.y *= iv; t.z *= iv; t.w *= iv;
             }
@@ -185,6 +185,13 @@
             const uint2 h = *reinterpret_cast<const uint2*>(reinterpret_cast<const unsigned short*>(value) + row * ldv + lane * 4);
             const h16x2 a = __builtin_bit_cast(h16x2, h.x), b_ = __builtin_bit_cast(h16x2, h.y);
             v = make_float4((float)a[0], (float)a[1], (float)b_[0], (float)b_[1]);
+        } else if constexpr (VBF16 == 3) {
+            typedef _Float16 h16x2 __attribute__((ext_vector_type(2)));
+            const char* rb = reinterpret_cast<const char*>(value) + (row * ldv) * 4 + (lane >> 3) * 128 + (lane & 7) * 8;
+            const uint2 h = *reinterpret_cast<const uint2*>(rb), l = *reinterpret_cast<const uint2*>(rb + 64);
+            const h16x2 a = __builtin_bit_cast(h16x2, h.x), b_ = __builtin_bit_cast(h16x2, h.y);
+            const h16x2 c = __builtin_bit_cast(h16x2, l.x), d_ = __builtin_bit_cast(h16x2, l.y);
+            v = make_float4((float)a[0] + (float)c[0], (float)a[1] + (float)c[1], (float)b_[0] + (float)d_[0], (float)b_[1] + (float)d_[1]);
         } else {
             v = *reinterpret_cast<const float4*>(value + row * ldv + lane * 4);
         }
@@ -288,3 +295,13 @@
     EV2H_CHECK_LAUNCH();
     return EV2H_OK;
 }
+
+int ev2h_attn_context_planes(const float* sim, const void* value_pm, int ldv, int B, int N, float* hf8, uint32_t* hf_amax, int amax_hand_stride,
+                             const float* value_unscale, const float* vscale, ev2h_stream_t stream) {
+    EV2H_CHECK_ARG(sim && value_pm && hf8 && vscale && B > 0 && N > 0 && ldv >= ATT_D && (ldv % 4) == 0);
+    dim3 grid(ceil_div(N, 4 * CTX_PTS_PER_WAVE), B);
+    attn_context_kernel<3><<<grid, 256, 0, (hipStream_t)stream>>>(sim, reinterpret_cast<const float*>(value_pm), ldv, N, (size_t)B * N, hf8, hf_amax, amax_hand_stride,
+                                                                 value_unscale, vscale);
+    EV2H_CHECK_LAUNCH();
+    return EV2H_OK;
+}
diff --git a/ev2hands_amd/csrc/forward.hip b/ev2hands_amd/csrc/forward.hip
--- a/ev2hands_amd/csrc/forward.hip
+++ b/ev2hands_amd/csrc/forward.hip
@@ -92,10 +92,13 @@
                           const int* nsample, int32_t* const* gidx, int32_t* cnt, ev2h_stream_t stream);
 bool ev2h_gemm_bf16_zsum_supported(const ev2h_gemm_desc* d);
 int ev2h_gemm_bf16_zsum(const ev2h_gemm_desc* d, const float* key_pm, float* zpart, int x_bf16, ev2h_stream_t stream, const float* x_scale = nullptr);
+int ev2h_gemm_bf16_tap3_planes(const ev2h_gemm_desc* d, const float* x_scale, ev2h_stream_t stream);
 int ev2h_fp_mlp_ex(const ev2h_fp_desc* d, int t_bf16, int out_bf16, ev2h_stream_t stream, float* row16_scale = nullptr, float w3_norm = 0.f, float b3_max = 0.f);
 int ev2h_attn_context_f16rows(const float* sim, const void* value_pm, int ldv, int B, int N, float* hf8, uint32_t* hf_amax, int amax_hand_stride,
                               const float* value_unscale, const float* vscale, ev2h_stream_t stream);
 int ev2h_attn_context_bf16rows(const float* sim, const void* value_pm, int ldv, int B, int N, float* hf8, const float* value_unscale, ev2h_stream_t stream);
+int ev2h_attn_context_planes(const float* sim, const void* value_pm, int ldv, int B, int N, float* hf8, uint32_t* hf_amax, int amax_hand_stride,
+                             const float* value_unscale, const float* vscale, ev2h_stream_t stream);
 int ev2h_attn_simfold_partials(const float* zpart, int rows_per_partial, const float* logits_pm, int B, int N, const float* w4t_left,
                                const float* w4t_right, const float* b4_left, const float* b4_right, float* sim, ev2h_stream_t stream);
 
@@ -364,11 +367,14 @@
     const bool cls_fused = prec != EV2H_PREC_F32 && w->clsm.W2s && !unfused_cls;
     const ev2h_gemm_desc qd = dense_desc(cx, w->qconv0, ws.f(WS_L0), 256, R, ws.f(WS_Q1), 512, 1, rg(R_L0, N),
                                          {.taps = 3, .rows_per_seq = N, .fam = EV2H_FAM_QCONV});
-    const bool zsum_ok = !unfused_zsum && prec != EV2H_PREC_F32 && w->qconv0.Ws && ev2h_gemm_bf16_zsum_supported(&qd);
+    const bool tap_shape = prec != EV2H_PREC_F32 && w->qconv0.Ws && ev2h_gemm_bf16_zsum_supported(&qd);
+    const bool zsum_ok = !unfused_zsum && tap_shape;
     const bool l0_bf16 = prec == EV2H_PREC_BF16 && fp1_fused && cls_fused && zsum_ok && !l0_f32;
     const bool l0_f16 = prec == EV2H_PREC_F16 && prec_rows == EV2H_PREC_F16 && prec_q == EV2H_PREC_F16 && ws.ranges_on && fp1_fused && cls_fused && zsum_ok && !l0_f32;
-    const bool l0_16 = l0_bf16 || l0_f16;
-    g_last_l0_bf16 = l0_bf16 ? 1 : (l0_f16 ? 2 : 0);
+    const bool l0_planes = prec == EV2H_PREC_F16X2 && prec_rows == EV2H_PREC_F16X2 && prec_q == EV2H_PREC_F16X2 && ws.ranges_on && fp1_fused && cls_fused && tap_shape && !l0_f32;
+    const bool l0_16 = l0_bf16 || l0_f16 || l0_planes;
+    const bool l0_scaled = l0_f16 || l0_planes;
+    g_last_l0_bf16 = l0_bf16 ? 1 : (l0_f16 ? 2 : (l0_planes ? 3 : 0));
     if (fp1_fused) {
         const ev2h_sa_module& m = w->fp1m;
         RUN(cx.wait_side(EV_FP1_NN));
@@ -382,7 +388,7 @@
             d.t_scale = ws.p1scale(4); d.t_amax = ws.r(R_FP1T); d.w2_norm = m.br[0].w2_norm; d.b2_max = m.br[0].b2_max; d.out_amax = ws.r(R_L0);
         }
         prof_begin("fp1", st);
-        RUN(ev2h_fp_mlp_ex(&d, 0, l0_16, st, l0_f16 ? ws.p1scale(5) : nullptr, m.br[0].w3_norm, m.br[0].b3_max));
+        RUN(ev2h_fp_mlp_ex(&d, 0, l0_16, st, l0_scaled ? ws.p1scale(5) : nullptr, m.br[0].w3_norm, m.br[0].b3_max));
         prof_end("fp1", st);
     } else {
         RUN(ev2h_three_nn_interp(ws.f(WS_PTS4), ws.f(WS_CTR1), B, N, 512, ws.f(WS_L1NEW), 128, 128, ws.f(WS_FP1IN), 128,
@@ -400,7 +406,7 @@
         d.out = ws.f(WS_LOGITS_PM); d.ldo = 4; d.out_cols = 4; d.no_relu_out = 1; d.out_cm = out->class_logits; d.out_cm_stride = out->logits_stride;
         d.B = B; d.N = N; d.C1 = c.C1; d.C2 = c.C2; d.C3 = c.C3; d.precision = prec_rows;
         if (ws.ranges_on) { d.t_amax = ws.r(R_L0); d.w2_norm = c.w2_norm; d.b2_max = c.b2_max; }
-        RUN(ev2h_fp_mlp_ex(&d, l0_16, 0, sd, l0_f16 ? ws.p1scale(5) : nullptr));
+        RUN(ev2h_fp_mlp_ex(&d, l0_16, 0, sd, l0_scaled ? ws.p1scale(5) : nullptr));
     } else {
         RUN(dense(cx, w->cls0, ws.f(WS_L0), 256, R, ws.f(WS_CLSH), 256, 1, sd, rg(R_L0, N, R_CLSH, N)));
         RUN(dense(cx, w->cls4, ws.f(WS_CLSH), 256, R, ws.f(WS_LOGITS_PM), 4, 0, sd, rg(R_CLSH, N)));
@@ -410,11 +416,12 @@
     if (zsum_ok) {
         RUN(cx.wait_side(EV_LOGITS));
         prof_begin("qconv0", st);
-        RUN(ev2h_gemm_bf16_zsum(&qd, ws.f(WS_LOGITS_PM), ws.f(WS_ZPART), l0_16, st, l0_f16 ? ws.p1scale(5) : nullptr));
+        RUN(ev2h_gemm_bf16_zsum(&qd, ws.f(WS_LOGITS_PM), ws.f(WS_ZPART), l0_16, st, l0_scaled ? ws.p1scale(5) : nullptr));
         prof_end("qconv0", st);
     } else {
         prof_begin("qconv0", st);
-        RUN(ev2h_gemm(&qd, st));
+        if (l0_planes) RUN(ev2h_gemm_bf16_tap3_planes(&qd, ws.p1scale(5), st));
+        else RUN(ev2h_gemm(&qd, st));
         prof_end("qconv0", st);
     }
     RUN(cx.wait_side(EV_LOGITS));
@@ -427,6 +434,7 @@
     }
     if (l0_bf16) RUN(ev2h_attn_context_bf16rows(ws.f(WS_SIM), ws.f(WS_L0), 256, B, N, ws.f(WS_HF8), w->l0_unscale, st));
     else if (l0_f16) RUN(ev2h_attn_context_f16rows(ws.f(WS_SIM), ws.f(WS_L0), 256, B, N, ws.f(WS_HF8), ws.r(R_HF), B, w->l0_unscale, ws.p1scale(5), st));
+    else if (l0_planes) RUN(ev2h_attn_context_planes(ws.f(WS_SIM), ws.f(WS_L0), 256, B, N, ws.f(WS_HF8), ws.r(R_HF), B, w->l0_unscale, ws.p1scale(5), st));
     else RUN(ev2h_attn_context(ws.f(WS_SIM), ws.f(WS_L0), 256, B, N, ws.f(WS_HF8), ws.r(R_HF), B, w->l0_unscale, st));
     RUN(cx.wait_side(EV_HAND_QUERIES));
     RUN(cx.signal_side(EV_HF8));
diff --git a/ev2hands_amd/csrc/gemm_bf16.hip b/ev2hands_amd/csrc/gemm_bf16.hip
--- a/ev2hands_amd/csrc/gemm_bf16.hip
+++ b/ev2hands_amd/csrc/gemm_bf16.hip
@@ -775,6 +775,129 @@
         EV2H_CHECK_HIP(hipFuncSetAttribute(reinterpret_cast<const void*>(gemm_nt_bf16_occ_kernel<NS, TAP3, false, ZS>),
                                            hipFuncAttributeMaxDynamicSharedMemorySize, GOCfg<NS, TAP3>::LDS_BYTES)););
     gemm_nt_bf16_occ_kernel<NS, TAP3, false, ZS><<<p.nblk, GO_THREADS, GOCfg<NS, TAP3>::LDS_BYTES, st>>>(p, Ws);
+    EV2H_CHECK_LAUNCH();
+    return EV2H_OK;
+}
+
+struct GPCfg {
+    static constexpr int ARS = 128;
+    static constexpr int A_ROWS = GB_BM + 2;
+    static constexpr int A_BYTES = A_ROWS * ARS;
+    static constexpr int A_PIECES = (A_BYTES + 1023) / 1024;
+    static constexpr int BRS = GBCfg<2>::RS;
+    static constexpr int B_BYTES = GO_BN * BRS;
+    static constexpr int LDS_BYTES = A_BYTES + 2 * B_BYTES;
+};
+static_assert(GPCfg::A_BYTES % 256 == 0, "the W tiles start on a bank row");
+static_assert(3 * GPCfg::LDS_BYTES <= 160 * 1024, "three workgroups per CU");
+
+template <bool ZS>
+__global__ __launch_bounds__(GO_THREADS, 3) void gemm_tap3_planes_kernel(GemmBP p, const char* __restrict__ Ws) {
+    using Cfg = GPCfg;
+    extern __shared__ __attribute__((aligned(16))) char smem[];
+    char* const sA = smem;
+    char* const sB0 = smem + Cfg::A_BYTES;
+
+    const int L = xcd_remap(blockIdx.x, p.nblk);
+    const int tn = L % p.tiles_n, tm = L / p.tiles_n;
+    const int m0 = tm * GB_BM, n0 = tn * GO_BN;
+    const int tid = threadIdx.x, lane = tid & 63;
+    const int wave = __builtin_amdgcn_readfirstlane(tid >> 6);
+    const int wm = wave >> 1, wn = wave & 1;
+    const int half = lane >> 5, l31 = lane & 31;
+    const int nkc = p.Kc / GB_BK, nk = 3 * nkc;
+    const int pos0 = m0 % p.rows_per_seq;
+    const bool zlo = pos0 == 0, zhi = pos0 + GB_BM == p.rows_per_seq;
+    if (zlo && tid < 8) *reinterpret_cast<u32x4*>(sA + tid * 16) = u32x4{0u, 0u, 0u, 0u};
+    if (zhi && tid >= 8 && tid < 16) *reinterpret_cast<u32x4*>(sA + (GB_BM + 1) * Cfg::ARS + (tid - 8) * 16) = u32x4{0u, 0u, 0u, 0u};
+
+    const size_t ldxb = (size_t)p.ldx * 4;
+    const int jl = lane >> 3;
+    const int pc = (lane & 7) ^ ((wave & 1) * 4 + (jl >> 1));
+    const char* const xlane = reinterpret_cast<const char*>(p.X) + ((long)m0 - 1 + jl) * (long)ldxb + pc * 16;
+    auto dma_a = [&](int kc) {
+        for (int i = wave; i < Cfg::A_PIECES; i += 4) {
+            const int j = i * 8 + jl;
+            const bool on = j < Cfg::A_ROWS && !(j == 0 && zlo) && !(j == GB_BM + 1 && zhi);
+            if (on)
+                __builtin_amdgcn_global_load_lds((const __attribute__((address_space(1))) void*)(xlane + (size_t)i * 8 * ldxb + kc * 128),
+                                                 (__attribute__((address_space(3))) void*)(sA + i * 1024), 16, 0, 0);
+        }
+    };
+    auto dma_b = [&](int kt, char* dst) {
+        const char* src = Ws + ((size_t)tn * nk + kt) * Cfg::B_BYTES;
+        for (int off = wave * 1024; off < Cfg::B_BYTES; off += 4 * 1024)
+            __builtin_amdgcn_global_load_lds((const __attribute__((address_space(1))) void*)(src + off + lane * 16),
+                                             (__attribute__((address_space(3))) void*)(dst + off), 16, 0, 0);
+    };
+    static_assert(Cfg::B_BYTES % 1024 == 0, "B tile image must be a whole number of 1 KiB DMA pieces");
+
+    f32x16 acc[2][2];
+#pragma unroll
+    for (int i = 0; i < 2; ++i)
+#pragma unroll
+        for (int j = 0; j < 2; ++j)
+#pragma unroll
+            for (int r = 0; r < 16; ++r) acc[i][j][r] = 0.f;
+
+    auto mma_tile = [&](int arow, const char* sB) {
+        const int r0 = wm * 64 + l31 + arow;
+        const char* pa = sA + r0 * Cfg::ARS;
+        const int sw = (half ^ ((r0 >> 1) & 7)) << 4;
+        const char* pb = sB + (wn * 64 + l31) * Cfg::BRS + half * 16;
+#pragma unroll
+        for (int m = 0; m < 2; ++m) {
+            u32x4 a[2][2], b[2][2];
+#pragma unroll
+            for (int s = 0; s < 2; ++s) {
+                const int ao = sw ^ (s * 64 + m * 32);
+                a[0][s] = *reinterpret_cast<const u32x4*>(pa + ao);
+                a[1][s] = *reinterpret_cast<const u32x4*>(pa + 32 * Cfg::ARS + ao);
+                b[0][s] = *reinterpret_cast<const u32x4*>(pb + s * 64 + m * 32);
+                b[1][s] = *reinterpret_cast<const u32x4*>(pb + 32 * Cfg::BRS + s * 64 + m * 32);
+            }
+#pragma unroll
+            for (int q = 0; q < Planes<2>::NPROD; ++q)
+#pragma unroll
+                for (int i = 0; i < 2; ++i)
+#pragma unroll
+                    for (int j = 0; j < 2; ++j)
+                        acc[i][j] = mfma_planes<2>(a[i][Planes<2>::A[q]], b[j][Planes<2>::B[q]], acc[i][j]);
+        }
+        asm volatile("s_waitcnt lgkmcnt(0)" ::: "memory");
+    };
+
+    dma_b(0, sB0);
+    int t = 0;
+    for (int kc = 0; kc < nkc; ++kc) {
+        if (kc) __builtin_amdgcn_s_barrier();
+        dma_a(kc);
+#pragma unroll 1
+        for (int tap = 0; tap < 3; ++tap, ++t) {
+            __builtin_amdgcn_s_waitcnt(0x0070);
+            __builtin_amdgcn_s_barrier();
+            if (t + 1 < nk) {
+                const int tap1 = tap == 2 ? 0 : tap + 1, kc1 = tap == 2 ? kc + 1 : kc;
+                dma_b(tap1 * nkc + kc1, sB0 + ((t + 1) & 1) * Cfg::B_BYTES);
+            }
+            mma_tile(tap, sB0 + (t & 1) * Cfg::B_BYTES);
+        }
+    }
+    if constexpr (ZS) {
+        zsum_epilogue<2>(p, acc, m0, wm, wn, n0, smem, tid);
+    } else {
+        __builtin_amdgcn_s_barrier();
+        gemm_epilogue<2, 2, 2, false>(p, acc, m0, wm * 64, n0 + wn * 64, wm, wn * 64, GO_BN, reinterpret_cast<float*>(smem), tid);
+    }
+}
+
+template <bool ZS>
+int launch_tap3_planes(const GemmBP& p, const char* Ws, hipStream_t st) {
+    static PerDevice attr_set{};
+    EV2H_ONCE_PER_DEVICE(attr_set,
+        EV2H_CHECK_HIP(hipFuncSetAttribute(reinterpret_cast<const void*>(gemm_tap3_planes_kernel<ZS>),
+                                           hipFuncAttributeMaxDynamicSharedMemorySize, GPCfg::LDS_BYTES)););
+    gemm_tap3_planes_kernel<ZS><<<p.nblk, GO_THREADS, GPCfg::LDS_BYTES, st>>>(p, Ws);
     EV2H_CHECK_LAUNCH();
     return EV2H_OK;
 }
@@ -924,7 +1047,9 @@
 
 int ev2h_gemm_bf16_zsum(const ev2h_gemm_desc* d, const float* key_pm, float* zpart, int x_bf16, ev2h_stream_t stream, const float* x_scale) {
     EV2H_CHECK_ARG(d && key_pm && zpart && ev2h_gemm_bf16_zsum_supported(d));
-    EV2H_CHECK_ARG(!x_bf16 || d->precision == EV2H_PREC_BF16 || (d->precision == EV2H_PREC_F16 && x_scale && d->x_group_rows > 0));
+    const bool scaled16 = d->precision == EV2H_PREC_F16 || d->precision == EV2H_PREC_F16X2;
+    EV2H_CHECK_ARG(!x_bf16 || d->precision == EV2H_PREC_BF16 || (scaled16 && x_scale && d->x_group_rows > 0));
+    EV2H_CHECK_ARG(!(x_bf16 && d->precision == EV2H_PREC_F16X2) || (d->ldx >= d->K && d->x_group_rows % d->rows_per_seq == 0));
     GemmBP p{};
     p.X = d->X; p.ldx = d->ldx; p.W = d->W; p.ldw = d->ldw; p.Y = nullptr; p.ldy = 0;
     p.M = d->M; p.N = d->N; p.taps = 3; p.Kc = d->K; p.K = d->K * 3;
@@ -937,14 +1062,33 @@
     }
     p.zs_key = reinterpret_cast<const float4*>(key_pm); p.zs_out = zpart;
     p.x_bf16 = x_bf16;
-    if (x_bf16 && d->precision == EV2H_PREC_F16) { p.x_scale = x_scale; p.x_amax = p.x_amax2 = nullptr; p.x_group_rows = d->x_group_rows; }
+    if (x_bf16 && scaled16) { p.x_scale = x_scale; p.x_amax = p.x_amax2 = nullptr; p.x_group_rows = d->x_group_rows; }
     p.tiles_n = d->N / GO_BN;
     p.nblk = (d->M / GB_BM) * p.tiles_n;
+    if (d->precision == EV2H_PREC_F16X2 && x_bf16) return launch_tap3_planes<true>(p, (const char*)d->Ws, (hipStream_t)stream);
     if (d->precision == EV2H_PREC_F16X2) return launch_go_t<2, true, true>(p, (const char*)d->Ws, (hipStream_t)stream);
     if (d->precision == EV2H_PREC_BF16) return launch_go_t<1, true, true>(p, (const char*)d->Ws, (hipStream_t)stream);
     if (d->precision == EV2H_PREC_BF16X3) return launch_go_t<3, true, true>(p, (const char*)d->Ws, (hipStream_t)stream);
     if (d->precision == EV2H_PREC_F16) return launch_go_t<4, true, true>(p, (const char*)d->Ws, (hipStream_t)stream);
     return EV2H_ERR_ARG;
+}
+
+int ev2h_gemm_bf16_tap3_planes(const ev2h_gemm_desc* d, const float* x_scale, ev2h_stream_t stream) {
+    EV2H_CHECK_ARG(d && d->Y && x_scale && d->precision == EV2H_PREC_F16X2 && ev2h_gemm_bf16_zsum_supported(d));
+    EV2H_CHECK_ARG(d->x_amax && d->x_group_rows > 0 && d->x_group_rows % d->rows_per_seq == 0 && d->ldx >= d->K && d->ldy >= d->N);
+    EV2H_CHECK_ARG(!d->y_amax && !d->y_scale && d->rowmax_rows == 0 && d->bias_group_rows == 0);
+    GemmBP p{};
+    p.X = d->X; p.ldx = d->ldx; p.W = d->W; p.ldw = d->ldw; p.Y = d->Y; p.ldy = d->ldy;
+    p.M = d->M; p.N = d->N; p.taps = 3; p.Kc = d->K; p.K = d->K * 3;
+    p.rows_per_seq = d->rows_per_seq;
+    p.bias = d->bias; p.relu = d->relu; p.post_scale = d->post_scale; p.post_shift = d->post_shift;
+    p.w_unscale = d->w_unscale > 0.f ? d->w_unscale : 1.f;
+    p.x_amax = d->x_amax;
+    p.x_scale = x_scale; p.x_group_rows = d->x_group_rows; p.y_group_rows = 1;
+    p.x_bf16 = 1;
+    p.tiles_n = d->N / GO_BN;
+    p.nblk = (d->M / GB_BM) * p.tiles_n;
+    return launch_tap3_planes<false>(p, (const char*)d->Ws, (hipStream_t)stream);
 }
 
 int ev2h_gemm_bf16(const ev2h_gemm_desc* d, ev2h_stream_t stream) {
diff --git a/ev2hands_amd/csrc/sa_mlp_bf16.hip b/ev2hands_amd/csrc/sa_mlp_bf16.hip
--- a/ev2hands_amd/csrc/sa_mlp_bf16.hip
+++ b/ev2hands_amd/csrc/sa_mlp_bf16.hip
@@ -229,6 +229,7 @@
             float a1 = __uint_as_float(p.p1_amax[b]);
             if constexpr (DIRECT) {
                 if (NS == 4 && p.t_bf16) s1 = p.row16_scale[b];
+                else if (NS == 2 && p.t_bf16) { s1 = p.row16_scale[b]; a1 *= s1; }
                 else { s1 = f16x2_scale(p.p1_amax[b]); a1 *= s1; }
             }
             else s1 = p.p1_scale[b];
@@ -246,7 +247,7 @@
         s1 = __uint_as_float(__builtin_amdgcn_readfirstlane(__float_as_uint(s1)));
         c2 = __uint_as_float(__builtin_amdgcn_readfirstlane(__float_as_uint(c2)));
         c3 = __uint_as_float(__builtin_amdgcn_readfirstlane(__float_as_uint(c3)));
-        if constexpr (ROWS && NS == 4) {
+        if constexpr (ROWS && F16) {
             if (p.out_bf16) {
                 const float bound2 = 32768.f * (c3 / p.u3);
                 so = f16x2_scale(__float_as_uint(__fmaf_rn(p.w3_norm, bound2, p.b3_max)));
@@ -333,10 +334,25 @@
                             continue;
                         }
                     }
+                    if constexpr (NS == 2 && DIRECT) {
+                        if (p.t_bf16) {
+                            const char* rb = reinterpret_cast<const char*>(trow[j]) + c * 128 + 8 * qi(j4);
+                            const uint2 h = *reinterpret_cast<const uint2*>(rb), l = *reinterpret_cast<const uint2*>(rb + 64);
+                            trw[j][j4] = __builtin_bit_cast(f32x4, u32x4{h.x, h.y, l.x, l.y});
+                            continue;
+                        }
+                    }
                     trw[j][j4] = *reinterpret_cast<const f32x4*>(trow[j] + c * 8 + qi(j4));
                 }
         };
         auto blend = [&]() {
+            if constexpr (NS == 2 && DIRECT) {
+                if (p.t_bf16) {
+#pragma unroll
+                    for (int j4 = 0; j4 < 4; ++j4) raw[j4] = trw[0][j4];
+                    return;
+                }
+            }
 #pragma unroll
             for (int j4 = 0; j4 < 4; ++j4)
 #pragma unroll
@@ -532,8 +548,13 @@
                     v[e] = ROWS ? raw[j4][e] : __fmaf_rn(wz[e], dz, __fmaf_rn(wy[e], dy, __fmaf_rn(wx[e], dx, raw[j4][e])));
                 unsigned lo[NPL], hi[NPL];
                 if constexpr (DIRECT) {
+                    if (NS == 2 && p.t_bf16) {
+                        lo[0] = __float_as_uint(v[0]); hi[0] = __float_as_uint(v[1]);
+                        lo[NPL - 1] = __float_as_uint(v[2]); hi[NPL - 1] = __float_as_uint(v[3]);
+                    } else {
                     split_planes<NS>(v[0], v[1], lo);
                     split_planes<NS>(v[2], v[3], hi);
+                    }
                 } else if constexpr (NS == 1) {
                     split_planes<NS>(v[0], v[1], lo);
                     split_planes<NS>(v[2], v[3], hi);
@@ -824,7 +845,25 @@
                         const int pt = 8 * (r >> 2) + (r & 3);
                         float o = acc[r] * c3 + b3u;
                         if (p.relu_out) o = fmaxf(o, 0.f);
+                        unsigned pw = 0u;
+                        if constexpr (NS == 2) {
+                            if (p.out_bf16) {
+                                o = __builtin_amdgcn_fmed3f(o * so, -65504.f, 65504.f);
+                                unsigned pl[2];
+                                split_planes<2>(o, 0.f, pl);
+                                const unsigned mine = (pl[0] & 0xffffu) | (pl[1] << 16);
+                                const unsigned nb = (unsigned)__builtin_amdgcn_update_dpp(0, (int)mine, 0xB1, 0xf, 0xf, false);
+                                pw = (lane & 1) ? ((nb >> 16) | (mine & 0xffff0000u)) : ((mine & 0xffffu) | (nb << 16));
+                                typedef _Float16 h16x2 __attribute__((ext_vector_type(2)));
+                                const h16x2 hl = __builtin_bit_cast(h16x2, mine);
+                                o = ((float)hl[0] + (float)hl[1]) * pow2_inverse(so);
+                            }
+                        }
                         if (colok && row0 + 4 * half + pt < p.N) {
+                            if (NS == 2 && p.out_bf16) {
+                                char* orow8 = reinterpret_cast<char*>(p.out) + ((size_t)b * p.N + row0 + 4 * half + pt) * p.ldo * 4 + 128 * u;
+                                *reinterpret_cast<unsigned*>(orow8 + ((lane & 1) ? 64 + 2 * (l31 - 1) : 2 * l31)) = pw;
+                            } else
                             if (NS == 1 && p.out_bf16) {
                                 unsigned short* o16 = reinterpret_cast<unsigned short*>(p.out) + ((size_t)b * p.N + row0 + 4 * half + pt) * p.ldo + 32 * u + l31;
                                 *o16 = (unsigned short)(__builtin_bit_cast(unsigned, __builtin_convertvector(f32x2{o, 0.f}, bf16x2)) & 0xffffu);
@@ -1045,8 +1084,12 @@
 
 int ev2h_fp_mlp_ex(const ev2h_fp_desc* d, int t_bf16, int out_bf16, ev2h_stream_t stream, float* row16_scale, float w3_norm, float b3_max) {
     EV2H_CHECK_ARG(d && d->T && d->W2s && d->W3s && d->b2 && d->b3 && d->out);
-    EV2H_CHECK_ARG(!(t_bf16 || out_bf16) || ((d->precision == EV2H_PREC_BF16 || (d->precision == EV2H_PREC_F16 && row16_scale && d->t_amax)) &&
+    EV2H_CHECK_ARG(!(t_bf16 || out_bf16) || ((d->precision == EV2H_PREC_BF16 || ((d->precision == EV2H_PREC_F16 || d->precision == EV2H_PREC_F16X2) && row16_scale && d->t_amax)) &&
                                              (!out_bf16 || !d->out_cm) && (!t_bf16 || !d->nn_idx)));
+    if (d->precision == EV2H_PREC_F16X2) {
+        EV2H_CHECK_ARG(!out_bf16 || (d->C3 % 32 == 0 && d->ldo >= d->C3 && d->out_cols <= 0));
+        EV2H_CHECK_ARG(!t_bf16 || (d->C1 % 32 == 0 && d->ldt >= d->C1));
+    }
     EV2H_CHECK_ARG((d->nn_idx != nullptr) == (d->nn_w != nullptr));
     EV2H_CHECK_ARG(d->B > 0 && d->N > 0 && d->ldt >= d->C1 && (d->ldt % 4) == 0);
     const int ncols = d->out_cols > 0 ? d->out_cols : d->C3;
diff --git a/ev2hands_amd/csrc/workspace.hip b/ev2hands_amd/csrc/workspace.hip
--- a/ev2hands_amd/csrc/workspace.hip
+++ b/ev2hands_amd/csrc/workspace.hip
@@ -91,7 +91,7 @@
 namespace {
 __global__ __launch_bounds__(256) void spread_count_kernel(const float* __restrict__ buf, size_t window_stride, int rows, int ld, int col0, int ncols,
                                                            const unsigned* __restrict__ rec, const unsigned* __restrict__ rec2,
-                                                           unsigned* __restrict__ counts, int half_elems) {
+                                                           unsigned* __restrict__ counts, int half_elems, const float* __restrict__ stored = nullptr) {
     const int b = blockIdx.y;
     unsigned a = rec[b];
     if (rec2) a = max(a, rec2[b]);
@@ -102,7 +102,13 @@
     for (size_t i = (size_t)blockIdx.x * 256 + threadIdx.x; i < total; i += (size_t)gridDim.x * 256) {
         const size_t r = i / ncols;
         const int c = (int)(i - r * ncols);
-        const float v = fabsf(half_elems ? (float)reinterpret_cast<const _Float16*>(buf)[(size_t)b * window_stride + r * ld + col0 + c] : base[r * ld + col0 + c]) * s;
+        float v;
+        if (half_elems == 2) {
+            const _Float16* hp = reinterpret_cast<const _Float16*>(base + r * ld) + ((col0 + c) >> 5) * 64 + ((col0 + c) & 31);
+            v = fabsf(((float)hp[0] + (float)hp[32]) * pow2_inverse(stored[b])) * s;
+        } else {
+            v = fabsf(half_elems ? (float)reinterpret_cast<const _Float16*>(buf)[(size_t)b * window_stride + r * ld + col0 + c] : base[r * ld + col0 + c]) * s;
+        }
         nz += v > 0.f;
         lo += v > 0.f && v < 0.125f;
         hi += v > 0.f && v < 6.103515625e-05f;
@@ -140,7 +146,7 @@
         const int gx = (int)std::min<size_t>(64, ((size_t)rows * e[i].ncols + 4095) / 4096);
         spread_count_kernel<<<dim3(std::max(gx, 1), B), 256, 0, (hipStream_t)st>>>(p, per_window, rows, e[i].ld, e[i].col0, e[i].ncols, ws.r(e[i].rec),
                                                                                   e[i].rec2 >= 0 ? ws.r(e[i].rec2) : nullptr, counts + (size_t)i * B * 3,
-                                                                                  (e[i].buf == WS_L0 && g_last_l0_bf16 == 2) ? 1 : 0);
+                                                                                  e[i].buf != WS_L0 ? 0 : (g_last_l0_bf16 == 2 ? 1 : (g_last_l0_bf16 == 3 ? 2 : 0)), ws.p1scale(5));
         EV2H_CHECK_LAUNCH();
     }
     return EV2H_OK;
diff --git a/ev2hands_amd/model.py b/ev2hands_amd/model.py
--- a/ev2hands_amd/model.py
+++ b/ev2hands_amd/model.py
@@ -394,13 +394,18 @@
         if not p:
             raise KeyError(name)
         off = p - ws.data_ptr()
-        if et.value in (1, 2):
+        if et.value in (1, 2, 3):
+            kind = {1: "bf16", 2: "fp16", 3: "fp16 plane pairs"}[et.value]
             if dtype != torch.float32:
-                raise TypeError(f"workspace buffer {name!r} holds {'bf16' if et.value == 1 else 'fp16'} values in this mode: ask for float32")
+                raise TypeError(f"workspace buffer {name!r} holds {kind} in this mode: ask for float32")
             if et.value == 1:
                 return ws[off:off + cnt.value * 2].view(torch.bfloat16).float()
+            scale = self.debug_buffer("p1scale").view(6, B)[5].view(B, 1)
+            if et.value == 3:
+                pl = ws[off:off + cnt.value * 4].view(torch.float16).view(-1, 2, 32).float()
+                return ((pl[:, 0] + pl[:, 1]).reshape(B, -1) / scale).view(-1)
             v = ws[off:off + cnt.value * 2].view(torch.float16).float().view(B, -1)
-            return (v / self.debug_buffer("p1scale").view(6, B)[5].view(B, 1)).view(-1)
+            return (v / scale).view(-1)
         return ws[off:off + cnt.value * 4].view(dtype).clone()
 
 
```

Result: no change. 21850 event-windows/s (-0.1%).
